# ruiminshen/yolo2-pytorch

Measured on AMD Instinct MI355X. Metric: images/sec (416x416) train+detect, Darknet-19 YOLOv2: value = TRAIN step, batch 64 per GPU (configs[2]) at every N; detect (configs[1]) = roofline.detect_images_per_sec, higher is better.
Workload: dtype f32; 1 GPU; Darknet-19 YOLOv2 20-class train 416x416 batch-64/GPU: fwd + region loss + bwd + SGD (BASELINE configs[2]); classes=20, global_batch=64, parallelism=single GPU, weights=random-init seed 0 (bench_data.randomize)

## Files before the change

### include/yolo2_hip.h

```cpp
#ifndef YOLO2_HIP_H
#define YOLO2_HIP_H

#include <stdint.h>

#ifdef __cplusplus
extern "C" {
#endif

#define Y2_OK 0
#define Y2_EINVAL (-1)
#define Y2_EALIGN (-2)
#define Y2_ENOSUP (-3)

#define Y2_STATS_REPL 32

typedef void* y2_stream_t;

int y2_abi_version(void);
const char* y2_build_info(void);


int y2_pack_weight(const float* w, float* dst, int Cout, int Cin, int ksize, int mode, y2_stream_t stream);

#define Y2_PREP_FPROP 0
#define Y2_PREP_DGRAD 1
#define Y2_PREP_WINO_FPROP 2
#define Y2_PREP_WINO_DGRAD 3
#define Y2_PREP_WINO6_DGRAD 4
#define Y2_PREP_MAX_ITEMS 96
typedef struct {
    const float* src;
    float* dst;
    int32_t Cout, Cin, ksize, mode;
} y2_prep_item;
int y2_prep_weights(const y2_prep_item* items, int32_t count, y2_stream_t stream);

#define Y2_MULTI_ZERO 0
#define Y2_MULTI_F64_TO_F32 1
#define Y2_MULTI_COPY 2
#define Y2_MULTI_MAX_ITEMS 96
typedef struct {
    const void* src;
    float* dst;
    int64_t n;
    int32_t op, reserved;
} y2_multi_item;
int y2_multi(const y2_multi_item* items, int32_t count, y2_stream_t stream);

int y2_small_dot(const float* v, const float* w, int32_t n, float* out, y2_stream_t stream);
int y2_small_scale(const float* g, const float* w, int32_t n, float* out, y2_stream_t stream);

int y2_unpack_weight_grad(const float* src, float* dst, int Cout, int Cin, int ksize, y2_stream_t stream);

int y2_bn_fold(const float* gamma, const float* beta, const float* mean, const float* var, float eps,
               float* scale, float* shift, int C, y2_stream_t stream);

typedef struct y2_conv_params {
    const float* x;
    const float* w;
    const float* scale;
    const float* shift;
    float* y;
    float* y_pool;
    double* stats;
    int32_t B, H, W;
    int32_t Cin, ldx;
    int32_t Cout;
    int32_t ksize;
    int32_t ldy, coff;
    int32_t ldp, poff;
    int32_t out_mode;
    float slope;
    int32_t tile;
    float* workspace;
    int64_t workspace_bytes;
    const float* residual;
    int32_t ldr;
    int32_t stride;
    int32_t pad_plus1;
    int32_t transposed;
    int32_t out_h, out_w;
    int32_t algo;
    int64_t w_plane;
} y2_conv_params;

#define Y2_ALGO_DIRECT 0
#define Y2_ALGO_WINOGRAD 1
#define Y2_ALGO_WINOGRAD_FUSED 2
#define Y2_ALGO_WINOGRAD_IMPLICIT 3
#define Y2_ALGO_WINOGRAD_SPLIT 4

#define Y2_ALGO_WINOGRAD_F43 6
#define Y2_ALGO_WINOGRAD_F43_PRE 7
#define Y2_ALGO_WINOGRAD_SPLIT_F16 5

int y2_split_f16x2(const float* src, void* dst, long long n, float scale, y2_stream_t stream);
int y2_split_f16_overflow(int reset);
int y2_gemm_split_f16(const void* A, const void* B, float* C, long long M, int32_t N, int32_t K, int32_t ldc, int32_t groups, float out_scale, y2_stream_t stream);

int y2_split_bf16x3(const float* src, void* dst, long long n, y2_stream_t stream);

int y2_gemm_split(const void* A, const void* B, float* C, long long M, int32_t N, int32_t K, int32_t ldc, int32_t groups, y2_stream_t stream);

int y2_wino_weight(const float* w_packed, float* u, int32_t Cout, int32_t Cin, y2_stream_t stream);
int y2_wino6_weight(const float* w_packed, float* u6, int32_t Cout, int32_t Cin, y2_stream_t stream);

long long y2_wino_wgrad_workspace_bytes(int32_t B, int32_t H, int32_t W, int32_t Cin, int32_t Cout);
long long y2_wino_wgrad_workspace_bytes_ex(int32_t B, int32_t H, int32_t W, int32_t Cin, int32_t Cout, int32_t native_layout);
int y2_wino_wgrad(const float* x, const float* dz, float* dw_packed, int32_t B, int32_t H, int32_t W, int32_t Cin, int32_t ldx,
                  int32_t Cout, int32_t ldz, const float* v_transformed, float* workspace, long long workspace_bytes, y2_stream_t stream);
int y2_wino_wgrad_ex(const float* x, const float* dz, float* dw, int32_t B, int32_t H, int32_t W, int32_t Cin, int32_t ldx,
                     int32_t Cout, int32_t ldz, const float* v_transformed, float* workspace, long long workspace_bytes, int32_t native_layout,
                     y2_stream_t stream);

int y2_conv_fwd(const y2_conv_params* p, y2_stream_t stream);

long long y2_conv_fwd_workspace_bytes(const y2_conv_params* p);

int y2_conv_fwd_batch(const y2_conv_params* params, int count, y2_stream_t stream);

int y2_conv0_fwd(const float* x_nchw, const float* w, const float* scale, const float* shift,
                 float* y, float* y_pool, double* stats,
                 int B, int H, int W, int Cin, int Cout, int ldy, int ldp, float slope, y2_stream_t stream);

int y2_maxpool2_fwd(const float* x, float* y, int B, int H, int W, int C, int ldx, int ldy, y2_stream_t stream);

int y2_maxpool_fwd(const float* x, float* y, int B, int H, int W, int C, int ldx, int ldy, int ksize, int stride, int pad, int pad_end, y2_stream_t stream);

int y2_nchw_to_nhwc(const float* x, float* y, int B, int C, int H, int W, int ld, y2_stream_t stream);

int y2_decode(const float* feature, const float* anchors, int B, int rows, int cols, int A, int C,
              float* iou, float* center_offset, float* size_norm, float* yx_min, float* yx_max, float* prob,
              float* prob_cls, int32_t* cls, y2_stream_t stream);

int y2_filter_visible(const float* iou, const float* prob, int B, int n, int C, int fix, float thr,
                      int32_t* count, int32_t* index, float* prob_cls, int32_t* cls, y2_stream_t stream);

int y2_expand_classes(const float* iou, const float* prob, const float* yx_min, const float* yx_max, const int32_t* cand, const int32_t* keep,
                      const int32_t* keep_count, int32_t B, int32_t n, int32_t C, int32_t limit, float threshold_cls, float* k_iou, float* k_min, float* k_max,
                      float* e_min, float* e_max, float* e_score, long long* e_cls, int32_t* e_count, y2_stream_t stream);

int y2_iou_rowmax(const float* yx_min1, const float* yx_max1, const float* yx_min2, const float* yx_max2, int32_t N1, int32_t N2, float min_union,
                  float* best, long long* which, y2_stream_t stream);

#define Y2_EVAL_MATCH_MAX_G 1024
int y2_eval_match(const float* det_min, const float* det_max, const long long* det_cls, const int32_t* det_count,
                  const float* gt_min, const float* gt_max, const long long* gt_cls, const uint8_t* gt_difficult,
                  int32_t B, int32_t M, int32_t G, int32_t C, float threshold, float min_union, uint8_t* tp, int32_t* cls_num, y2_stream_t stream);

#define Y2_COLLATE_MAX_W 4096
int y2_collate_images(const uint8_t* src, const int64_t* offset, const int32_t* geom, const float* lut,
                      int32_t B, int32_t H, int32_t W, int32_t flags, float* out, y2_stream_t stream);

#define Y2_WARP_MAX_DIM 16384
int y2_warp_affine_images(const uint8_t* src, const int64_t* src_offset, const int32_t* src_geom, const double* inv,
                          uint8_t* dst, const int64_t* dst_offset, const int32_t* dst_geom,
                          int32_t B, int32_t max_h, int32_t max_w, int32_t fill, y2_stream_t stream);

#define Y2_JITTER_MAX_BLUR 7
int y2_collate_jitter_images(const uint8_t* src, const int64_t* offset, const int32_t* geom, const int32_t* jitter, const uint8_t* hsv_tab,
                             const float* lut, int32_t B, int32_t H, int32_t W, int32_t flags, float* out, y2_stream_t stream);

#define Y2_JPEG_MAX_DIM 16384
#define Y2_JPEG_DESC_BYTES 4096
int y2_jpeg_decode_images(const uint8_t* src, int64_t src_bytes, const int64_t* src_offset, const uint8_t* desc,
                          uint8_t* dst, int64_t dst_bytes, const int64_t* dst_offset, const int32_t* dst_geom,
                          uint8_t* ws, int64_t ws_bytes, int32_t* status, int32_t B, y2_stream_t stream);

#define Y2_KMEANS_MAX_K 16
int y2_anchor_kmeans(const double* size, int32_t N, int32_t K, const int32_t* init, int32_t R, int32_t max_iter, double conv_test,
                     double* means, int32_t* iters, int32_t* status, double* cost, int32_t* counts, y2_stream_t stream);
int y2_anchor_assign(const double* size, int32_t N, const double* means, int32_t K, int32_t* index, double* iou, y2_stream_t stream);

int y2_iou_matrix(const float* yx_min1, const float* yx_max1, const float* yx_min2, const float* yx_max2,
                  int Bt, int N1, int N2, float min_union, int mode, float* out, y2_stream_t stream);
int y2_iou_pair(const float* yx_min1, const float* yx_max1, const float* yx_min2, const float* yx_max2,
                int n, float min_union, float* out, y2_stream_t stream);

int y2_nms(const float* score, const float* yx_min, const float* yx_max, const int32_t* cand, const int32_t* n, int B, int stride,
           float overlap, int limit, int32_t* order_ws, int32_t* keep, int32_t* keep_count, y2_stream_t stream);

int y2_nms_host(const float* score, const float* yx_min, const float* yx_max, const int32_t* cand, const int32_t* n, int B, int stride,
                float overlap, int limit, int32_t* keep, int32_t* keep_count);
int y2_iou_matrix_host(const float* yx_min1, const float* yx_max1, const float* yx_min2, const float* yx_max2,
                       int Bt, int N1, int N2, float min_union, int mode, float* out);
int y2_iou_pair_host(const float* yx_min1, const float* yx_max1, const float* yx_min2, const float* yx_max2,
                     int n, float min_union, float* out);
int y2_eval_match_host(const float* det_min, const float* det_max, const long long* det_cls, const int32_t* det_count,
                       const float* gt_min, const float* gt_max, const long long* gt_cls, const uint8_t* gt_difficult,
                       int32_t B, int32_t M, int32_t G, int32_t C, float threshold, float min_union, uint8_t* tp, int32_t* cls_num);
int y2_collate_images_host(const uint8_t* src, const int64_t* offset, const int32_t* geom, const float* lut,
                           int32_t B, int32_t H, int32_t W, int32_t flags, float* out);
int y2_warp_affine_images_host(const uint8_t* src, const int64_t* src_offset, const int32_t* src_geom, const double* inv,
                               uint8_t* dst, const int64_t* dst_offset, const int32_t* dst_geom,
                               int32_t B, int32_t max_h, int32_t max_w, int32_t fill);
int y2_collate_jitter_images_host(const uint8_t* src, const int64_t* offset, const int32_t* geom, const int32_t* jitter, const uint8_t* hsv_tab,
                                  const float* lut, int32_t B, int32_t H, int32_t W, int32_t flags, float* out);
int y2_jpeg_probe_host(const uint8_t* data, int64_t nbytes, uint8_t* desc);
long long y2_jpeg_workspace_bytes(const uint8_t* desc, int32_t B);
int y2_jpeg_decode_images_host(const uint8_t* src, int64_t src_bytes, const int64_t* src_offset, const uint8_t* desc,
                               uint8_t* dst, int64_t dst_bytes, const int64_t* dst_offset, const int32_t* dst_geom,
                               uint8_t* ws, int64_t ws_bytes, int32_t* status, int32_t B);
int y2_anchor_kmeans_host(const double* size, int32_t N, int32_t K, const int32_t* init, int32_t R, int32_t max_iter, double conv_test,
                          double* means, int32_t* iters, int32_t* status, double* cost, int32_t* counts);
int y2_anchor_assign_host(const double* size, int32_t N, const double* means, int32_t K, int32_t* index, double* iou);

int y2_set_deterministic(int on, float* workspace, long long workspace_bytes);
int y2_get_deterministic(void);
int y2_colstats_det(const float* z, long long M, int32_t C, int32_t ld, double* stats, float* workspace, long long workspace_bytes, y2_stream_t stream);

int y2_prof_enable(int on);
int y2_prof_count(void);
int y2_prof_get(int i, char* name, int name_cap, float* ms, double* flops);
int y2_prof_set_tag(int tag);
int y2_prof_get_tag(int i);


int y2_conv_wgrad(const float* x, const float* dz, float* dw, int B, int H, int W, int Cin, int ldx, int Cout, int ldz,
                  int ksize, y2_stream_t stream);

int y2_conv_wgrad_ex(const float* x, const float* dz, float* dw, int B, int Hi, int Wi, int Cin, int ldx, int Cout, int ldz,
                     int ksize, int stride, int pad, y2_stream_t stream);

int y2_conv0_wgrad(const float* x_nchw, const float* dz, float* dw, int B, int H, int W, int Cin, int Cout, int ldz, y2_stream_t stream);

int y2_conv0_wgrad_fused(const float* x_nchw, const float* z, const float* scale, const float* shift, const float* mean, const float* invstd,
                         const float* gamma, float slope, const float* dy_pool, int32_t ldp, const double* sums, float* dw,
                         int32_t B, int32_t H, int32_t W, int32_t Cin, int32_t Cout, int32_t ldz, int32_t has_bn, y2_stream_t stream);

int y2_bn_finalize(const double* stats, double count, const float* gamma, const float* beta,
                   float* running_mean, float* running_var, float momentum, float eps,
                   float* scale, float* shift, float* mean, float* invstd, int C, long long* num_batches_tracked, y2_stream_t stream);

int y2_bn_act_fwd(const float* z, const float* scale, const float* shift, float slope, float* y, float* y_pool,
                  int B, int H, int W, int C, int ldz, int ldy, int coff, int ldp, int poff, int out_mode, y2_stream_t stream);

int y2_bn_act_bwd(const float* z, const float* scale, const float* shift, const float* mean, const float* invstd, const float* gamma,
                  float slope, const float* dy_full, int ldf, int foff, int fmode, const float* dy_pool, int ldp, int poff,
                  double* sums, float* dz, int ldd, int B, int H, int W, int C, int ldz, int has_bn, y2_stream_t stream);

int y2_bn_act_fwd_ex(const float* z, const float* scale, const float* shift, float slope, const float* residual, int ldr, float* y, float* y_pool,
                     int B, int H, int W, int C, int ldz, int ldy, int coff, int ldp, int poff, int out_mode, y2_stream_t stream);
int y2_bn_act_bwd_ex(const float* z, const float* scale, const float* shift, const float* mean, const float* invstd, const float* gamma,
                     float slope, const float* dy_full, int ldf, int foff, int fmode, const float* dy_pool, int ldp, int poff,
                     const float* dy_full2, int ld2, const float* residual, int ldr, float* dres, int lddr,
                     double* sums, float* dz, int ldd, int B, int H, int W, int C, int ldz, int has_bn, y2_stream_t stream);

long long y2_wino6_tiles(int32_t B, int32_t H, int32_t W);
int y2_bn_act_bwd_wino6(const float* z, const float* scale, const float* shift, const float* mean, const float* invstd, const float* gamma,
                        float slope, const float* dy_full, int ldf, int foff, double* sums, float* v6, float* m6, float* dz, int ldd,
                        int B, int H, int W, int C, int ldz, int has_bn, y2_stream_t stream);

int y2_maxpool_bwd(const float* x, const float* dy, const float* dy2, float* dx, int B, int H, int W, int C, int ldx, int ldy, int lddx,
                   int ksize, int stride, int pad, int pad_end, y2_stream_t stream);

int y2_colsum(const float* x, long long M, int C, int ld, double* out, y2_stream_t stream);
int y2_f64_to_f32(const double* src, float* dst, int n, double mul, y2_stream_t stream);

int y2_decode_bwd(const float* iou, const float* center_offset, const float* d_iou, const float* d_center_offset, const float* d_size_norm,
                  const float* d_logits, float* d_feature, int boxes, int C, y2_stream_t stream);

int y2_region_loss_fwd(const float* iou, const float* center_offset, const float* size_norm, const float* logits,
                       const float* yx_min, const float* yx_max,
                       const float* gt_yx_min, const float* gt_yx_max, const int64_t* gt_cls, const float* gt_onehot,
                       const float* anchors, int B, int rows, int cols, int A, int C, int N, float threshold,
                       float* best_iou, int32_t* best_idx, uint8_t* positive, double* sums, float* loss_out, y2_stream_t stream);

int y2_region_loss_finalize(const double* sums, double cnt, int cross_entropy, float* loss_out, y2_stream_t stream);

int y2_region_loss_bwd(const float* iou, const float* center_offset, const float* size_norm, const float* logits,
                       const float* gt_yx_min, const float* gt_yx_max, const int64_t* gt_cls, const float* gt_onehot,
                       const float* anchors, int B, int rows, int cols, int A, int C, int N, float threshold,
                       const float* best_iou, const int32_t* best_idx, const uint8_t* positive, const double* sums, const float* weights,
                       float* d_iou, float* d_center_offset, float* d_size_norm, float* d_logits, y2_stream_t stream);

#define Y2_OPT_MAX_TENSORS 48
typedef struct {
    float* param;
    float* grad;
    float* state1;
    float* state2;
    int64_t numel;
} y2_opt_tensor;

int y2_opt_sgd(const y2_opt_tensor* tensors, int32_t count, float lr, float momentum, float dampening, float weight_decay,
               int32_t nesterov, int32_t first_step, y2_stream_t stream);
int y2_opt_adam(const y2_opt_tensor* tensors, int32_t count, float lr, float beta1, float beta2, float eps, float weight_decay,
                int32_t step, y2_stream_t stream);
int y2_opt_grad_sumsq(const y2_opt_tensor* tensors, int32_t count, double* sumsq, y2_stream_t stream);
int y2_opt_clip_grads(const y2_opt_tensor* tensors, int32_t count, const double* sumsq, float max_norm, y2_stream_t stream);

int y2_dwconv_fwd(const float* x, const float* w, const float* scale, const float* shift, float slope, float* y, double* stats,
                  int B, int H, int W, int C, int ldx, int ldy, int stride, y2_stream_t stream);
int y2_dwconv_dgrad(const float* dz, const float* w, float* dx, int B, int H, int W, int C, int ldz, int lddx, int stride, y2_stream_t stream);
int y2_dwconv_wgrad(const float* x, const float* dz, float* dw, float* workspace, long long workspace_bytes,
                    int B, int H, int W, int C, int ldx, int ldz, int stride, y2_stream_t stream);
long long y2_dwconv_wgrad_workspace_bytes(int B, int H, int W, int C, int stride);

int y2_preact_conv1x1_fwd(const float* x, const float* w, const float* pre_scale, const float* pre_shift, float pre_slope,
                          const float* scale, const float* shift, float slope, float* y, double* stats,
                          int B, int H, int W, int K, int ldx, int N, int ldy, int coff, int pool, y2_stream_t stream);
int y2_preact_fwd(const float* x, const float* pre_scale, const float* pre_shift, float pre_slope, float* out,
                  int B, int H, int W, int C, int ldx, int ldo, int pool, y2_stream_t stream);
int y2_preact_bwd(const float* x, const float* pre_scale, const float* pre_shift, float pre_slope, const float* mean, const float* invstd,
                  const float* gamma, const float* dA, int ldda, double* sums, float* dx, int lddx, int accumulate,
                  int B, int H, int W, int C, int ldx, int pool, int has_bn, y2_stream_t stream);

#ifdef __cplusplus
}
#endif
#endif
```

### yolo2-pytorch_amd/_hip.py

```python
import ctypes
import os
import subprocess

import torch

_HERE = os.path.dirname(os.path.abspath(__file__))
LIB_PATH = os.environ.get('Y2_LIB') or os.path.join(_HERE, 'csrc', 'libyolo2_hip.so')
_lib = None

c_int, c_float, c_void_p = ctypes.c_int, ctypes.c_float, ctypes.c_void_p


class ConvParams(ctypes.Structure):
    _fields_ = [('x', c_void_p), ('w', c_void_p), ('scale', c_void_p), ('shift', c_void_p),
                ('y', c_void_p), ('y_pool', c_void_p), ('stats', c_void_p),
                ('B', ctypes.c_int32), ('H', ctypes.c_int32), ('W', ctypes.c_int32),
                ('Cin', ctypes.c_int32), ('ldx', ctypes.c_int32), ('Cout', ctypes.c_int32), ('ksize', ctypes.c_int32),
                ('ldy', ctypes.c_int32), ('coff', ctypes.c_int32), ('ldp', ctypes.c_int32), ('poff', ctypes.c_int32),
                ('out_mode', ctypes.c_int32), ('slope', c_float), ('tile', ctypes.c_int32),
                ('workspace', c_void_p), ('workspace_bytes', ctypes.c_int64),
                ('residual', c_void_p), ('ldr', ctypes.c_int32), ('stride', ctypes.c_int32), ('pad_plus1', ctypes.c_int32),
                ('transposed', ctypes.c_int32), ('out_h', ctypes.c_int32), ('out_w', ctypes.c_int32), ('algo', ctypes.c_int32),
                ('w_plane', ctypes.c_int64)]


class OptTensor(ctypes.Structure):
    _fields_ = [('param', c_void_p), ('grad', c_void_p), ('state1', c_void_p), ('state2', c_void_p), ('numel', ctypes.c_int64)]


OPT_MAX_TENSORS = 48


class PrepItem(ctypes.Structure):
    _fields_ = [('src', c_void_p), ('dst', c_void_p), ('Cout', ctypes.c_int32), ('Cin', ctypes.c_int32), ('ksize', ctypes.c_int32), ('mode', ctypes.c_int32)]


PREP_FPROP, PREP_DGRAD, PREP_WINO_FPROP, PREP_WINO_DGRAD, PREP_WINO6_DGRAD = 0, 1, 2, 3, 4


class MultiItem(ctypes.Structure):
    _fields_ = [('src', c_void_p), ('dst', c_void_p), ('n', ctypes.c_int64), ('op', ctypes.c_int32), ('reserved', ctypes.c_int32)]


MULTI_ZERO, MULTI_F64_TO_F32, MULTI_COPY = 0, 1, 2

EVAL_MATCH_MAX_G = 1024
COLLATE_MAX_W = 4096
WARP_MAX_DIM = 16384
JITTER_MAX_BLUR = 7
JPEG_MAX_DIM = 16384
JPEG_DESC_BYTES = 4096
KMEANS_MAX_K = 16

SIGNATURES = {
    'y2_abi_version': [],
    'y2_pack_weight': [c_void_p, c_void_p, c_int, c_int, c_int, c_int, c_void_p],
    'y2_prep_weights': [ctypes.POINTER(PrepItem), c_int, c_void_p],
    'y2_expand_classes': [c_void_p] * 7 + [c_int, c_int, c_int, c_int, c_float] + [c_void_p] * 8 + [c_void_p],
    'y2_iou_rowmax': [c_void_p, c_void_p, c_void_p, c_void_p, c_int, c_int, c_float, c_void_p, c_void_p, c_void_p],
    'y2_split_bf16x3': [c_void_p, c_void_p, ctypes.c_longlong, c_void_p],
    'y2_split_f16x2': [c_void_p, c_void_p, ctypes.c_longlong, c_float, c_void_p],
    'y2_split_f16_overflow': [c_int],
    'y2_gemm_split_f16': [c_void_p, c_void_p, c_void_p, ctypes.c_longlong, c_int, c_int, c_int, c_int, c_float, c_void_p],
    'y2_gemm_split': [c_void_p, c_void_p, c_void_p, ctypes.c_longlong, c_int, c_int, c_int, c_int, c_void_p],
    'y2_multi': [ctypes.POINTER(MultiItem), c_int, c_void_p],
    'y2_small_dot': [c_void_p, c_void_p, c_int, c_void_p, c_void_p],
    'y2_small_scale': [c_void_p, c_void_p, c_int, c_void_p, c_void_p],
    'y2_unpack_weight_grad': [c_void_p, c_void_p, c_int, c_int, c_int, c_void_p],
    'y2_bn_fold': [c_void_p, c_void_p, c_void_p, c_void_p, c_float, c_void_p, c_void_p, c_int, c_void_p],
    'y2_conv_fwd': [ctypes.POINTER(ConvParams), c_void_p],
    'y2_conv_fwd_workspace_bytes': [ctypes.POINTER(ConvParams)],
    'y2_wino_weight': [c_void_p, c_void_p, c_int, c_int, c_void_p],
    'y2_wino6_weight': [c_void_p, c_void_p, c_int, c_int, c_void_p],
    'y2_opt_sgd': [ctypes.POINTER(OptTensor), c_int, c_float, c_float, c_float, c_float, c_int, c_int, c_void_p],
    'y2_opt_adam': [ctypes.POINTER(OptTensor), c_int, c_float, c_float, c_float, c_float, c_float, c_int, c_void_p],
    'y2_opt_grad_sumsq': [ctypes.POINTER(OptTensor), c_int, c_void_p, c_void_p],
    'y2_opt_clip_grads': [ctypes.POINTER(OptTensor), c_int, c_void_p, c_float, c_void_p],
    'y2_wino_wgrad_workspace_bytes': [c_int, c_int, c_int, c_int, c_int],
    'y2_wino_wgrad_workspace_bytes_ex': [c_int, c_int, c_int, c_int, c_int, c_int],
    'y2_wino_wgrad': [c_void_p, c_void_p, c_void_p, c_int, c_int, c_int, c_int, c_int, c_int, c_int, c_void_p, c_void_p, ctypes.c_longlong, c_void_p],
    'y2_wino_wgrad_ex': [c_void_p, c_void_p, c_void_p, c_int, c_int, c_int, c_int, c_int, c_int, c_int, c_void_p, c_void_p, ctypes.c_longlong, c_int, c_void_p],
    'y2_conv_fwd_batch': [ctypes.POINTER(ConvParams), c_int, c_void_p],
    'y2_conv0_fwd': [c_void_p, c_void_p, c_void_p, c_void_p, c_void_p, c_void_p, c_void_p,
                     c_int, c_int, c_int, c_int, c_int, c_int, c_int, c_float, c_void_p],
    'y2_maxpool2_fwd': [c_void_p, c_void_p, c_int, c_int, c_int, c_int, c_int, c_int, c_void_p],
    'y2_maxpool_fwd': [c_void_p, c_void_p, c_int, c_int, c_int, c_int, c_int, c_int, c_int, c_int, c_int, c_int, c_void_p],
    'y2_nchw_to_nhwc': [c_void_p, c_void_p, c_int, c_int, c_int, c_int, c_int, c_void_p],
    'y2_decode': [c_void_p, c_void_p, c_int, c_int, c_int, c_int, c_int,
                  c_void_p, c_void_p, c_void_p, c_void_p, c_void_p, c_void_p, c_void_p, c_void_p, c_void_p],
    'y2_filter_visible': [c_void_p, c_void_p, c_int, c_int, c_int, c_int, c_float, c_void_p, c_void_p, c_void_p, c_void_p, c_void_p],
    'y2_iou_matrix': [c_void_p, c_void_p, c_void_p, c_void_p, c_int, c_int, c_int, c_float, c_int, c_void_p, c_void_p],
    'y2_iou_pair': [c_void_p, c_void_p, c_void_p, c_void_p, c_int, c_float, c_void_p, c_void_p],
    'y2_conv_wgrad': [c_void_p, c_void_p, c_void_p, c_int, c_int, c_int, c_int, c_int, c_int, c_int, c_int, c_void_p],
    'y2_conv_wgrad_ex': [c_void_p, c_void_p, c_void_p, c_int, c_int, c_int, c_int, c_int, c_int, c_int, c_int, c_int, c_int, c_void_p],
    'y2_conv0_wgrad_fused': [c_void_p] * 7 + [c_float, c_void_p, c_int, c_void_p, c_void_p] + [c_int] * 7 + [c_void_p],
    'y2_conv0_wgrad': [c_void_p, c_void_p, c_void_p, c_int, c_int, c_int, c_int, c_int, c_int, c_void_p],
    'y2_bn_finalize': [c_void_p, ctypes.c_double, c_void_p, c_void_p, c_void_p, c_void_p, c_float, c_float, c_void_p, c_void_p, c_void_p, c_void_p, c_int, c_void_p, c_void_p],
    'y2_bn_act_fwd': [c_void_p, c_void_p, c_void_p, c_float, c_void_p, c_void_p, c_int, c_int, c_int, c_int, c_int, c_int, c_int, c_int, c_int, c_int, c_void_p],
    'y2_bn_act_bwd': [c_void_p, c_void_p, c_void_p, c_void_p, c_void_p, c_void_p, c_float, c_void_p, c_int, c_int, c_int, c_void_p, c_int, c_int,
                      c_void_p, c_void_p, c_int, c_int, c_int, c_int, c_int, c_int, c_int, c_void_p],
    'y2_bn_act_fwd_ex': [c_void_p, c_void_p, c_void_p, c_float, c_void_p, c_int, c_void_p, c_void_p, c_int, c_int, c_int, c_int, c_int, c_int, c_int, c_int, c_int, c_int, c_void_p],
    'y2_bn_act_bwd_ex': [c_void_p, c_void_p, c_void_p, c_void_p, c_void_p, c_void_p, c_float, c_void_p, c_int, c_int, c_int, c_void_p, c_int, c_int,
                         c_void_p, c_int, c_void_p, c_int, c_void_p, c_int,
                         c_void_p, c_void_p, c_int, c_int, c_int, c_int, c_int, c_int, c_int, c_void_p],
    'y2_wino6_tiles': [c_int, c_int, c_int],
    'y2_bn_act_bwd_wino6': [c_void_p, c_void_p, c_void_p, c_void_p, c_void_p, c_void_p, c_float, c_void_p, c_int, c_int, c_void_p, c_void_p, c_void_p, c_void_p, c_int,
                            c_int, c_int, c_int, c_int, c_int, c_int, c_void_p],
    'y2_maxpool_bwd': [c_void_p, c_void_p, c_void_p, c_void_p, c_int, c_int, c_int, c_int, c_int, c_int, c_int, c_int, c_int, c_int, c_int, c_void_p],
    'y2_colsum': [c_void_p, ctypes.c_longlong, c_int, c_int, c_void_p, c_void_p],
    'y2_dwconv_fwd': [c_void_p, c_void_p, c_void_p, c_void_p, c_float, c_void_p, c_void_p, c_int, c_int, c_int, c_int, c_int, c_int, c_int, c_void_p],
    'y2_dwconv_dgrad': [c_void_p, c_void_p, c_void_p, c_int, c_int, c_int, c_int, c_int, c_int, c_int, c_void_p],
    'y2_dwconv_wgrad': [c_void_p, c_void_p, c_void_p, c_void_p, ctypes.c_longlong, c_int, c_int, c_int, c_int, c_int, c_int, c_int, c_void_p],
    'y2_dwconv_wgrad_workspace_bytes': [c_int, c_int, c_int, c_int, c_int],
    'y2_preact_conv1x1_fwd': [c_void_p, c_void_p, c_void_p, c_void_p, c_float, c_void_p, c_void_p, c_float, c_void_p, c_void_p] + [c_int] * 9 + [c_void_p],
    'y2_preact_fwd': [c_void_p, c_void_p, c_void_p, c_float, c_void_p] + [c_int] * 7 + [c_void_p],
    'y2_preact_bwd': [c_void_p, c_void_p, c_void_p, c_float, c_void_p, c_void_p, c_void_p, c_void_p, c_int, c_void_p, c_void_p, c_int, c_int] + [c_int] * 7 + [c_void_p],
    'y2_f64_to_f32': [c_void_p, c_void_p, c_int, ctypes.c_double, c_void_p],
    'y2_decode_bwd': [c_void_p, c_void_p, c_void_p, c_void_p, c_void_p, c_void_p, c_void_p, c_int, c_int, c_void_p],
    'y2_region_loss_fwd': [c_void_p] * 11 + [c_int] * 6 + [c_float] + [c_void_p] * 5 + [c_void_p],
    'y2_region_loss_finalize': [c_void_p, ctypes.c_double, c_int, c_void_p, c_void_p],
    'y2_region_loss_bwd': [c_void_p] * 9 + [c_int] * 6 + [c_float] + [c_void_p] * 5 + [c_void_p] * 4 + [c_void_p],
    'y2_nms_host': [c_void_p, c_void_p, c_void_p, c_void_p, c_void_p, c_int, c_int, c_float, c_int, c_void_p, c_void_p],
    'y2_iou_matrix_host': [c_void_p, c_void_p, c_void_p, c_void_p, c_int, c_int, c_int, c_float, c_int, c_void_p],
    'y2_iou_pair_host': [c_void_p, c_void_p, c_void_p, c_void_p, c_int, c_float, c_void_p],
    'y2_eval_match': [c_void_p] * 8 + [c_int, c_int, c_int, c_int, c_float, c_float, c_void_p, c_void_p, c_void_p],
    'y2_eval_match_host': [c_void_p] * 8 + [c_int, c_int, c_int, c_int, c_float, c_float, c_void_p, c_void_p],
    'y2_collate_images': [c_void_p] * 4 + [c_int, c_int, c_int, c_int, c_void_p, c_void_p],
    'y2_collate_images_host': [c_void_p] * 4 + [c_int, c_int, c_int, c_int, c_void_p],
    'y2_warp_affine_images': [c_void_p] * 7 + [c_int, c_int, c_int, c_int, c_void_p],
    'y2_warp_affine_images_host': [c_void_p] * 7 + [c_int, c_int, c_int, c_int],
    'y2_collate_jitter_images': [c_void_p] * 6 + [c_int, c_int, c_int, c_int, c_void_p, c_void_p],
    'y2_collate_jitter_images_host': [c_void_p] * 6 + [c_int, c_int, c_int, c_int, c_void_p],
    'y2_jpeg_probe_host': [c_void_p, ctypes.c_int64, c_void_p],
    'y2_jpeg_workspace_bytes': [c_void_p, c_int],
    'y2_jpeg_decode_images': [c_void_p, ctypes.c_int64, c_void_p, c_void_p, c_void_p, ctypes.c_int64, c_void_p, c_void_p, c_void_p, ctypes.c_int64, c_void_p, c_int, c_void_p],
    'y2_jpeg_decode_images_host': [c_void_p, ctypes.c_int64, c_void_p, c_void_p, c_void_p, ctypes.c_int64, c_void_p, c_void_p, c_void_p, ctypes.c_int64, c_void_p, c_int],
    'y2_anchor_kmeans': [c_void_p, c_int, c_int, c_void_p, c_int, c_int, ctypes.c_double] + [c_void_p] * 5 + [c_void_p],
    'y2_anchor_kmeans_host': [c_void_p, c_int, c_int, c_void_p, c_int, c_int, ctypes.c_double] + [c_void_p] * 5,
    'y2_anchor_assign': [c_void_p, c_int, c_void_p, c_int, c_void_p, c_void_p, c_void_p],
    'y2_anchor_assign_host': [c_void_p, c_int, c_void_p, c_int, c_void_p, c_void_p],
    'y2_set_deterministic': [c_int, c_void_p, ctypes.c_longlong],
    'y2_get_deterministic': [],
    'y2_colstats_det': [c_void_p, ctypes.c_longlong, c_int, c_int, c_void_p, c_void_p, ctypes.c_longlong, c_void_p],
    'y2_prof_enable': [c_int],
    'y2_prof_count': [],
    'y2_prof_set_tag': [c_int],
    'y2_prof_get_tag': [c_int],
    'y2_prof_get': [c_int, ctypes.c_char_p, c_int, ctypes.POINTER(c_float), ctypes.POINTER(ctypes.c_double)],
    'y2_nms': [c_void_p, c_void_p, c_void_p, c_void_p, c_void_p, c_int, c_int, c_float, c_int, c_void_p, c_void_p, c_void_p, c_void_p],
}

STATS_REPL = 32

ERRORS = {-1: 'Y2_EINVAL (bad size / null pointer)', -2: 'Y2_EALIGN (unaligned pointer or stride)', -3: 'Y2_ENOSUP (unsupported combination)'}


class HipLibraryMissing(RuntimeError):
    pass


def build(verbose=False):
    out = subprocess.run(['bash', os.path.join(_HERE, 'csrc', 'build.sh')], capture_output=True, text=True)
    if verbose or out.returncode != 0:
        print(out.stdout + out.stderr)
    if out.returncode != 0:
        raise RuntimeError('building libyolo2_hip.so failed')
    return LIB_PATH


def lib():
    global _lib
    if _lib is None:
        if not os.path.exists(LIB_PATH):
            raise HipLibraryMissing('%s not found: run `python __graft_entry__.py build` (or yolo2-pytorch_amd/csrc/build.sh); '
                                    'the YOLOv2 hot path has no CPU/eager fallback' % LIB_PATH)
        l = ctypes.CDLL(LIB_PATH)
        for name, argtypes in SIGNATURES.items():
            fn = getattr(l, name)
            fn.argtypes = argtypes
            fn.restype = c_int
        l.y2_conv_fwd_workspace_bytes.restype = ctypes.c_longlong
        l.y2_wino_wgrad_workspace_bytes.restype = ctypes.c_longlong
        l.y2_wino6_tiles.restype = ctypes.c_longlong
        l.y2_dwconv_wgrad_workspace_bytes.restype = ctypes.c_longlong
        l.y2_wino_wgrad_workspace_bytes_ex.restype = ctypes.c_longlong
        l.y2_jpeg_workspace_bytes.restype = ctypes.c_longlong
        l.y2_build_info.argtypes = []
        l.y2_build_info.restype = ctypes.c_char_p
        _lib = l
    return _lib


LAUNCHES = [0]


def check(rc, what):
    LAUNCHES[0] += 1
    if rc != 0:
        if rc <= -1000:
            raise RuntimeError('%s: HIP error %d' % (what, -rc - 1000))
        raise RuntimeError('%s: %s' % (what, ERRORS.get(rc, rc)))


_LAUNCH = None


def stream():
    return c_void_p((_LAUNCH if _LAUNCH is not None else torch.cuda.current_stream()).cuda_stream)


class launch_on(object):

    def __init__(self, s):
        self.s, self.prev = s, None

    def __enter__(self):
        global _LAUNCH
        self.prev, _LAUNCH = _LAUNCH, self.s
        return self.s

    def __exit__(self, *exc):
        global _LAUNCH
        _LAUNCH = self.prev
        return False


def _timing_stream():
    import contextlib
    return torch.cuda.stream(_LAUNCH) if _LAUNCH is not None else contextlib.nullcontext()


def ptr(t):
    return None if t is None else c_void_p(t.data_ptr())


def multi(items, st=None):
    if not items:
        return
    table = (MultiItem * len(items))()
    for e, (op, dst, src) in zip(table, items):
        e.op, e.dst = op, dst.data_ptr()
        if op == MULTI_ZERO:
            nbytes = dst.numel() * dst.element_size()
            assert nbytes % 4 == 0 and dst.is_contiguous()
            e.n, e.src = nbytes // 4, None
        else:
            assert dst.dtype == torch.float32 and dst.is_contiguous() and src.is_contiguous() and src.numel() >= dst.numel()
            e.n, e.src = dst.numel(), src.data_ptr()
    check(lib().y2_multi(table, len(items), stream() if st is None else st), 'y2_multi')


def require_gpu(*tensors):
    for t in tensors:
        if t is not None and not t.is_cuda:
            raise RuntimeError('yolo2-hip: this operator runs only on an MI355X GPU tensor (got device %s); there is no CPU fallback' % t.device)


def wrote(tensors):
    try:
        torch.autograd.graph.increment_version(tensors)
    except TypeError:
        for t in tensors:
            torch.autograd.graph.increment_version(t)


_TUNE_EPOCH = [0]


def tune_epoch():
    return _TUNE_EPOCH[0]


DETERMINISTIC = os.environ.get('Y2_DETERMINISTIC', '0') == '1'
_DET_WS = {}
_DET_BYTES = int(os.environ.get('Y2_DET_WS_MB', '256')) << 20


def set_deterministic(on, dev=None):
    global DETERMINISTIC
    DETERMINISTIC = bool(on)
    L = lib()
    if not on:
        check(L.y2_set_deterministic(0, None, 0), 'y2_set_deterministic')
        return
    dev = torch.device('cuda', torch.cuda.current_device()) if dev is None else torch.device(dev)
    ws = _DET_WS.get(str(dev))
    if ws is None:
        ws = torch.empty(_DET_BYTES // 4, dtype=torch.float32, device=dev)
        _DET_WS[str(dev)] = ws
    check(L.y2_set_deterministic(1, ws.data_ptr(), ws.numel() * 4), 'y2_set_deterministic')


def ensure_deterministic(dev):
    if DETERMINISTIC and (str(torch.device(dev)) not in _DET_WS or not lib().y2_get_deterministic()):
        set_deterministic(True, dev)
    return DETERMINISTIC


def colstats_det(z, M, C, ld, stats):
    G = min(1024, (M + 255) // 256)
    key = 'colstats:' + str(z.device)
    ws = _DET_WS.get(key)
    if ws is None or ws.numel() * 4 < G * 2 * C * 8:
        ws = torch.empty(max(G * 2 * C * 2, 1 << 18), dtype=torch.float32, device=z.device)
        _DET_WS[key] = ws
    check(lib().y2_colstats_det(ptr(z), M, C, ld, ptr(stats), ptr(ws), ws.numel() * 4, stream()), 'y2_colstats_det')


_WS = {}
SCOPE = None


def _cache(d):
    if SCOPE is None:
        return d
    return SCOPE.setdefault(('_hip', id(d)), {})


def workspace(dev, nbytes):
    key = str(dev)
    ws = _cache(_WS)
    t = ws.get(key)
    if t is None or t.numel() * 4 < nbytes:
        _retire(t)
        t = torch.empty(max(int(nbytes) // 4 + 4, 1024), dtype=torch.float32, device=dev)
        ws[key] = t
    return t


def _retire(t):
    if t is not None and SCOPE is not None:
        SCOPE.setdefault(('_hip', 'retired'), []).append(t)


def conv_workspace(params, dev):
    need = lib().y2_conv_fwd_workspace_bytes(ctypes.byref(params))
    if need > 0:
        ws = workspace(dev, need)
        params.workspace, params.workspace_bytes = ws.data_ptr(), ws.numel() * 4
    else:
        params.workspace, params.workspace_bytes = None, 0
    return need


class PlanCache(object):

    def __init__(self, entries=None, gbytes=None):
        import collections
        self.entries = int(os.environ.get('Y2_PLAN_CACHE', '12')) if entries is None else entries
        self.bytes = int(float(os.environ.get('Y2_PLAN_CACHE_GB', '64')) * (1 << 30)) if gbytes is None else int(gbytes * (1 << 30))
        self.d = collections.OrderedDict()
        self.hits = self.misses = 0

    def get(self, key):
        plan = self.d.get(key)
        if plan is None:
            self.misses += 1
            return None
        self.hits += 1
        self.d.move_to_end(key)
        return plan

    def put(self, key, plan, nbytes):
        self.d[key] = plan
        plan['nbytes'] = nbytes
        while len(self.d) > 1 and (len(self.d) > self.entries or sum(p['nbytes'] for p in self.d.values()) > self.bytes):
            self.d.popitem(last=False)

    def latest(self):
        return next(reversed(self.d.values())) if self.d else None

    def clear(self):
        self.d.clear()


_TUNE = {}
TUNE_MISSES = []
AUTOTUNE = os.environ.get('Y2_AUTOTUNE', '1') != '0'
TUNE_CACHE = os.environ.get('Y2_TUNE_CACHE')
if TUNE_CACHE and os.path.exists(TUNE_CACHE):
    try:
        import json as _json
        _TUNE.update({tuple(_json.loads(k)): v for k, v in _json.load(open(TUNE_CACHE)).items()})
    except Exception:
        pass


TUNE_DEFAULTS = os.environ.get('Y2_TUNE_DEFAULTS', '1') != '0'
DEFAULTS_PATH = os.path.join(_HERE, 'tune', 'default_gfx950.json')
_DEFAULTS_SEEN = {}


def kernel_hash():
    import glob
    import hashlib
    files = sorted(glob.glob(os.path.join(_HERE, 'csrc', '*.hip'))) + [os.path.join(_HERE, 'csrc', 'common.h'), os.path.join(_HERE, 'csrc', 'resample.h'), os.path.join(_HERE, 'csrc', 'jpeg.h'), os.path.join(_HERE, 'csrc', 'kmeans.h'), os.path.join(os.path.dirname(_HERE), 'include', 'yolo2_hip.h')]
    if len(files) < 3 or not all(os.path.exists(f) for f in files):
        return None
    h = hashlib.sha256()
    for f in files:
        h.update(os.path.basename(f).encode())
        for line in open(f, 'r', errors='replace'):
            if line.startswith('// y2-build-flags:'):
                h.update(line.strip().encode())
                h.update(b'\n')
            cut = line.find('//')
            while cut >= 0 and line.count('"', 0, cut) % 2:
# ... 383 lines not shown
```

### yolo2-pytorch_amd/csrc/conv0_fwd.hip

```cpp
#include <stdlib.h>
#include "common.h"

namespace {

constexpr int TH = 16, TW = 32;
constexpr int PW = 48;
constexpr int PLANE = (TH + 2) * PW;

struct Conv0Args {
    const float* x; const float* w; const float* scale; const float* shift;
    float* y; float* y_pool; double* stats;
    int B, H, W, Cout, ldy, ldp;
    float slope;
    int tiles_y, tiles_x, ntiles;
};

typedef float f32x2 __attribute__((ext_vector_type(2)));

template <int CIN>
struct StepTap {
    static constexpr int G0 = 3 * CIN, G1 = G0 + CIN, G2 = G1 + CIN / 2;
    static constexpr int group(int s) { return s < G0 ? 0 : s < G1 ? 1 : s < G2 ? 2 : 3; }
    static constexpr int tap0(int s) {
        return s < G0 ? (s / 3) * 9 + (s % 3) * 3 : s < G1 ? (s - G0) * 9 + 2 : s < G2 ? (2 * (s - G1)) * 9 + 8 : (CIN - 1) * 9 + 8;
    }
    static constexpr int tap1(int s) {
        return s < G0 ? tap0(s) + 1 : s < G1 ? tap0(s) + 3 : s < G2 ? tap0(s) + 9 : -1;
    }
    static constexpr int lds(int tap) { return (tap / 9) * PLANE + ((tap % 9) / 3) * PW + (tap % 3); }
    static constexpr int dist(int g) { return g == 0 ? 1 : g == 1 ? PW : g == 2 ? PLANE : 0; }
};

template <int CIN, int NBLK, int OUT = -1, bool FULL = false, bool RAW = false>
__global__ __launch_bounds__(256) void conv0_kernel(const Conv0Args a) {
    const bool has_y = OUT < 0 ? a.y != nullptr : (OUT & 1) != 0;
    const bool has_pool = OUT < 0 ? a.y_pool != nullptr : (OUT & 2) != 0;
    const bool has_stats = OUT < 0 ? a.stats != nullptr : (OUT & 4) != 0;
    constexpr bool POOL_FIRST = FULL && OUT == 2 && !RAW;
    constexpr int K = CIN * 9;
    constexpr int KS = (K + 1) / 2;
    constexpr int PR = TH + 2;
    constexpr int RPW = (PR + 3) / 4, RIT = CIN * RPW;
    __shared__ __attribute__((aligned(16))) float patch[3][CIN * PLANE];

    const int t = threadIdx.x;
    const int lane = t & 63, wave = __builtin_amdgcn_readfirstlane(t >> 6);
    const int l31 = lane & 31, half = lane >> 5;
    const int ldy = FULL ? 32 * NBLK : a.ldy, ldp = FULL ? 32 * NBLK : a.ldp;

    float sc[NBLK], sh[NBLK];
#pragma unroll
    for (int j = 0; j < NBLK; ++j) {
        const int n = j * 32 + l31;
        sc[j] = (!RAW && a.scale != nullptr && n < a.Cout) ? a.scale[n] : 1.f;
        sh[j] = (!RAW && a.shift != nullptr && n < a.Cout) ? a.shift[n] : 0.f;
    }
    float wreg[NBLK][KS];
#pragma unroll
    for (int j = 0; j < NBLK; ++j) {
        const int n = j * 32 + l31;
#pragma unroll
        for (int s = 0; s < KS; ++s) {
            const int k = half ? StepTap<CIN>::tap1(s) : StepTap<CIN>::tap0(s);
            const float w = (n < a.Cout && k >= 0) ? a.w[(size_t)n * K + k] : 0.f;
            wreg[j][s] = (POOL_FIRST && sc[j] < 0.f) ? -w : w;
        }
        if (POOL_FIRST) sc[j] = fabsf(sc[j]);
    }

    float pv[RIT];
    const int HW = a.H * a.W;
    auto origin = [&](int tile, int& b, int& y0, int& x0) {
        const unsigned u = (unsigned)tile, row = u / (unsigned)a.tiles_x, tx = u - row * (unsigned)a.tiles_x;
        const unsigned ub = row / (unsigned)a.tiles_y, ty = row - ub * (unsigned)a.tiles_y;
        b = (int)ub; y0 = (int)ty * TH; x0 = (int)tx * TW;
    };
    auto issue = [&](int b, int y0, int x0) {
        const float* xb = a.x + (size_t)b * CIN * HW;
        const int gx = min(max(x0 + lane - 1, 0), a.W - 1);
#pragma unroll
        for (int it = 0; it < RIT; ++it) {
            const int c = it / RPW, py = min(wave + 4 * (it % RPW), PR - 1);
            const int gy = min(max(y0 + py - 1, 0), a.H - 1);
            const float* rowp = xb + (c * HW + gy * a.W);
            pv[it] = rowp[gx];
        }
    };
    auto commit = [&](int y0, int x0, float* dst) {
        const bool okx = (unsigned)(x0 + lane - 1) < (unsigned)a.W;
        float* d = dst + wave * PW + lane;
        if (lane < TW + 2) {
#pragma unroll
            for (int it = 0; it < RIT; ++it) {
                const int c = it / RPW, k4 = 4 * (it % RPW), py = wave + k4;
                const bool oky = (unsigned)(y0 + py - 1) < (unsigned)a.H;
                const float v = (okx && oky) ? pv[it] : 0.f;
                if (k4 + 3 < PR || py < PR) d[c * PLANE + k4 * PW] = v;
            }
        }
    };

    double d1[NBLK], d2[NBLK];
#pragma unroll
    for (int j = 0; j < NBLK; ++j) { d1[j] = 0.0; d2[j] = 0.0; }
    const int stride = gridDim.x;
    int tile = blockIdx.x;
    __builtin_amdgcn_s_waitcnt(0x0f70);
    int b, y0, x0, b1 = 0, y1 = 0, x1 = 0;
    origin(tile, b, y0, x0);
    issue(b, y0, x0);
    commit(y0, x0, patch[0]);
    if (tile + stride < a.ntiles) { origin(tile + stride, b1, y1, x1); issue(b1, y1, x1); commit(y1, x1, patch[1]); }
    __syncthreads();

    const int wi = l31 >> 2, e = l31 & 3;
    const int lpy = e >> 1, lpx = 2 * wi + (e & 1);
    int buf = 0;
    for (; tile < a.ntiles; tile += stride, buf = buf == 2 ? 0 : buf + 1) {
    const float* cur = patch[buf];
    const bool more = tile + 2 * stride < a.ntiles;
    int b2 = 0, y2 = 0, x2 = 0;
    f32x2 s1[NBLK], s2[NBLK];
#pragma unroll
    for (int j = 0; j < NBLK; ++j) { s1[j] = 0.f; s2[j] = 0.f; }
    const int bt = b, yt = y0, xt = x0;

#pragma unroll 1
    for (int blk = 0; blk < 4; blk += 2) {
        const int rp = (wave * 4 + blk) >> 1;
        const int pbase = (2 * rp + lpy) * PW + lpx;
        f32x16 acc[2][NBLK];
#pragma unroll
        for (int u = 0; u < 2; ++u)
#pragma unroll
            for (int j = 0; j < NBLK; ++j)
#pragma unroll
                for (int r = 0; r < 16; ++r) acc[u][j][r] = 0.f;
        float av[2][KS];
        const float* gb[4];
#pragma unroll
        for (int g = 0; g < 4; ++g) gb[g] = cur + pbase + (half ? StepTap<CIN>::dist(g) : 0);
#pragma unroll
        for (int s = 0; s < KS; ++s) {
            const int g = StepTap<CIN>::group(s);
#pragma unroll
            for (int u = 0; u < 2; ++u) {
                av[u][s] = gb[g][StepTap<CIN>::lds(StepTap<CIN>::tap0(s)) + 16 * u];
                if (g == 3) av[u][s] = half ? 0.f : av[u][s];
            }
        }
        __builtin_amdgcn_sched_barrier(0);
#if defined(Y2_C0_DBG) && (Y2_C0_DBG & 1)
#pragma unroll
        for (int u = 0; u < 2; ++u)
#pragma unroll
            for (int j = 0; j < NBLK; ++j)
#pragma unroll
                for (int r = 0; r < 16; ++r) acc[u][j][r] = av[u][r % KS] * wreg[j][r % KS];
#else
#pragma unroll
        for (int s = 0; s < KS; ++s)
#pragma unroll
            for (int u = 0; u < 2; ++u)
#pragma unroll
                for (int j = 0; j < NBLK; ++j)
                    acc[u][j] = __builtin_amdgcn_mfma_f32_32x32x2f32(av[u][s], wreg[j][s], acc[u][j], 0, 0, 0);
#endif
#if !(defined(Y2_C0_DBG) && (Y2_C0_DBG & 4))
        if (more) {
            if (blk == 0) { origin(tile + 2 * stride, b2, y2, x2); issue(b2, y2, x2); }
            else commit(y2, x2, patch[buf == 0 ? 2 : buf - 1]);
        }
#endif
#if defined(Y2_C0_DBG) && (Y2_C0_DBG & 2)
        if (acc[0][0][0] + acc[1][0][5] == 12345.678f) a.y_pool[lane] = 1.f;
        if (false)
#endif
#pragma unroll
        for (int u = 0; u < 2; ++u) {
        const int Y0 = yt + 2 * rp, X0 = xt + 16 * u;
        float* yb0 = has_y ? a.y + ((size_t)(bt * a.H + Y0) * a.W + X0) * ldy : nullptr;
        float* yb1 = has_y ? yb0 + (size_t)a.W * ldy : nullptr;
        float* pb = has_pool ? a.y_pool + ((size_t)(bt * (a.H >> 1) + (Y0 >> 1)) * (a.W >> 1) + (X0 >> 1)) * ldp : nullptr;
        const unsigned ylane = (unsigned)(2 * half * ldy + l31), plane = (unsigned)(half * ldp + l31);
#pragma unroll
        for (int j = 0; j < NBLK; ++j) {
            const int n = j * 32 + l31;
            const bool nok = FULL || n < a.Cout;
#pragma unroll
            for (int g = 0; g < 4; ++g) {
                const int w = 2 * g + half;
                const int Y = Y0, X = X0 + 2 * w;
                if (has_stats) {
                    if (FULL) {
                        const f32x2 za = {acc[u][j][4 * g], acc[u][j][4 * g + 1]}, zb = {acc[u][j][4 * g + 2], acc[u][j][4 * g + 3]};
                        s1[j] += za; s2[j] = __builtin_elementwise_fma(za, za, s2[j]);
                        s1[j] += zb; s2[j] = __builtin_elementwise_fma(zb, zb, s2[j]);
                    } else {
#pragma unroll
                        for (int q = 0; q < 4; ++q) {
                            const float z = acc[u][j][4 * g + q];
                            if ((Y + (q >> 1)) < a.H && (X + (q & 1)) < a.W) { s1[j][q & 1] += z; s2[j][q & 1] += z * z; }
                        }
                    }
                }
                if (!nok) continue;
                if (POOL_FIRST) {
                    const float m = fmaxf(fmaxf(acc[u][j][4 * g], acc[u][j][4 * g + 1]), fmaxf(acc[u][j][4 * g + 2], acc[u][j][4 * g + 3]));
                    const float uu = m * sc[j] + sh[j];
                    (pb + (2 * g * ldp + j * 32))[plane] = fmaxf(uu, uu * a.slope);
                    continue;
                }
                float v[4];
#pragma unroll
                for (int q = 0; q < 4; ++q) {
                    const float z = acc[u][j][4 * g + q];
                    if (RAW) { v[q] = z; continue; }
                    const float uu = z * sc[j] + sh[j];
                    v[q] = uu > 0.f ? uu : uu * a.slope;
                }
                if (has_y) {
#pragma unroll
                    for (int q = 0; q < 4; ++q) {
                        const int yy = Y + (q >> 1), xx = X + (q & 1);
                        if (FULL || (yy < a.H && xx < a.W)) (((q >> 1) ? yb1 : yb0) + ((4 * g + (q & 1)) * ldy + j * 32))[ylane] = v[q];
                    }
                }
                if (has_pool && (FULL || (Y < a.H && X < a.W))) {
                    const float pm = fmaxf(fmaxf(v[0], v[1]), fmaxf(v[2], v[3]));
                    (pb + (2 * g * ldp + j * 32))[plane] = pm;
                }
            }
        }
        }
    }
    if (has_stats) {
#pragma unroll
        for (int j = 0; j < NBLK; ++j) { d1[j] += (double)s1[j][0] + (double)s1[j][1]; d2[j] += (double)s2[j][0] + (double)s2[j][1]; }
    }
    b = b1; y0 = y1; x0 = x1; b1 = b2; y1 = y2; x1 = x2;
    __syncthreads();
    }
    if (has_stats) {
#pragma unroll
        for (int j = 0; j < NBLK; ++j) {
            const int n = j * 32 + l31;
            const double t1 = d1[j] + __shfl_xor(d1[j], 32);
            const double t2 = d2[j] + __shfl_xor(d2[j], 32);
            if (half == 0 && n < a.Cout) {
                double* st = a.stats + (size_t)(blockIdx.x % Y2_STATS_REPL) * 2 * a.Cout;
                atomicAdd(st + n, t1);
                atomicAdd(st + a.Cout + n, t2);
            }
        }
    }
}

template <int CIN>
int launch0(const Conv0Args& a, hipStream_t s) {
    const long long tiles = (long long)a.B * a.tiles_y * a.tiles_x;
    if (tiles <= 0 || tiles > 0x7fffffffLL) return Y2_EINVAL;
    static const int per_cu = getenv("Y2_CONV0_WGS") != nullptr ? atoi(getenv("Y2_CONV0_WGS")) : 8;
    const long long grid = per_cu > 0 && tiles > (long long)Y2_NUM_CU * per_cu ? (long long)Y2_NUM_CU * per_cu : tiles;
    const double flops = 2.0 * (double)a.B * a.H * a.W * 9 * CIN * a.Cout;
    if (CIN == 3 && (a.H % TH) == 0 && (a.W % TW) == 0 && (a.Cout == 32 || a.Cout == 64) && (a.y == nullptr || a.ldy == a.Cout) && (a.y_pool == nullptr || a.ldp == a.Cout)) {
        const int out = (a.y != nullptr ? 1 : 0) | (a.y_pool != nullptr ? 2 : 0) | (a.stats != nullptr ? 4 : 0);
        const bool raw = a.scale == nullptr && a.shift == nullptr && a.slope == 1.f;
        const bool mono = a.slope >= 0.f && a.slope <= 1.f;
#define Y2_C0(NB_, OUT_, RAW_) Y2_LAUNCH("conv0_kernel", flops, (conv0_kernel<3, NB_, OUT_, true, RAW_>), dim3((unsigned)grid), dim3(256), 0, s, a)
        bool done = true;
        if (a.Cout == 32) {
            if (out == 2 && mono) Y2_C0(1, 2, false); else if (out == 5 && raw) Y2_C0(1, 5, true); else if (out == 5) Y2_C0(1, 5, false);
            else if (out == 1) Y2_C0(1, 1, false); else if (out == 3) Y2_C0(1, 3, false); else done = false;
        } else {
            if (out == 2 && mono) Y2_C0(2, 2, false); else if (out == 5 && raw) Y2_C0(2, 5, true); else if (out == 1) Y2_C0(2, 1, false); else done = false;
        }
#undef Y2_C0
        if (done) { Y2_LAUNCH_CHECK(); return Y2_OK; }
    }
    if (a.Cout <= 32) Y2_LAUNCH("conv0_kernel", flops, (conv0_kernel<CIN, 1>), dim3((unsigned)grid), dim3(256), 0, s, a);
    else Y2_LAUNCH("conv0_kernel", flops, (conv0_kernel<CIN, 2>), dim3((unsigned)grid), dim3(256), 0, s, a);
    Y2_LAUNCH_CHECK();
    return Y2_OK;
}

}

extern "C" int y2_conv0_fwd(const float* x_nchw, const float* w, const float* scale, const float* shift,
                            float* y, float* y_pool, double* stats,
                            int B, int H, int W, int Cin, int Cout, int ldy, int ldp, float slope, y2_stream_t stream) {
    if (x_nchw == nullptr || w == nullptr || (y == nullptr && y_pool == nullptr && stats == nullptr)) return Y2_EINVAL;
    if (B <= 0 || H <= 0 || W <= 0 || Cin < 1 || Cin > 4 || Cout < 1 || Cout > 64) return Y2_ENOSUP;
    if (y != nullptr && ldy < Cout) return Y2_EINVAL;
    if (y_pool != nullptr && (ldp < Cout || (H & 1) || (W & 1))) return Y2_EINVAL;
    if (stats != nullptr && y2_det.on) return Y2_ENOSUP;
    Conv0Args a;
    a.x = x_nchw; a.w = w; a.scale = scale; a.shift = shift; a.y = y; a.y_pool = y_pool; a.stats = stats;
    a.B = B; a.H = H; a.W = W; a.Cout = Cout; a.ldy = ldy; a.ldp = ldp; a.slope = slope;
    a.tiles_y = y2_cdiv(H, TH); a.tiles_x = y2_cdiv(W, TW);
    a.ntiles = B * a.tiles_y * a.tiles_x;
    hipStream_t s = y2_s(stream);
    switch (Cin) {
        case 1: return launch0<1>(a, s);
        case 2: return launch0<2>(a, s);
        case 3: return launch0<3>(a, s);
        default: return launch0<4>(a, s);
    }
}
```

### yolo2-pytorch_amd/csrc/train.hip

```cpp
#include "common.h"

namespace {

inline int stream_grid(long long total, int block, int cap_mult = 8) {
    long long g = (total + block - 1) / block;
    const long long cap = (long long)Y2_NUM_CU * cap_mult;
    return (int)(g < 1 ? 1 : (g > cap ? cap : g));
}

__global__ void bn_finalize_kernel(const double* __restrict__ stats, double n, const float* gamma, const float* beta,
                                   float* running_mean, float* running_var, float momentum, float eps,
                                   float* scale, float* shift, float* mean_out, float* invstd_out, int C, long long* num_batches_tracked) {
    const int c = blockIdx.x * blockDim.x + threadIdx.x;
    if (c >= C) return;
    if (c == 0 && num_batches_tracked != nullptr) *num_batches_tracked += 1;
    double s1 = 0.0, s2 = 0.0;
    for (int r = 0; r < Y2_STATS_REPL; ++r) { s1 += stats[(size_t)r * 2 * C + c]; s2 += stats[(size_t)r * 2 * C + C + c]; }
    const double mean = s1 / n;
    double var = s2 / n - mean * mean;
    if (var < 0.0) var = 0.0;
    const float invstd = (float)(1.0 / sqrt(var + (double)eps));
    const float s = gamma[c] * invstd;
    scale[c] = s;
    shift[c] = beta[c] - (float)mean * s;
    mean_out[c] = (float)mean;
    invstd_out[c] = invstd;
    if (running_mean != nullptr) {
        const double unbiased = n > 1.0 ? var * n / (n - 1.0) : var;
        running_mean[c] = (1.f - momentum) * running_mean[c] + momentum * (float)mean;
        running_var[c] = (1.f - momentum) * running_var[c] + momentum * (float)unbiased;
    }
}

struct ActArgs {
    const float* z; const float* scale; const float* shift;
    float* y; float* y_pool;
    int B, H, W, C, ldz, ldy, coff, ldp, poff, out_mode;
    float slope;
    const float* res; int ldr;
    y2_fastdiv d_wo, d_ho;
};

__device__ __forceinline__ float act1(float z, float sc, float sh, float slope) {
    const float u = z * sc + sh;
    return u > 0.f ? u : u * slope;
}

__device__ __forceinline__ void act_decode(uint32_t p, const y2_fastdiv& d_wo, const y2_fastdiv& d_ho, int Wo, int Ho, int& b, int& yo, int& xo) {
    const uint32_t r = y2_div(p, d_wo);
    xo = (int)(p - r * (uint32_t)Wo);
    const uint32_t bb = y2_div(r, d_ho);
    yo = (int)(r - bb * (uint32_t)Ho);
    b = (int)bb;
}

template <bool POOL, int CV>
__global__ void bn_act_fwd_kernel(const ActArgs a, long long total) {
    const int Cg = a.C / CV;
    const int Wo = POOL ? a.W / 2 : a.W, Ho = POOL ? a.H / 2 : a.H;
    const long long tid = (long long)blockIdx.x * blockDim.x + threadIdx.x;
    const long long nthreads = (long long)gridDim.x * blockDim.x;
    const int c = (int)(tid % Cg) * CV;
    const uint32_t npix = (uint32_t)(total / Cg), pstep = (uint32_t)(nthreads / Cg);
    float sc[CV], sh[CV];
#pragma unroll
    for (int e = 0; e < CV; ++e) { sc[e] = a.scale ? a.scale[c + e] : 1.f; sh[e] = a.shift ? a.shift[c + e] : 0.f; }
    const bool need_yx = POOL || a.out_mode == 1;
    for (uint32_t p = (uint32_t)(tid / Cg); p < npix; p += pstep) {
        int b = 0, yo = 0, xo = 0;
        if (need_yx) act_decode(p, a.d_wo, a.d_ho, Wo, Ho, b, yo, xo);
        float pm[CV];
#pragma unroll
        for (int q = 0; q < (POOL ? 4 : 1); ++q) {
            const int yy = POOL ? 2 * yo + (q >> 1) : yo, xx = POOL ? 2 * xo + (q & 1) : xo;
            const long long pix = need_yx ? ((long long)b * a.H + yy) * a.W + xx : (long long)p;
            float v[CV];
            if (CV == 4) {
                const f32x4 zz = *reinterpret_cast<const f32x4*>(a.z + pix * a.ldz + c);
                f32x4 rr = {0.f, 0.f, 0.f, 0.f};
                if (a.res != nullptr) rr = *reinterpret_cast<const f32x4*>(a.res + pix * a.ldr + c);
#pragma unroll
                for (int e = 0; e < 4; ++e) { const float u = zz[e] * sc[e] + sh[e] + rr[e]; v[e] = u > 0.f ? u : u * a.slope; }
            } else {
                const float u = a.z[pix * a.ldz + c] * sc[0] + sh[0] + (a.res != nullptr ? a.res[pix * a.ldr + c] : 0.f);
                v[0] = u > 0.f ? u : u * a.slope;
            }
            if (a.y != nullptr) {
                long long o;
                if (a.out_mode == 1) {
                    o = (((long long)b * (a.H >> 1) + (yy >> 1)) * (a.W >> 1) + (xx >> 1)) * a.ldy + a.coff + ((yy & 1) * 2 + (xx & 1)) * a.C + c;
                } else {
                    o = pix * a.ldy + a.coff + c;
                }
                if (CV == 4) { f32x4 w = {v[0], v[1], v[2], v[3]}; *reinterpret_cast<f32x4*>(a.y + o) = w; }
                else a.y[o] = v[0];
            }
#pragma unroll
            for (int e = 0; e < CV; ++e) pm[e] = (q == 0) ? v[e] : fmaxf(pm[e], v[e]);
        }
        if (POOL && a.y_pool != nullptr) {
            const long long o = (long long)p * a.ldp + a.poff + c;
            if (CV == 4) { f32x4 w = {pm[0], pm[1], pm[2], pm[3]}; *reinterpret_cast<f32x4*>(a.y_pool + o) = w; }
            else a.y_pool[o] = pm[0];
        }
    }
}

struct ActBwdArgs {
    const float* z; const float* scale; const float* shift; const float* mean; const float* invstd; const float* gamma;
    const float* dy_full; const float* dy_pool;
    const float* dy_full2; int ld2;
    const float* res; int ldr;
    float* dres; int lddr;
    double* sums;
    float* partial;
    float* block_partial;
    float* dz;
    int B, H, W, C, ldz, ldf, foff, fmode, ldp, poff, ldd;
    float slope;
    double n;
    int has_bn;
    y2_fastdiv d_wo, d_ho;
};

template <bool POOL, int CV, bool APPLY>
__global__ void bn_act_bwd_kernel(const ActBwdArgs a, long long total) {
    extern __shared__ float red[];
    const int Cg = a.C / CV;
    if (!APPLY) {
        for (int i = threadIdx.x; i < 2 * a.C; i += blockDim.x) red[i] = 0.f;
        __syncthreads();
    }
    const int Wo = POOL ? a.W / 2 : a.W, Ho = POOL ? a.H / 2 : a.H;
    const long long tid = (long long)blockIdx.x * blockDim.x + threadIdx.x;
    const long long nthreads = (long long)gridDim.x * blockDim.x;
    const int c = (int)(tid % Cg) * CV;
    float sc[CV], sh[CV], mu[CV], is[CV], gs[CV], ma[CV], mb[CV];
#pragma unroll
    for (int e = 0; e < CV; ++e) {
        sc[e] = a.scale ? a.scale[c + e] : 1.f; sh[e] = a.shift ? a.shift[c + e] : 0.f;
        mu[e] = a.has_bn ? a.mean[c + e] : 0.f; is[e] = a.has_bn ? a.invstd[c + e] : 1.f;
        if (APPLY && a.has_bn == 1) {
            gs[e] = a.gamma[c + e] * is[e];
            ma[e] = (float)(a.sums[c + e] / a.n);
            mb[e] = (float)(a.sums[a.C + c + e] / a.n);
        } else if (APPLY && a.has_bn == 2) {
            gs[e] = a.gamma[c + e] * is[e]; ma[e] = 0.f; mb[e] = 0.f;
        } else { gs[e] = 1.f; ma[e] = 0.f; mb[e] = 0.f; }
    }
    float s1[CV], s2[CV];
#pragma unroll
    for (int e = 0; e < CV; ++e) { s1[e] = 0.f; s2[e] = 0.f; }

    const uint32_t npix = (uint32_t)(total / Cg), pstep = (uint32_t)(nthreads / Cg);
    const bool need_yx = POOL || a.fmode == 1;
    for (uint32_t p = (uint32_t)(tid / Cg); p < npix; p += pstep) {
        int b = 0, yo = 0, xo = 0;
        if (need_yx) act_decode(p, a.d_wo, a.d_ho, Wo, Ho, b, yo, xo);
        float zv[POOL ? 4 : 1][CV], yv[POOL ? 4 : 1][CV];
        long long pixs[POOL ? 4 : 1];
#pragma unroll
        for (int q = 0; q < (POOL ? 4 : 1); ++q) {
            const int yy = POOL ? 2 * yo + (q >> 1) : yo, xx = POOL ? 2 * xo + (q & 1) : xo;
            pixs[q] = need_yx ? ((long long)b * a.H + yy) * a.W + xx : (long long)p;
            if (CV == 4) {
                const f32x4 zz = *reinterpret_cast<const f32x4*>(a.z + pixs[q] * a.ldz + c);
#pragma unroll
                for (int e = 0; e < 4; ++e) zv[q][e] = zz[e];
            } else zv[q][0] = a.z[pixs[q] * a.ldz + c];
#pragma unroll
            for (int e = 0; e < CV; ++e) yv[q][e] = zv[q][e] * sc[e] + sh[e];
            if (a.res != nullptr) {
                if (CV == 4) {
                    const f32x4 rr = *reinterpret_cast<const f32x4*>(a.res + pixs[q] * a.ldr + c);
#pragma unroll
                    for (int e = 0; e < 4; ++e) yv[q][e] += rr[e];
                } else yv[q][0] += a.res[pixs[q] * a.ldr + c];
            }
        }
        float dp[CV];
        int arg[CV];
        if (POOL) {
            const long long o = (long long)p * a.ldp + a.poff + c;
            if (CV == 4) { const f32x4 d = *reinterpret_cast<const f32x4*>(a.dy_pool + o);
#pragma unroll
                for (int e = 0; e < 4; ++e) dp[e] = d[e]; }
            else dp[0] = a.dy_pool[o];
#pragma unroll
            for (int e = 0; e < CV; ++e) {
                float best = 0.f; int bi = 0;
#pragma unroll
                for (int q = 0; q < 4; ++q) {
                    const float u = yv[q][e];
                    const float v = u > 0.f ? u : u * a.slope;
                    if (q == 0 || v > best) { best = v; bi = q; }
                }
                arg[e] = bi;
            }
        }
#pragma unroll
        for (int q = 0; q < (POOL ? 4 : 1); ++q) {
            float g[CV];
#pragma unroll
            for (int e = 0; e < CV; ++e) g[e] = (POOL && arg[e] == q) ? dp[e] : 0.f;
            if (a.dy_full != nullptr) {
                const int yy = POOL ? 2 * yo + (q >> 1) : yo, xx = POOL ? 2 * xo + (q & 1) : xo;
                long long o;
                if (a.fmode == 1) o = (((long long)b * (a.H >> 1) + (yy >> 1)) * (a.W >> 1) + (xx >> 1)) * a.ldf + a.foff + ((yy & 1) * 2 + (xx & 1)) * a.C + c;
                else o = pixs[q] * a.ldf + a.foff + c;
                if (CV == 4) { const f32x4 d = *reinterpret_cast<const f32x4*>(a.dy_full + o);
#pragma unroll
                    for (int e = 0; e < 4; ++e) g[e] += d[e]; }
                else g[0] += a.dy_full[o];
            }
            if (a.dy_full2 != nullptr) {
                const long long o = pixs[q] * a.ld2 + c;
                if (CV == 4) { const f32x4 d = *reinterpret_cast<const f32x4*>(a.dy_full2 + o);
#pragma unroll
                    for (int e = 0; e < 4; ++e) g[e] += d[e]; }
                else g[0] += a.dy_full2[o];
            }
            float outv[CV], gev[CV];
#pragma unroll
            for (int e = 0; e < CV; ++e) {
                const float ge = g[e] * (yv[q][e] > 0.f ? 1.f : a.slope);
                gev[e] = ge;
                const float zh = (zv[q][e] - mu[e]) * is[e];
                if (!APPLY) { s1[e] += ge; s2[e] += ge * zh; }
                else outv[e] = gs[e] * (ge - ma[e] - zh * mb[e]);
            }
            if (APPLY) {
                const long long o = pixs[q] * a.ldd + c;
                if (CV == 4) { f32x4 w = {outv[0], outv[1], outv[2], outv[3]}; *reinterpret_cast<f32x4*>(a.dz + o) = w; }
                else a.dz[o] = outv[0];
                if (a.dres != nullptr) {
                    const long long r = pixs[q] * a.lddr + c;
                    if (CV == 4) { f32x4 w = {gev[0], gev[1], gev[2], gev[3]}; *reinterpret_cast<f32x4*>(a.dres + r) = w; }
                    else a.dres[r] = gev[0];
                }
            }
        }
    }
    if (!APPLY && a.partial != nullptr) {
        float* row = a.partial + (size_t)(tid / Cg) * 2 * a.C;
#pragma unroll
        for (int e = 0; e < CV; ++e) { row[c + e] = s1[e]; row[a.C + c + e] = s2[e]; }
        return;
    }
    if (!APPLY) {
#pragma unroll
        for (int e = 0; e < CV; ++e) { atomicAdd(&red[c + e], s1[e]); atomicAdd(&red[a.C + c + e], s2[e]); }
        __syncthreads();
        if (a.block_partial != nullptr) {
            float* row = a.block_partial + (size_t)blockIdx.x * 2 * a.C;
            for (int i = threadIdx.x; i < 2 * a.C; i += blockDim.x) row[i] = red[i];
            return;
        }
        for (int i = threadIdx.x; i < 2 * a.C; i += blockDim.x) {
            const float v = red[i];
            if (v != 0.f) atomicAdd(a.sums + i, (double)v);
        }
    }
}

__global__ __launch_bounds__(1024) void bn_bwd_block_reduce_kernel(const float* __restrict__ part, int rows, int n, double* __restrict__ sums) {
    __shared__ double acc[16][65];
    const int col = blockIdx.x * 64 + (threadIdx.x & 63), lane = threadIdx.x >> 6;
    const int per = (rows + (int)gridDim.y - 1) / (int)gridDim.y;
    const int r0 = blockIdx.y * per, r1 = min(rows, r0 + per);
    double s = 0.0;
    if (col < n)
        for (int r = r0 + lane; r < r1; r += 16) s += (double)part[(size_t)r * n + col];
    acc[lane][threadIdx.x & 63] = s;
    __syncthreads();
    if (lane == 0 && col < n) {
        double t = 0.0;
#pragma unroll
        for (int l = 0; l < 16; ++l) t += acc[l][threadIdx.x & 63];
        atomicAdd(sums + col, t);
    }
}

struct BnWino6Args {
    const float* z; const float* scale; const float* shift; const float* mean; const float* invstd; const float* gamma;
    const float* dy; const double* sums;
    float* v6; float* m6;
    float* dz;
    int B, H, W, C, ldz, ldf, foff, ldd, has_bn;
    float slope;
    double n;
    int th, tw, T, tall, wide, gx;
    y2_fastdiv d_c, d_tt, d_tw, d_tall, d_wide;
};

__global__ __launch_bounds__(256) void bn_bwd_wino6_kernel(const BnWino6Args a) {
    constexpr float BT[6][6] = {{1.f, 1.5f, -2.f, -1.5f, 1.f, 0.f}, {0.f, -1.f, -2.5f, -0.5f, 1.f, 0.f}, {0.f, 1.f, 0.5f, -2.5f, 1.f, 0.f},
                                {0.f, -0.5f, -1.f, 0.5f, 1.f, 0.f}, {0.f, 2.f, -1.f, -2.f, 1.f, 0.f}, {0.f, 1.f, 1.5f, -2.f, -1.5f, 1.f}};
    constexpr float GM[6][4] = {{1.f, 0.f, 0.f, 0.f}, {-1.f / 3, -1.f / 3, -1.f / 3, -1.f / 3}, {1.f / 3, -1.f / 3, 1.f / 3, -1.f / 3},
                                {1.f / 15, 2.f / 15, 4.f / 15, 8.f / 15}, {-16.f / 15, 8.f / 15, -4.f / 15, 2.f / 15}, {0.f, 0.f, 0.f, 1.f}};
    const uint32_t idx = blockIdx.x * 256u + threadIdx.x;
    const uint32_t t = y2_div(idx, a.d_c);
    if (t >= (uint32_t)a.T) return;
    const int c = (int)(idx - t * (uint32_t)a.C);
    const float sc = a.scale ? a.scale[c] : 1.f, sh = a.shift ? a.shift[c] : 0.f;
    const float mu = a.has_bn ? a.mean[c] : 0.f, is = a.has_bn ? a.invstd[c] : 1.f;
    float gs = 1.f, ma = 0.f, mb = 0.f;
    if (a.has_bn == 1) { gs = a.gamma[c] * is; ma = (float)(a.sums[c] / a.n); mb = (float)(a.sums[a.C + c] / a.n); }
    else if (a.has_bn == 2) { gs = a.gamma[c] * is; }
    int b = 0, ty, tx;
    if (a.tall) {
        ty = (int)y2_div(t, a.d_tw);
        tx = (int)t - ty * a.tw;
    } else {
        b = (int)y2_div(t, a.d_tt);
        const int r = (int)t - b * a.th * a.tw;
        ty = (int)y2_div((uint32_t)r, a.d_tw);
        tx = r - ty * a.tw;
    }
    const int y0 = 4 * ty - 1, x0 = 4 * tx - 1;
    int colx[6], colb[6];
#pragma unroll
    for (int j = 0; j < 6; ++j) {
        int xx = x0 + j, bx = 0;
        bool ok = (unsigned)xx < (unsigned)a.W;
        if (a.wide) {
            ok = (unsigned)xx < (unsigned)(a.gx * a.wide);
            bx = ok ? (int)y2_div((uint32_t)xx, a.d_wide) : 0;
            xx -= bx * a.wide;
            ok = ok && xx < a.W;
        }
        colx[j] = ok ? xx : -1;
        colb[j] = bx;
    }
    float d[6][6];
#pragma unroll
    for (int half = 0; half < 2; ++half) {
        uint32_t pixs[3][6];
        bool oks[3][6];
#pragma unroll
        for (int ii = 0; ii < 3; ++ii) {
            int yy = y0 + 3 * half + ii, by = 0;
            bool rowok = (unsigned)yy < (unsigned)a.H;
            if (a.tall) {
                rowok = yy >= 0;
                by = rowok ? (int)y2_div((uint32_t)yy, a.d_tall) : 0;
                yy -= by * a.tall;
                rowok = rowok && yy < a.H;
            }
#pragma unroll
            for (int j = 0; j < 6; ++j) {
                const int bb = a.tall ? by * a.gx + colb[j] : b;
                const bool ok = rowok && colx[j] >= 0 && bb < a.B;
                oks[ii][j] = ok;
                pixs[ii][j] = ok ? (uint32_t)((bb * a.H + yy) * a.W + colx[j]) : 0u;
            }
        }
        float zs[3][6], gsrc[3][6];
#pragma unroll
        for (int ii = 0; ii < 3; ++ii)
#pragma unroll
            for (int j = 0; j < 6; ++j) {
                zs[ii][j] = a.z[(size_t)pixs[ii][j] * a.ldz + c];
                gsrc[ii][j] = a.dy[(size_t)pixs[ii][j] * a.ldf + a.foff + c];
            }
#pragma unroll
        for (int ii = 0; ii < 3; ++ii)
#pragma unroll
            for (int j = 0; j < 6; ++j) {
                const int i = 3 * half + ii;
                const float zv = zs[ii][j];
                const float g = 0.f + gsrc[ii][j];
                const float yv = zv * sc + sh;
                const float ge = g * (yv > 0.f ? 1.f : a.slope);
                const float zh = (zv - mu) * is;
                const float v = oks[ii][j] ? gs * (ge - ma - zh * mb) : 0.f;
                if (a.dz != nullptr && oks[ii][j] && i >= 1 && i <= 4 && j >= 1 && j <= 4) a.dz[(size_t)pixs[ii][j] * a.ldd + c] = v;
                d[i][j] = v;
            }
    }
    const size_t plane = (size_t)a.T * a.C;
    if (a.v6 != nullptr) {
        float sm[6][6];
#pragma unroll
        for (int u = 0; u < 6; ++u)
#pragma unroll
            for (int j = 0; j < 6; ++j) {
                float v = 0.f;
#pragma unroll
                for (int i = 0; i < 6; ++i)
                    if (BT[u][i] != 0.f) v += BT[u][i] * d[i][j];
                sm[u][j] = v;
            }
        float* dst = a.v6 + (size_t)t * a.C + c;
#pragma unroll
        for (int u = 0; u < 6; ++u)
#pragma unroll
            for (int v6 = 0; v6 < 6; ++v6) {
                float v = 0.f;
#pragma unroll
                for (int j = 0; j < 6; ++j)
                    if (BT[v6][j] != 0.f) v += BT[v6][j] * sm[u][j];
                dst[(size_t)(6 * u + v6) * plane] = v;
            }
    }
    if (a.m6 != nullptr) {
        float sm[6][4];
// ... 130 lines not shown
        const int wx = w % WW, wy = w / WW;
        const int oy = y0 / 2 + wy, ox = x0 / 2 + wx;
        int at = 255;
        if (oy < Ho && ox < Wo) {
            float best = 0.f;
#pragma unroll
            for (int ky = 0; ky < 3; ++ky) {
                const int gy = 2 * oy - 1 + ky;
                if ((unsigned)gy >= (unsigned)H) continue;
#pragma unroll
                for (int kx = 0; kx < 3; ++kx) {
                    const int gx = 2 * ox - 1 + kx;
                    if ((unsigned)gx >= (unsigned)W) continue;
                    const float v = xs[((2 * wy + ky) * RW + 2 * wx + kx) * MP_CH + c];
                    if (at == 255 || v > best) { best = v; at = ky * 3 + kx; }
                }
            }
        }
        arg[i] = (unsigned char)at;
    }
    __syncthreads();
    const float* dyb = dy + (size_t)b * Ho * Wo * ldy + c0;
    const float* dy2b = dy2 != nullptr ? dy2 + (size_t)b * Ho * Wo * ldy + c0 : nullptr;
    for (int i = t; i < MP_TH * MP_TW * (MP_CH / 4); i += 256) {
        const int c4 = i % (MP_CH / 4), p = i / (MP_CH / 4);
        const int lx = p % MP_TW, ly = p / MP_TW;
        const int yy = y0 + ly, xx = x0 + lx;
        if (yy >= H || xx >= W) continue;
        float g[4] = {0.f, 0.f, 0.f, 0.f};
#pragma unroll
        for (int a = 0; a < 2; ++a) {
            const int oy = (yy + 1) / 2 - a;
            if (oy < 0 || oy >= Ho || 2 * oy - 1 > yy || 2 * oy + 1 < yy) continue;
#pragma unroll
            for (int bb = 0; bb < 2; ++bb) {
                const int ox = (xx + 1) / 2 - bb;
                if (ox < 0 || ox >= Wo || 2 * ox - 1 > xx || 2 * ox + 1 < xx) continue;
                const int mine = (yy - (2 * oy - 1)) * 3 + (xx - (2 * ox - 1));
                const unsigned char* aw = arg + ((oy - y0 / 2) * WW + (ox - x0 / 2)) * MP_CH + 4 * c4;
                const bool m0 = aw[0] == mine, m1 = aw[1] == mine, m2 = aw[2] == mine, m3 = aw[3] == mine;
                if (m0 || m1 || m2 || m3) {
                    const size_t o = ((size_t)oy * Wo + ox) * ldy + 4 * c4;
                    float4 d = *reinterpret_cast<const float4*>(dyb + o);
                    if (dy2b != nullptr) { const float4 e = *reinterpret_cast<const float4*>(dy2b + o); d.x += e.x; d.y += e.y; d.z += e.z; d.w += e.w; }
                    if (m0) g[0] += d.x;
                    if (m1) g[1] += d.y;
                    if (m2) g[2] += d.z;
                    if (m3) g[3] += d.w;
                }
            }
        }
        *reinterpret_cast<float4*>(dx + ((size_t)(b * H + yy) * W + xx) * lddx + c0 + 4 * c4) = make_float4(g[0], g[1], g[2], g[3]);
    }
}

__global__ void colsum_kernel(const float* __restrict__ x, long long M, int C, int ld, double* out) {
    extern __shared__ float red[];
    for (int i = threadIdx.x; i < C; i += blockDim.x) red[i] = 0.f;
    __syncthreads();
    const long long total = M * C;
    const long long tid = (long long)blockIdx.x * blockDim.x + threadIdx.x, nth = (long long)gridDim.x * blockDim.x;
    const int c = (int)(tid % C);
    float s = 0.f;
    for (long long i = tid; i < total; i += nth) s += x[(i / C) * ld + c];
    atomicAdd(&red[c], s);
    __syncthreads();
    for (int i = threadIdx.x; i < C; i += blockDim.x) if (red[i] != 0.f) atomicAdd(out + i, (double)red[i]);
}

__global__ void f64_to_f32_kernel(const double* s, float* d, int n, double mul) {
    const int i = blockIdx.x * blockDim.x + threadIdx.x;
    if (i < n) d[i] = (float)(s[i] * mul);
}

__global__ void decode_bwd_kernel(const float* __restrict__ iou, const float* __restrict__ co, const float* __restrict__ d_iou,
                                  const float* __restrict__ d_co, const float* __restrict__ d_sn, const float* __restrict__ d_logits,
                                  float* __restrict__ dfeat, int total, int C) {
    const int E = 5 + C;
    for (long long i = (long long)blockIdx.x * blockDim.x + threadIdx.x; i < (long long)total * E; i += (long long)gridDim.x * blockDim.x) {
        const int box = (int)(i / E), k = (int)(i % E);
        float v;
        if (k == 0) { const float s = iou[box]; v = d_iou ? d_iou[box] * s * (1.f - s) : 0.f; }
        else if (k < 3) { const float s = co[2 * (size_t)box + k - 1]; v = d_co ? d_co[2 * (size_t)box + k - 1] * s * (1.f - s) : 0.f; }
        else if (k < 5) v = d_sn ? d_sn[2 * (size_t)box + k - 3] : 0.f;
        else v = d_logits ? d_logits[(size_t)box * C + k - 5] : 0.f;
        dfeat[i] = v;
    }
}

__device__ __forceinline__ float iou_box(float ymin1, float xmin1, float ymax1, float xmax1,
                                         float ymin2, float xmin2, float ymax2, float xmax2) {
    const float ih = fmaxf(fminf(ymax1, ymax2) - fmaxf(ymin1, ymin2), 0.f);
    const float iw = fmaxf(fminf(xmax1, xmax2) - fmaxf(xmin1, xmin2), 0.f);
    const float inter = ih * iw;
    const float a1 = (ymax1 - ymin1) * (xmax1 - xmin1);
    const float a2 = (ymax2 - ymin2) * (xmax2 - xmin2);
    const float uni = fmaxf((a1 + a2) - inter, 1.1920929e-07f);
    return inter / uni;
}

__global__ __launch_bounds__(256) void loss_match_kernel(const float* __restrict__ yx_min, const float* __restrict__ yx_max,
                                                         const float* __restrict__ gt_min, const float* __restrict__ gt_max,
                                                         int n, int N, float* best_iou, int32_t* best_idx, uint8_t* positive, double* sums) {
    __shared__ float g[4 * 256];
    const int b = blockIdx.y;
    const int i = blockIdx.x * 256 + threadIdx.x;
    if (blockIdx.x == 0 && b == 0 && threadIdx.x < 6) sums[threadIdx.x] = 0.0;
    if (i < n) positive[(size_t)b * n + i] = 0;
    float y0 = 0, x0 = 0, y1 = 0, x1 = 0;
    if (i < n) {
        const size_t o = ((size_t)b * n + i) * 2;
        y0 = yx_min[o]; x0 = yx_min[o + 1]; y1 = yx_max[o]; x1 = yx_max[o + 1];
    }
    float best = 0.f; int arg = 0; bool first = true;
    for (int j0 = 0; j0 < N; j0 += 256) {
        const int cnt = min(256, N - j0);
        __syncthreads();
        if (threadIdx.x < cnt) {
            const size_t o = ((size_t)b * N + j0 + threadIdx.x) * 2;
            g[4 * threadIdx.x] = gt_min[o]; g[4 * threadIdx.x + 1] = gt_min[o + 1];
            g[4 * threadIdx.x + 2] = gt_max[o]; g[4 * threadIdx.x + 3] = gt_max[o + 1];
        }
        __syncthreads();
        for (int j = 0; j < cnt; ++j) {
            const float v = iou_box(y0, x0, y1, x1, g[4 * j], g[4 * j + 1], g[4 * j + 2], g[4 * j + 3]);
            if (first || v > best) { best = v; arg = j0 + j; first = false; }
        }
    }
    if (i < n) { best_iou[(size_t)b * n + i] = best; best_idx[(size_t)b * n + i] = arg; }
}

__global__ void loss_positive_kernel(const float* __restrict__ gt_min, const float* __restrict__ gt_max, const float* __restrict__ anchors,
                                     int B, int N, int rows, int cols, int A, uint8_t* positive) {
    const int i = blockIdx.x * blockDim.x + threadIdx.x;
    if (i >= B * N) return;
    const int b = i / N;
    const float y0 = gt_min[2 * (size_t)i], x0 = gt_min[2 * (size_t)i + 1], y1 = gt_max[2 * (size_t)i], x1 = gt_max[2 * (size_t)i + 1];
    if (!(y0 < y1 && x0 < x1)) return;
    const float cy = (y0 + y1) / 2.f, cx = (x0 + x1) / 2.f;
    const int ci = (int)floorf(cy), cj = (int)floorf(cx);
    if (ci < 0 || ci >= rows || cj < 0 || cj >= cols) return;
    float best = 0.f; int arg = 0;
    for (int k = 0; k < A; ++k) {
        const float ah = anchors[2 * k] / 2.f, aw = anchors[2 * k + 1] / 2.f;
        const float v = iou_box(y0 - cy, x0 - cx, y1 - cy, x1 - cx, -ah, -aw, ah, aw);
        if (k == 0 || v > best) { best = v; arg = k; }
    }
    positive[((size_t)b * rows * cols + (size_t)ci * cols + cj) * A + arg] = 1;
}

struct LossArgs {
    const float* iou; const float* co; const float* sn; const float* logits;
    const float* best_iou; const int32_t* best_idx; const uint8_t* positive;
    const float* gt_min; const float* gt_max; const int64_t* gt_cls; const float* gt_onehot;
    const float* anchors;
    int B, n, N, A, C;
    float threshold;
};

__device__ __forceinline__ void slot_targets(const LossArgs& a, int b, int i, float& t_cy, float& t_cx, float& t_h, float& t_w, int& gi) {
    gi = a.best_idx[(size_t)b * a.n + i];
    const size_t o = ((size_t)b * a.N + gi) * 2;
    const float y0 = a.gt_min[o], x0 = a.gt_min[o + 1], y1 = a.gt_max[o], x1 = a.gt_max[o + 1];
    const float cy = (y0 + y1) / 2.f, cx = (x0 + x1) / 2.f;
    t_cy = cy - floorf(cy); t_cx = cx - floorf(cx);
    const int anc = i % a.A;
    t_h = logf((y1 - y0) / a.anchors[2 * anc]);
    t_w = logf((x1 - x0) / a.anchors[2 * anc + 1]);
}

__global__ __launch_bounds__(256) void loss_fwd_kernel(const LossArgs a, double* sums, float* blocksums) {
    __shared__ float part[6][4];
    const int b = blockIdx.y;
    const int i = blockIdx.x * 256 + threadIdx.x;
    float v[6] = {0, 0, 0, 0, 0, 0};
    if (i < a.n) {
        const size_t s = (size_t)b * a.n + i;
        const float p_iou = a.iou[s];
        const float bi = a.best_iou[s];
        const bool pos = a.positive[s] != 0;
        const bool neg = !pos && bi < a.threshold;
        if (neg) v[1] = p_iou * p_iou;
        if (pos) {
            float t_cy, t_cx, t_h, t_w; int gi;
            slot_targets(a, b, i, t_cy, t_cx, t_h, t_w, gi);
            const float d0 = p_iou - bi; v[0] = d0 * d0;
            const float dcy = a.co[2 * s] - t_cy, dcx = a.co[2 * s + 1] - t_cx; v[2] = dcy * dcy + dcx * dcx;
            const float dh = a.sn[2 * s] - t_h, dw = a.sn[2 * s + 1] - t_w; v[3] = dh * dh + dw * dw;
            v[5] = 1.f;
            if (a.C > 0) {
                const float* lg = a.logits + s * a.C;
                float mx = lg[0];
                for (int c = 1; c < a.C; ++c) mx = fmaxf(mx, lg[c]);
                float sum = 0.f;
                for (int c = 0; c < a.C; ++c) sum += expf(lg[c] - mx);
                if (a.gt_cls != nullptr) {
                    const int k = (int)a.gt_cls[(size_t)b * a.N + gi];
                    v[4] = -(lg[k] - mx - logf(sum));
                } else if (a.gt_onehot != nullptr) {
                    const float* oh = a.gt_onehot + ((size_t)b * a.N + gi) * a.C;
                    float acc = 0.f;
                    for (int c = 0; c < a.C; ++c) { const float d = expf(lg[c] - mx) / sum - oh[c]; acc += d * d; }
                    v[4] = acc;
                }
            }
        }
    }
    const int lane = threadIdx.x & 63, wave = threadIdx.x >> 6;
#pragma unroll
    for (int k = 0; k < 6; ++k) {
        float x = v[k];
#pragma unroll
        for (int off = 32; off > 0; off >>= 1) x += __shfl_xor(x, off);
        if (lane == 0) part[k][wave] = x;
    }
    __syncthreads();
    if (threadIdx.x < 6) {
        const float x = part[threadIdx.x][0] + part[threadIdx.x][1] + part[threadIdx.x][2] + part[threadIdx.x][3];
        if (blocksums != nullptr) blocksums[((size_t)blockIdx.y * gridDim.x + blockIdx.x) * 6 + threadIdx.x] = x;
        else if (x != 0.f) atomicAdd(sums + threadIdx.x, (double)x);
    }
}

__global__ void loss_finalize_kernel(const double* sums, double cnt, int ce, float* out) {
    const int k = threadIdx.x;
    if (k < 4) out[k] = (float)(sums[k] / cnt);
    else if (k == 4) out[4] = ce ? (float)(sums[4] / sums[5] / cnt) : (float)(sums[4] / cnt);
}

__global__ __launch_bounds__(256) void loss_bwd_kernel(const LossArgs a, const double* sums, double cnt, const float* __restrict__ w,
                                                       float* d_iou, float* d_co, float* d_sn, float* d_logits) {
    const int b = blockIdx.y;
    const int i = blockIdx.x * 256 + threadIdx.x;
    if (i >= a.n) return;
    const size_t s = (size_t)b * a.n + i;
    const float inv = (float)(1.0 / cnt);
    const float p_iou = a.iou[s];
    const float bi = a.best_iou[s];
    const bool pos = a.positive[s] != 0;
    const bool neg = !pos && bi < a.threshold;
    float g_iou = 0.f, g_cy = 0.f, g_cx = 0.f, g_h = 0.f, g_w = 0.f;
    if (neg) g_iou = w[1] * 2.f * p_iou * inv;
    int gi = 0;
    if (pos) {
        float t_cy, t_cx, t_h, t_w;
        slot_targets(a, b, i, t_cy, t_cx, t_h, t_w, gi);
        g_iou = w[0] * 2.f * (p_iou - bi) * inv;
        g_cy = w[2] * 2.f * (a.co[2 * s] - t_cy) * inv;
        g_cx = w[2] * 2.f * (a.co[2 * s + 1] - t_cx) * inv;
        g_h = w[3] * 2.f * (a.sn[2 * s] - t_h) * inv;
        g_w = w[3] * 2.f * (a.sn[2 * s + 1] - t_w) * inv;
    }
    d_iou[s] = g_iou;
    d_co[2 * s] = g_cy; d_co[2 * s + 1] = g_cx;
    d_sn[2 * s] = g_h; d_sn[2 * s + 1] = g_w;
    if (a.C > 0 && d_logits != nullptr) {
        float* dl = d_logits + s * a.C;
        if (!pos || (a.gt_cls == nullptr && a.gt_onehot == nullptr)) {
            for (int c = 0; c < a.C; ++c) dl[c] = 0.f;
        } else {
            const float* lg = a.logits + s * a.C;
            float mx = lg[0];
            for (int c = 1; c < a.C; ++c) mx = fmaxf(mx, lg[c]);
            float sum = 0.f;
            for (int c = 0; c < a.C; ++c) sum += expf(lg[c] - mx);
            if (a.gt_cls != nullptr) {
                const int k = (int)a.gt_cls[(size_t)b * a.N + gi];
                const float f = w[4] * inv / (float)sums[5];
                for (int c = 0; c < a.C; ++c) dl[c] = f * (expf(lg[c] - mx) / sum - (c == k ? 1.f : 0.f));
            } else {
                const float* oh = a.gt_onehot + ((size_t)b * a.N + gi) * a.C;
                const float f = w[4] * 2.f * inv;
                float dot = 0.f;
                for (int c = 0; c < a.C; ++c) { const float sm = expf(lg[c] - mx) / sum; dot += f * (sm - oh[c]) * sm; }
                for (int c = 0; c < a.C; ++c) { const float sm = expf(lg[c] - mx) / sum; dl[c] = sm * (f * (sm - oh[c]) - dot); }
            }
        }
    }
}

inline int act_grid(long long total, int Cg) {
    int g = 256, r = Cg;
    while (r) { const int t = g % r; g = r; r = t; }
    const int unit = Cg / g;
    long long want = (total + 256 * 8 - 1) / (256 * 8);
    const long long cap = (long long)Y2_NUM_CU * 8;
    if (want > cap) want = cap;
    if (want < 1) want = 1;
    return (int)(((want + unit - 1) / unit) * unit);
}

}

extern "C" int y2_bn_finalize(const double* stats, double count, const float* gamma, const float* beta,
                              float* running_mean, float* running_var, float momentum, float eps,
                              float* scale, float* shift, float* mean, float* invstd, int C, long long* num_batches_tracked, y2_stream_t stream) {
    if (!stats || !gamma || !beta || !scale || !shift || !mean || !invstd || C <= 0 || count <= 0) return Y2_EINVAL;
    Y2_LAUNCH("bn_finalize_kernel", 0.0, bn_finalize_kernel, dim3(y2_cdiv(C, 256)), dim3(256), 0, y2_s(stream), stats, count, gamma, beta, running_mean, running_var,
                       momentum, eps, scale, shift, mean, invstd, C, num_batches_tracked);
    Y2_LAUNCH_CHECK();
    return Y2_OK;
}

extern "C" int y2_bn_act_fwd_ex(const float* z, const float* scale, const float* shift, float slope, const float* residual, int ldr, float* y, float* y_pool,
                                int B, int H, int W, int C, int ldz, int ldy, int coff, int ldp, int poff, int out_mode, y2_stream_t stream) {
    if (!z || (!y && !y_pool) || B <= 0 || H <= 0 || W <= 0 || C <= 0) return Y2_EINVAL;
    const bool pool = y_pool != nullptr;
    if ((pool || out_mode == 1) && ((H & 1) || (W & 1))) return Y2_EINVAL;
    ActArgs a;
    a.z = z; a.scale = scale; a.shift = shift; a.y = y; a.y_pool = y_pool;
    a.B = B; a.H = H; a.W = W; a.C = C; a.ldz = ldz; a.ldy = ldy; a.coff = coff; a.ldp = ldp; a.poff = poff; a.out_mode = out_mode; a.slope = slope;
    a.res = residual; a.ldr = ldr;
    if (residual != nullptr && ldr < C) return Y2_EINVAL;
    const bool vec = (!residual || (!(ldr & 3) && y2_aligned16(residual))) && !(C & 3) && !(ldz & 3) && (!y || (!(ldy & 3) && !(coff & 3) && y2_aligned16(y))) && (!pool || (!(ldp & 3) && !(poff & 3) && y2_aligned16(y_pool))) && y2_aligned16(z);
    const long long pix = (long long)B * (pool ? H / 2 : H) * (pool ? W / 2 : W);
    if (pix >= 0x7fffffffLL || C > 8192) return Y2_ENOSUP;
    const long long total = pix * (vec ? C / 4 : C);
    const int grid = act_grid(total, vec ? C / 4 : C);
    a.d_wo = y2_make_fastdiv((uint32_t)(pool ? W / 2 : W)); a.d_ho = y2_make_fastdiv((uint32_t)(pool ? H / 2 : H));
    hipStream_t s = y2_s(stream);
    if (pool) { if (vec) Y2_LAUNCH("bn_act_fwd_kernel", 0.0, (bn_act_fwd_kernel<true, 4>), dim3(grid), dim3(256), 0, s, a, total); else Y2_LAUNCH("bn_act_fwd_kernel", 0.0, (bn_act_fwd_kernel<true, 1>), dim3(grid), dim3(256), 0, s, a, total); }
    else { if (vec) Y2_LAUNCH("bn_act_fwd_kernel", 0.0, (bn_act_fwd_kernel<false, 4>), dim3(grid), dim3(256), 0, s, a, total); else Y2_LAUNCH("bn_act_fwd_kernel", 0.0, (bn_act_fwd_kernel<false, 1>), dim3(grid), dim3(256), 0, s, a, total); }
    Y2_LAUNCH_CHECK();
    return Y2_OK;
}

static int bn_act_bwd_impl(const float* z, const float* scale, const float* shift, const float* mean, const float* invstd, const float* gamma,
                           float slope, const float* dy_full, int ldf, int foff, int fmode, const float* dy_pool, int ldp, int poff,
                           const float* dy_full2, int ld2, const float* residual, int ldr, float* dres, int lddr,
                           double* sums, float* dz, int ldd, int B, int H, int W, int C, int ldz, int has_bn, y2_stream_t stream, float* park, long long park_floats) {
    if (!z || (!dy_full && !dy_pool) || !sums || B <= 0 || H <= 0 || W <= 0 || C <= 0) return Y2_EINVAL;
    if (dz == nullptr && dres != nullptr) return Y2_EINVAL;
    if (has_bn < 0 || has_bn > 2 || (has_bn && (!mean || !invstd || !gamma))) return Y2_EINVAL;
    const bool pool = dy_pool != nullptr;
    if ((pool || fmode == 1) && ((H & 1) || (W & 1))) return Y2_EINVAL;
    if (C > 8192) return Y2_ENOSUP;
    ActBwdArgs a;
    a.z = z; a.scale = scale; a.shift = shift; a.mean = mean; a.invstd = invstd; a.gamma = gamma;
    a.dy_full = dy_full; a.dy_pool = dy_pool; a.sums = sums; a.dz = dz;
    a.B = B; a.H = H; a.W = W; a.C = C; a.ldz = ldz; a.ldf = ldf; a.foff = foff; a.fmode = fmode; a.ldp = ldp; a.poff = poff; a.ldd = ldd;
    a.slope = slope; a.n = (double)B * H * W; a.has_bn = has_bn;
    a.dy_full2 = dy_full2; a.ld2 = ld2; a.res = residual; a.ldr = ldr; a.dres = dres; a.lddr = lddr;
    const bool vec = (!dy_full2 || (!(ld2 & 3) && y2_aligned16(dy_full2))) && (!residual || (!(ldr & 3) && y2_aligned16(residual))) && (!dres || (!(lddr & 3) && y2_aligned16(dres))) && !(C & 3) && !(ldz & 3) && (!dz || (!(ldd & 3) && y2_aligned16(dz))) && y2_aligned16(z) &&
                     (!dy_full || (!(ldf & 3) && !(foff & 3) && y2_aligned16(dy_full))) && (!pool || (!(ldp & 3) && !(poff & 3) && y2_aligned16(dy_pool)));
    const int Cg = vec ? C / 4 : C;
    const long long pix = (long long)B * (pool ? H / 2 : H) * (pool ? W / 2 : W);
    if (pix >= 0x7fffffffLL) return Y2_ENOSUP;
    const long long total = pix * Cg;
    const int grid = act_grid(total, Cg);
    a.d_wo = y2_make_fastdiv((uint32_t)(pool ? W / 2 : W)); a.d_ho = y2_make_fastdiv((uint32_t)(pool ? H / 2 : H));
    const size_t lds = (size_t)2 * C * sizeof(float);
    hipStream_t s = y2_s(stream);
    a.partial = nullptr;
    const long long npix = (long long)B * H * W;
    auto overlaps = [&](const float* p, long long floats) {
        if (p == nullptr) return false;
        const char* lo = (const char*)dz; const char* hi = lo + (size_t)npix * ldd * sizeof(float);
        const char* q = (const char*)p;
        return q < hi && lo < q + (size_t)floats * sizeof(float);
    };
    const long long opix = pix;
    const bool aliased = dz != nullptr && (overlaps(z, npix * ldz) || overlaps(dy_full, (fmode == 1 ? npix / 4 : npix) * (long long)ldf) || overlaps(dy_pool, opix * ldp) ||
                                           overlaps(dy_full2, npix * ld2) || overlaps(residual, npix * ldr) || overlaps(dres, npix * lddr));
    a.block_partial = (dz != nullptr && !aliased && !y2_det.on && ldd == C && grid > 16 && (long long)grid * 2 * C <= npix * ldd) ? dz : nullptr;
    if (dz == nullptr && park != nullptr && !y2_det.on && grid > 16 && (long long)grid * 2 * C <= park_floats && y2_aligned16(park)) a.block_partial = park;
    const long long prow = (long long)grid * 256 / Cg;
    if (y2_det.on) {
        if ((size_t)prow * 2 * C * sizeof(float) > y2_det.bytes || prow > 0x7fffffffLL) return Y2_EINVAL;
        a.partial = y2_det.ws;
    }
#define Y2_BWD(POOL, CV)                                                                                             \
    do {                                                                                                             \
        Y2_LAUNCH("bn_act_bwd_kernel", 0.0, (bn_act_bwd_kernel<POOL, CV, false>), dim3(grid), dim3(256), lds, s, a, total);            \
        if (a.partial != nullptr) {                                                                                  \
            const int rc_ = y2_det_reduce_f32(a.partial, (int)prow, (long long)2 * C, (long long)2 * C, sums, nullptr, s);            \
            if (rc_ != Y2_OK) return rc_;                                                                            \
        }                                                                                                            \
        if (a.block_partial != nullptr)                                                                              \
            Y2_LAUNCH("bn_bwd_block_reduce_kernel", 0.0, bn_bwd_block_reduce_kernel, dim3((unsigned)y2_cdiv(2 * C, 64), (unsigned)(grid >= 512 ? 16 : (grid >= 64 ? 4 : 1))), dim3(1024), 0, s, a.block_partial, grid, 2 * C, sums);            \
        if (dz != nullptr) Y2_LAUNCH("bn_act_bwd_kernel", 0.0, (bn_act_bwd_kernel<POOL, CV, true>), dim3(grid), dim3(256), 0, s, a, total);               \
    } while (0)
    if (pool) { if (vec) Y2_BWD(true, 4); else Y2_BWD(true, 1); }
    else { if (vec) Y2_BWD(false, 4); else Y2_BWD(false, 1); }
#undef Y2_BWD
    Y2_LAUNCH_CHECK();
    return Y2_OK;
}

extern "C" int y2_bn_act_bwd_ex(const float* z, const float* scale, const float* shift, const float* mean, const float* invstd, const float* gamma,
                                float slope, const float* dy_full, int ldf, int foff, int fmode, const float* dy_pool, int ldp, int poff,
                                const float* dy_full2, int ld2, const float* residual, int ldr, float* dres, int lddr,
                                double* sums, float* dz, int ldd, int B, int H, int W, int C, int ldz, int has_bn, y2_stream_t stream) {
    return bn_act_bwd_impl(z, scale, shift, mean, invstd, gamma, slope, dy_full, ldf, foff, fmode, dy_pool, ldp, poff, dy_full2, ld2, residual, ldr, dres, lddr,
                           sums, dz, ldd, B, H, W, C, ldz, has_bn, stream, nullptr, 0);
}

extern "C" long long y2_wino6_tiles(int32_t B, int32_t H, int32_t W) {
    if (B <= 0 || H <= 0 || W <= 0) return Y2_EINVAL;
    return wino6_grid(B, H, W).T;
}

extern "C" int y2_bn_act_bwd_wino6(const float* z, const float* scale, const float* shift, const float* mean, const float* invstd, const float* gamma,
                                   float slope, const float* dy_full, int ldf, int foff, double* sums, float* v6, float* m6, float* dz, int ldd,
                                   int B, int H, int W, int C, int ldz, int has_bn, y2_stream_t stream) {
    if (!z || !dy_full || !sums || (v6 == nullptr && m6 == nullptr) || B <= 0 || H <= 0 || W <= 0 || C <= 0 || ldz < C || ldf < foff + C) return Y2_EINVAL;
    if (dz != nullptr && ldd < C) return Y2_EINVAL;
    if (y2_det.on) return Y2_ENOSUP;
    const Wino6Grid g6 = wino6_grid(B, H, W);
    if (g6.T * C >= 0xffffffffLL || g6.T > 0x7fffffff || (long long)B * H * W >= 0x7fffffffLL) return Y2_ENOSUP;
    float* park = v6 != nullptr ? v6 : m6;
    if (const int rc = bn_act_bwd_impl(z, scale, shift, mean, invstd, gamma, slope, dy_full, ldf, foff, 0, nullptr, 0, 0, nullptr, 0, nullptr, 0, nullptr, 0,
                                       sums, nullptr, 0, B, H, W, C, ldz, has_bn, stream, park, 36LL * g6.T * C)) return rc;
    BnWino6Args a;
    a.z = z; a.scale = scale; a.shift = shift; a.mean = mean; a.invstd = invstd; a.gamma = gamma; a.dy = dy_full; a.sums = sums;
    a.v6 = v6; a.m6 = m6; a.dz = dz; a.ldd = ldd;
    a.B = B; a.H = H; a.W = W; a.C = C; a.ldz = ldz; a.ldf = ldf; a.foff = foff; a.has_bn = has_bn; a.slope = slope; a.n = (double)B * H * W;
    a.th = g6.th; a.tw = g6.tw; a.T = (int)g6.T; a.tall = g6.tall; a.wide = g6.wide; a.gx = g6.gx;
    a.d_c = y2_make_fastdiv((uint32_t)C); a.d_tt = y2_make_fastdiv((uint32_t)(g6.th * g6.tw)); a.d_tw = y2_make_fastdiv((uint32_t)g6.tw);
    a.d_tall = y2_make_fastdiv((uint32_t)(g6.tall > 0 ? g6.tall : 1)); a.d_wide = y2_make_fastdiv((uint32_t)(g6.wide > 0 ? g6.wide : 1));
    Y2_LAUNCH("bn_bwd_wino6_kernel", 0.0, bn_bwd_wino6_kernel, dim3((unsigned)y2_cdiv(g6.T * C, 256)), dim3(256), 0, y2_s(stream), a);
    Y2_LAUNCH_CHECK();
    return Y2_OK;
}

extern "C" int y2_bn_act_fwd(const float* z, const float* scale, const float* shift, float slope, float* y, float* y_pool,
                             int B, int H, int W, int C, int ldz, int ldy, int coff, int ldp, int poff, int out_mode, y2_stream_t stream) {
    return y2_bn_act_fwd_ex(z, scale, shift, slope, nullptr, 0, y, y_pool, B, H, W, C, ldz, ldy, coff, ldp, poff, out_mode, stream);
}

extern "C" int y2_bn_act_bwd(const float* z, const float* scale, const float* shift, const float* mean, const float* invstd, const float* gamma,
                             float slope, const float* dy_full, int ldf, int foff, int fmode, const float* dy_pool, int ldp, int poff,
                             double* sums, float* dz, int ldd, int B, int H, int W, int C, int ldz, int has_bn, y2_stream_t stream) {
    return y2_bn_act_bwd_ex(z, scale, shift, mean, invstd, gamma, slope, dy_full, ldf, foff, fmode, dy_pool, ldp, poff, nullptr, 0, nullptr, 0, nullptr, 0,
                            sums, dz, ldd, B, H, W, C, ldz, has_bn, stream);
}

extern "C" int y2_colsum(const float* x, long long M, int C, int ld, double* out, y2_stream_t stream) {
    if (!x || !out || M <= 0 || C <= 0 || ld < C || C > 16384) return Y2_EINVAL;
    int g = 256, r = C;
    while (r) { const int t = g % r; g = r; r = t; }
    const int unit = C / g;
    long long want = (M * C + 256 * 16 - 1) / (256 * 16);
    const long long cap = (long long)Y2_NUM_CU * 4;
    if (want > cap) want = cap;
    if (want < 1) want = 1;
    const int grid = (int)(((want + unit - 1) / unit) * unit);
    Y2_LAUNCH("colsum_kernel", 0.0, colsum_kernel, dim3(grid), dim3(256), (size_t)C * sizeof(float), y2_s(stream), x, M, C, ld, out);
    Y2_LAUNCH_CHECK();
    return Y2_OK;
}

extern "C" int y2_f64_to_f32(const double* src, float* dst, int n, double mul, y2_stream_t stream) {
    if (!src || !dst || n <= 0) return Y2_EINVAL;
    Y2_LAUNCH("f64_to_f32_kernel", 0.0, f64_to_f32_kernel, dim3(y2_cdiv(n, 256)), dim3(256), 0, y2_s(stream), src, dst, n, mul);
    Y2_LAUNCH_CHECK();
    return Y2_OK;
}

extern "C" int y2_decode_bwd(const float* iou, const float* center_offset, const float* d_iou, const float* d_center_offset, const float* d_size_norm,
                             const float* d_logits, float* d_feature, int boxes, int C, y2_stream_t stream) {
    if (!iou || !center_offset || !d_feature || boxes <= 0 || C < 0) return Y2_EINVAL;
    const long long total = (long long)boxes * (5 + C);
    Y2_LAUNCH("decode_bwd_kernel", 0.0, decode_bwd_kernel, dim3(stream_grid(total, 256)), dim3(256), 0, y2_s(stream), iou, center_offset, d_iou, d_center_offset, d_size_norm, d_logits,
                       d_feature, boxes, C);
    Y2_LAUNCH_CHECK();
    return Y2_OK;
}

extern "C" int y2_region_loss_fwd(const float* iou, const float* center_offset, const float* size_norm, const float* logits,
                                  const float* yx_min, const float* yx_max,
                                  const float* gt_yx_min, const float* gt_yx_max, const int64_t* gt_cls, const float* gt_onehot,
                                  const float* anchors, int B, int rows, int cols, int A, int C, int N, float threshold,
                                  float* best_iou, int32_t* best_idx, uint8_t* positive, double* sums, float* loss_out, y2_stream_t stream) {
    if (!iou || !center_offset || !size_norm || !yx_min || !yx_max || !gt_yx_min || !gt_yx_max || !anchors) return Y2_EINVAL;
    if (!best_iou || !best_idx || !positive || !sums || !loss_out) return Y2_EINVAL;
    if (B <= 0 || rows <= 0 || cols <= 0 || A <= 0 || C < 0 || N <= 0) return Y2_EINVAL;
    if (C > 0 && !logits) return Y2_EINVAL;
    const int n = rows * cols * A;
    hipStream_t s = y2_s(stream);
    Y2_LAUNCH("loss_match_kernel", 0.0, loss_match_kernel, dim3(y2_cdiv(n, 256), B), dim3(256), 0, s, yx_min, yx_max, gt_yx_min, gt_yx_max, n, N, best_iou, best_idx, positive, sums);
    Y2_LAUNCH("loss_positive_kernel", 0.0, loss_positive_kernel, dim3(y2_cdiv((long long)B * N, 256)), dim3(256), 0, s, gt_yx_min, gt_yx_max, anchors, B, N, rows, cols, A, positive);
    LossArgs a;
    a.iou = iou; a.co = center_offset; a.sn = size_norm; a.logits = logits; a.best_iou = best_iou; a.best_idx = best_idx; a.positive = positive;
    a.gt_min = gt_yx_min; a.gt_max = gt_yx_max; a.gt_cls = gt_cls; a.gt_onehot = gt_onehot; a.anchors = anchors;
    a.B = B; a.n = n; a.N = N; a.A = A; a.C = C; a.threshold = threshold;
    float* blocksums = nullptr;
    const long long nblk = (long long)y2_cdiv(n, 256) * B;
    if (y2_det.on) {
        if ((size_t)nblk * 6 * sizeof(float) > y2_det.bytes) return Y2_EINVAL;
        blocksums = y2_det.ws;
    }
    Y2_LAUNCH("loss_fwd_kernel", 0.0, loss_fwd_kernel, dim3(y2_cdiv(n, 256), B), dim3(256), 0, s, a, sums, blocksums);
    if (blocksums != nullptr) {
        const int rc = y2_det_reduce_f32(blocksums, (int)nblk, 6, 6, sums, nullptr, s);
        if (rc != Y2_OK) return rc;
    }
    Y2_LAUNCH("loss_finalize_kernel", 0.0, loss_finalize_kernel, dim3(1), dim3(64), 0, s, sums, (double)B * n, gt_cls != nullptr ? 1 : 0, loss_out);
    Y2_LAUNCH_CHECK();
    return Y2_OK;
}

extern "C" int y2_region_loss_bwd(const float* iou, const float* center_offset, const float* size_norm, const float* logits,
                                  const float* gt_yx_min, const float* gt_yx_max, const int64_t* gt_cls, const float* gt_onehot,
                                  const float* anchors, int B, int rows, int cols, int A, int C, int N, float threshold,
                                  const float* best_iou, const int32_t* best_idx, const uint8_t* positive, const double* sums, const float* weights,
                                  float* d_iou, float* d_center_offset, float* d_size_norm, float* d_logits, y2_stream_t stream) {
    if (!iou || !center_offset || !size_norm || !gt_yx_min || !gt_yx_max || !anchors || !best_iou || !best_idx || !positive || !sums || !weights) return Y2_EINVAL;
    if (!d_iou || !d_center_offset || !d_size_norm) return Y2_EINVAL;
    const int n = rows * cols * A;
    LossArgs a;
    a.iou = iou; a.co = center_offset; a.sn = size_norm; a.logits = logits; a.best_iou = best_iou; a.best_idx = best_idx; a.positive = positive;
    a.gt_min = gt_yx_min; a.gt_max = gt_yx_max; a.gt_cls = gt_cls; a.gt_onehot = gt_onehot; a.anchors = anchors;
    a.B = B; a.n = n; a.N = N; a.A = A; a.C = C; a.threshold = threshold;
    Y2_LAUNCH("loss_bwd_kernel", 0.0, loss_bwd_kernel, dim3(y2_cdiv(n, 256), B), dim3(256), 0, y2_s(stream), a, sums, (double)B * n, weights, d_iou, d_center_offset, d_size_norm, d_logits);
    Y2_LAUNCH_CHECK();
    return Y2_OK;
}

extern "C" int y2_region_loss_finalize(const double* sums, double cnt, int cross_entropy, float* loss_out, y2_stream_t stream) {
    if (!sums || !loss_out || cnt <= 0) return Y2_EINVAL;
    Y2_LAUNCH("loss_finalize_kernel", 0.0, loss_finalize_kernel, dim3(1), dim3(64), 0, y2_s(stream), sums, cnt, cross_entropy, loss_out);
    Y2_LAUNCH_CHECK();
    return Y2_OK;
}

extern "C" int y2_maxpool_bwd(const float* x, const float* dy, const float* dy2, float* dx, int B, int H, int W, int C, int ldx, int ldy, int lddx,
                              int ksize, int stride, int pad, int pad_end, y2_stream_t stream) {
    if (!x || !dy || !dx || B <= 0 || H <= 0 || W <= 0 || C <= 0 || ksize <= 0 || stride <= 0 || pad < 0 || pad_end < 0) return Y2_EINVAL;
    const int Ho = (H + pad + pad_end - ksize) / stride + 1, Wo = (W + pad + pad_end - ksize) / stride + 1;
    if (Ho <= 0 || Wo <= 0) return Y2_EINVAL;
    const long long total = (long long)B * H * W * C;
    const bool aligned = !(C & 3) && !(ldx & 3) && !(ldy & 3) && !(lddx & 3) && y2_aligned16(x) && y2_aligned16(dy) && y2_aligned16(dx) && (!dy2 || y2_aligned16(dy2));
    static const bool tiled_env = getenv("Y2_POOL_BWD_TILED") == nullptr || atoi(getenv("Y2_POOL_BWD_TILED")) != 0;
    if (tiled_env && aligned && ksize == 3 && stride == 2 && pad == 1 && !(C % MP_CH) && (long long)B * (C / MP_CH) < 65535 && (long long)H * W * ldx < 0x7fffffffLL) {
        const dim3 grid((unsigned)y2_cdiv(W, MP_TW), (unsigned)y2_cdiv(H, MP_TH), (unsigned)(B * (C / MP_CH)));
        Y2_LAUNCH("maxpool_bwd_kernel", 0.0, maxpool3s2_bwd_kernel, grid, dim3(256), 0, y2_s(stream), x, dy, dy2, dx, H, W, Ho, Wo, C / MP_CH, ldx, ldy, lddx);
        Y2_LAUNCH_CHECK();
        return Y2_OK;
    }
    if (!(C & 3) && !(ldx & 3) && !(ldy & 3) && !(lddx & 3) && y2_aligned16(x) && y2_aligned16(dy) && y2_aligned16(dx) && (!dy2 || y2_aligned16(dy2)) && (long long)B * H < 65535
        && (long long)H * W * ldx < 0x7fffffffLL) {
        const int per_row = W * (C / 4);
        Y2_LAUNCH("maxpool_bwd_kernel", 0.0, maxpool_bwd4_kernel, dim3((per_row + 255) / 256, B * H), dim3(256), 0, y2_s(stream), x, dy, dy2, dx, H, W, Ho, Wo, C / 4, ldx, ldy, lddx, ksize, stride, pad);
        Y2_LAUNCH_CHECK();
        return Y2_OK;
    }
    Y2_LAUNCH("maxpool_bwd_kernel", 0.0, maxpool_bwd_kernel, dim3(stream_grid(total, 256)), dim3(256), 0, y2_s(stream), x, dy, dy2, dx, H, W, Ho, Wo, C, ldx, ldy, lddx, ksize, stride, pad, total);
    Y2_LAUNCH_CHECK();
    return Y2_OK;
}
```

### yolo2-pytorch_amd/model/train_graph.py

```python
import collections
import ctypes
import os

import numpy as np
import torch
import torch.distributed as dist

import _hip
from model import train_oplist
from model._train_parts import BN_MOMENTUM, LEAKY, GradSink, StatsArena, _new, bn_params, cached_buf, prep_weights

BWD_STREAMS = int(os.environ.get('Y2_BWD_STREAMS', '2'))
_SIDE = {}


def _side_stream(dev):
    s = _SIDE.get(str(dev))
    if s is None:
        s = torch.cuda.Stream(device=dev)
        _SIDE[str(dev)] = s
    return s


GRAPH_FORK = {'1': True, '0': False}.get(os.environ.get('Y2_GRAPH_FORK', 'auto'), 'auto')
GRAD_F43 = os.environ.get('Y2_GRAD_F43', '1') != '0'
FUSE_WINO6 = os.environ.get('Y2_FUSE_WINO6', '1') != '0'
FUSE_CONV0 = os.environ.get('Y2_FUSE_CONV0', '1') != '0'
DEBUG_TAP = None

SYNC_POSITIVES = True

DP_TAG = '_y2_dp_reduce'


def _sum_over_ranks(t, reducer):
    return bool(reducer(t)) if reducer is not None else False


_WINO_CHUNK_BYTES = int(os.environ.get('Y2_WINO_CHUNK_MB', '4096')) << 20


OperandPruned = _hip.OperandMissing


def _problem(B, H, W, cin, ldx, cout, k, ldy, coff=0, ldp=0, out_mode=0, slope=1.0):
    p = _hip.ConvParams()
    p.x = p.y = 256
    p.B, p.H, p.W, p.Cin, p.ldx, p.Cout, p.ksize = B, H, W, cin, ldx, cout, k
    p.ldy, p.coff, p.ldp, p.poff, p.out_mode = ldy, coff, ldp, 0, out_mode
    p.slope, p.tile = slope, 0
    return p


def _f43_offered(eligible, cin, H, W):
    return bool(GRAD_F43 and eligible and cin >= 128 and H * W <= 52 * 52)


def _conv(L, st, x, wp, y, B, H, W, cin, ldx, cout, k, ldy, scale=None, shift=None, slope=1.0, stats=None, y_pool=None, ldp=0, coff=0, out_mode=0, keep_v=False, u=False,
          us=None, us_plane=0, grad=False, note=None, u_eligible=None, u6=None, choice=None, pre=None, problem=None):
    p = problem if problem is not None else _problem(B, H, W, cin, ldx, cout, k, ldy, coff, ldp, out_mode, slope)
    p.x, p.w = (x.data_ptr() if x is not None else 256), (wp.data_ptr() if wp is not None else None)
    for field, t in (('scale', scale), ('shift', shift), ('y', y), ('y_pool', y_pool), ('stats', stats)):
        setattr(p, field, t.data_ptr() if t is not None else None)
    if u is False:
        u = _hip.wino_weight(wp, cout, cin) if (out_mode == 0 and _hip.wino_eligible(cout, cin, k)) else None
    elif out_mode != 0:
        u = None
    def f43_operand():
        if u6 is not None:
            return u6
        if wp is None:
            raise OperandPruned('the 4x4-tile data-gradient operand is derived from a packed weight this step did not prepare')
        return _hip.wino6_weight(wp, cout, cin)
    eligible = (u is not None) if u_eligible is None else (bool(u_eligible) and out_mode == 0)
    dev = (x if x is not None else pre).device
    _hip.autotune_conv(p, dev, wino_w=u, implicit_ok=not keep_v, wino_split=us if u is not None else None, split_plane=us_plane,
                       f43=f43_operand if (grad and _f43_offered(eligible, cin, H, W)) else None, wino_eligible=eligible, choice=choice)
    if pre is not None:
        assert p.algo == 6, p.algo
        p.algo, p.x, p.ldx = 7, pre.data_ptr(), cin
    if wp is None and (p.algo == 0 or (p.algo in (6, 7) and u6 is None)):
        raise OperandPruned('algorithm %d reads the packed weight, which this step did not prepare' % p.algo)
    if note is not None:
        note('w' if p.algo == 0 else '6' if p.algo in (6, 7) else 'u')
    kept = None
    if keep_v and p.algo in (1, 2):
        T = B * ((H + 1) // 2) * ((W + 1) // 2)
        if 16 * T * (cin + cout) * 4 <= _WINO_CHUNK_BYTES and 16 * T * cin * 4 < 0x7fffffff:
            need = L.y2_conv_fwd_workspace_bytes(ctypes.byref(p))
            kept = torch.empty(need // 4 + 4, dtype=torch.float32, device=x.device)
            p.workspace, p.workspace_bytes = kept.data_ptr(), kept.numel() * 4
    if kept is None:
        _hip.conv_workspace(p, dev)
    _hip.check(L.y2_conv_fwd(ctypes.byref(p), st), 'y2_conv_fwd')
    return kept


class _Block(object):
    __slots__ = ('mod', 'name', 'x', 'ldx', 'H', 'W', 'cin', 'cout', 'k', 'z', 'scale', 'shift', 'mean', 'invstd', 'pool',
                 'out_full', 'out_pool', 'out_ld', 'out_off', 'out_mode', 'has_bn', 'slope', 'first', 'wino_v', 'eff')


PRUNE_OPERANDS = os.environ.get('Y2_PRUNE_OPERANDS', '1') != '0'


def _train_operands(dnn, dev, scope=None, only=None, alloc_only=False):
    from model import yolo2 as _yolo2
    if _hip.split_mode() or scope is None:
        only = None
    key = (dev, dnn._weight_versions(), _hip.split_mode(), _hip.WINOGRAD)
    if scope is not None:
        bufs = (dev, scope)
    else:
        cache = getattr(dnn, '_train_cache', None)
        if cache is not None and cache[0] == key:
            return cache[1]
        bufs = getattr(dnn, '_train_bufs', None)
        if bufs is None or bufs[0] != dev:
            bufs = (dev, {})
            dnn._train_bufs = bufs

    def buf(tag, n):
        return cached_buf(bufs[1], tag, n, dev)
    first = dnn._first_block()
    items, ops = [], {}
    wino = []
    for name, blk in dnn.named_modules():
        if not isinstance(blk, _yolo2.Conv2d) or blk is first:
            continue
        w = blk.conv.weight.detach()
        cout, cin, k, _ = w.shape
        if cout % 4 or cin % 4 or not w.is_contiguous() or w.dtype != torch.float32:
            continue
        n = w.numel()
        want = lambda tag: only is None or (blk, tag) in only
        d = dict(name=name, wp=buf((name, 'wp'), n) if want('wp') else None, wd=buf((name, 'wd'), n) if want('wd') else None, uf=None, ud=None, ufs=None, uds=None, plane=0,
                 uf_ok=bool(_hip.wino_eligible(cout, cin, k)), ud_ok=bool(_hip.wino_eligible(cin, cout, k)))
        if d['wp'] is not None:
            items.append((w, d['wp'], cout, cin, k, _hip.PREP_FPROP))
        if d['wd'] is not None:
            items.append((w, d['wd'], cout, cin, k, _hip.PREP_DGRAD))
        if _hip.wino_eligible(cout, cin, k) and want('uf'):
            wino.append((d, 'uf', w, cout, cin, k, _hip.PREP_WINO_FPROP))
        if _hip.wino_eligible(cin, cout, k) and want('ud'):
            wino.append((d, 'ud', w, cout, cin, k, _hip.PREP_WINO_DGRAD))
        d['u6d'] = None
        if only is not None and (blk, 'u6d') in only and d['ud_ok']:
            d['u6d'] = buf((name, 'u6d'), 36 * cout * cin)
            items.append((w, d['u6d'], cout, cin, k, _hip.PREP_WINO6_DGRAD))
        ops[blk] = d
    usize = sum(16 * cout * cin for _, _, _, cout, cin, _, _ in wino)
    if usize:
        if only is None:
            arena = buf('u_arena', usize)
        off = 0
        for d, tag, w, cout, cin, k, mode in wino:
            d[tag] = arena[off:off + 16 * cout * cin] if only is None else buf((d['name'], tag), 16 * cout * cin)
            items.append((w, d[tag], cout, cin, k, mode))
            off += 16 * cout * cin
    if alloc_only:
        return ops
    prep_weights(items)
    if usize and _hip.split_mode():
        f16 = _hip.split_mode() == 'f16'
        np_, dt = (2, torch.float16) if f16 else (3, torch.bfloat16)
        planes = bufs[1].get('u_split')
        if planes is None or planes.numel() != np_ * usize or planes.dtype != dt:
            planes = bufs[1]['u_split'] = torch.empty(np_ * usize, dtype=dt, device=dev)
        if f16:
            _hip.check(_hip.lib().y2_split_f16x2(_hip.ptr(arena), _hip.ptr(planes), usize, _hip.F16_U_SCALE, _hip.stream()), 'y2_split_f16x2')
        else:
            _hip.check(_hip.lib().y2_split_bf16x3(_hip.ptr(arena), _hip.ptr(planes), usize, _hip.stream()), 'y2_split_bf16x3')
        off = 0
        for d, tag, w, cout, cin, k, mode in wino:
            if (cout if tag == 'ud' else cin) % 32 == 0:
                d[tag + 's'] = planes[off:off + 16 * cout * cin]
            d['plane'] = usize
            off += 16 * cout * cin
    if scope is None:
        dnn._train_cache = (key, ops)
    return ops


def darknet_forward(dnn, x):
    params = [p for p in dnn.parameters()]
    out = DarknetTrainFn.apply(dnn, x, *params)
    return out.permute(0, 3, 1, 2)


def darknet_forward_eval_grad(dnn, x):
    params = [p for p in dnn.parameters()]
    out = DarknetEvalGradFn.apply(dnn, x, *params)
    return out.permute(0, 3, 1, 2)


class _Eff(object):
    __slots__ = ('w', 'gamma', 'beta', 'rm', 'rv', 'bias', 'cout', 'cin', 'cout_r', 'cin_r', 'in_idx', 'padded')


def _pad_layout(dnn):
    b1, b2, b3 = dnn._blocks()
    up = lambda c: (c + 3) // 4 * 4
    mods = [m for _, m, _ in b1 + b2 + b3] + [dnn.passthrough]
    head = b3[-1][1]
    if all(m.conv.weight.shape[0] % 4 == 0 or m is head for m in mods) and all(m.conv.weight.shape[1] % 4 == 0 for m in mods[1:]):
        return None
    lay = {}
    prev = None
    for i, (_, m, _) in enumerate(b1):
        cout, cin = m.conv.weight.shape[:2]
        lay[m] = (up(cout), cin if i == 0 else prev, None)
        prev = up(cout)
    route = prev
    m = dnn.passthrough
    c_pt = m.conv.weight.shape[0]
    lay[m] = (up(c_pt), route, None)
    for _, m, _ in b2:
        lay[m] = (up(m.conv.weight.shape[0]), prev, None)
        prev = up(m.conv.weight.shape[0])
    c_l2 = b2[-1][1].conv.weight.shape[0]
    idx = [q * up(c_pt) + c for q in range(4) for c in range(c_pt)] + [4 * up(c_pt) + c for c in range(c_l2)]
    m = b3[0][1]
    lay[m] = (up(m.conv.weight.shape[0]), 4 * up(c_pt) + up(c_l2), idx)
    lay[head] = (head.conv.weight.shape[0], up(m.conv.weight.shape[0]), None)
    return lay


def _effective(dnn, dev, frozen):
    lay = _pad_layout(dnn)
    out = {}
    for m in dnn.modules():
        if not hasattr(m, 'conv') or not hasattr(m, 'has_act'):
            continue
        e = _Eff()
        w = m.conv.weight.detach()
        cout, cin = w.shape[:2]
        e.cout_r, e.cin_r = cout, cin
        e.cout, e.cin, e.in_idx = (cout, cin, None) if lay is None else lay[m]
        e.padded = (e.cout, e.cin) != (cout, cin)
        bn = m.bn
        if not e.padded:
            e.w = _hip.f32c(w)
            e.gamma, e.beta = (bn.weight.detach(), bn.bias.detach()) if bn is not None else (None, None)
            e.rm, e.rv = (bn.running_mean, bn.running_var) if bn is not None else (None, None)
            e.bias = _hip.f32c(m.conv.bias.detach()) if m.conv.bias is not None else None
        else:
            k = w.shape[2]
            e.w = torch.zeros(e.cout, e.cin, k, k, dtype=torch.float32, device=dev)
            if e.in_idx is None:
                e.w[:cout, :cin] = w
            else:
                e.w[:cout].index_copy_(1, torch.tensor(e.in_idx, dtype=torch.long, device=dev), _hip.f32c(w))
            pad = lambda t, fill: torch.cat([_hip.f32c(t.detach()), torch.full((e.cout - cout,), fill, dtype=torch.float32, device=dev)])
            e.gamma, e.beta = (pad(bn.weight, 1.0), pad(bn.bias, 0.0)) if bn is not None else (None, None)
            e.rm, e.rv = (pad(bn.running_mean, 0.0), pad(bn.running_var, 1.0)) if bn is not None else (None, None)
            e.bias = pad(m.conv.bias, 0.0) if m.conv.bias is not None else None
        out[m] = e
    return out


def _darknet_fwd(ctx, dnn, x, params, frozen, scope=None):
    _hip.require_gpu(x)
    L = _hip.lib()
    st = _hip.stream()
    x = _hip.f32c(x.detach())
    B, cin0, H, W = x.shape
    if H % 32 or W % 32:
        raise ValueError('input size must be a multiple of 32 (got %dx%d)' % (H, W))
    dev = x.device
    b1, b2, b3 = dnn._blocks()
    eff = _effective(dnn, dev, frozen)
    used = ctx.used = set()
    prepared = _train_operands(dnn, dev, (getattr(ctx, 'ops_scope', None) or scope) if scope is not None else None, only=getattr(ctx, 'only', None)) if not any(e.padded for e in eff.values()) else {}
    arena = StatsArena(dev, sum(e.cout for e in eff.values()), frozen)
    blocks = []
    written = []

    def keep_v(h, w, cin, ldx, cout, k):
        if k != 3:
            return False
        with_v, without_v = (_hip.wgrad_choice(B, h, w, cin, ldx, cout, cout, k, hv, dev) for hv in (True, False))
        return not (with_v in (0, 2) or (with_v is None and without_v in (0, 2)))

    def run_block(name, mod, xin, ldx, h, w, pool, out_full=None, out_ld=0, out_off=0, out_mode=0, want_full=True, first=False):
        blk = _Block()
        e = eff[mod]
        L.y2_prof_set_tag(1 + len(blocks))
        cout, cin, k = e.cout, e.cin, mod.kernel_size
        blk.mod, blk.name, blk.x, blk.ldx, blk.H, blk.W, blk.cin, blk.cout, blk.k = mod, name, xin, ldx, h, w, cin, cout, k
        blk.pool, blk.has_bn, blk.slope, blk.first = pool, mod.bn is not None, (LEAKY if mod.has_act else 1.0), first
        blk.wino_v = None
        blk.eff = e
        z = _new(dev, B, h, w, cout)
        stats = arena.take(cout) if (blk.has_bn and not frozen) else None
        estats = arena.epilogue(stats)
        if first:
            _hip.check(L.y2_conv0_fwd(_hip.ptr(xin), _hip.ptr(e.w), None, None, _hip.ptr(z), None, _hip.ptr(estats),
                                      B, h, w, cin, cout, cout, 0, 1.0, st), 'y2_conv0_fwd')
        elif mod in prepared:
            blk.wino_v = _conv(L, st, xin, prepared[mod]['wp'], z, B, h, w, cin, ldx, cout, k, cout, stats=estats, keep_v=keep_v(h, w, cin, ldx, cout, k), u=prepared[mod]['uf'],
                               us=prepared[mod]['ufs'], us_plane=prepared[mod]['plane'], note=lambda kind, m=mod: used.add((m, 'uf' if kind == 'u' else 'wp')), u_eligible=prepared[mod]['uf_ok'])
        else:
            wp = _new(dev, e.w.numel())
            _hip.check(L.y2_pack_weight(_hip.ptr(e.w), _hip.ptr(wp), cout, cin, k, 0, st), 'y2_pack_weight')
            blk.wino_v = _conv(L, st, xin, wp, z, B, h, w, cin, ldx, cout, k, cout, stats=estats, keep_v=keep_v(h, w, cin, ldx, cout, k))
        arena.settle(stats, z, B * h * w, cout, cout)
        blk.z = z
        if blk.has_bn:
            bn = mod.bn
            blk.scale, blk.shift, blk.mean, blk.invstd = bn_params(L, st, dev, bn, stats, B * h * w, cout, frozen, BN_MOMENTUM, tensors=(e.gamma, e.beta, e.rm, e.rv))
            if not frozen and e.padded and bn.running_mean is not None:
                bn.running_mean.copy_(e.rm[:e.cout_r])
                bn.running_var.copy_(e.rv[:e.cout_r])
                written.extend(t for t in (bn.num_batches_tracked,) if t is not None)
            elif not frozen:
                written.extend(t for t in (bn.running_mean, bn.running_var, bn.num_batches_tracked) if t is not None)
        else:
            blk.scale, blk.mean, blk.invstd = None, None, None
            blk.shift = e.bias
        y_full = y_pool = None
        if out_full is not None:
            y_full = out_full
        elif want_full:
            y_full, out_ld, out_off = _new(dev, B, h, w, cout), cout, 0
        if pool:
            y_pool = _new(dev, B, h // 2, w // 2, cout)
        _hip.check(L.y2_bn_act_fwd(_hip.ptr(z), _hip.ptr(blk.scale), _hip.ptr(blk.shift), blk.slope, _hip.ptr(y_full), _hip.ptr(y_pool),
                                   B, h, w, cout, cout, out_ld, out_off, cout, 0, out_mode, st), 'y2_bn_act_fwd')
        blk.out_full, blk.out_pool, blk.out_ld, blk.out_off, blk.out_mode = y_full, y_pool, out_ld, out_off, out_mode
        blocks.append(blk)
        return blk, y_full, y_pool

    cur, ld, h, w = x, cin0, H, W
    full_last = None
    for i, (name, mod, pool) in enumerate(b1):
        last = i == len(b1) - 1
        pool = pool or last
        blk, yf, yp = run_block(name, mod, cur, ld, h, w, pool, want_full=(not pool) or last, first=(i == 0))
        if last:
            full_last, fh, fw = yf, h, w
        if pool:
            cur, h, w = yp, h // 2, w // 2
        else:
            cur = yf
        ld = blk.cout
    c_pt = eff[dnn.passthrough].cout
    c_l2 = eff[b2[-1][1]].cout
    cat = _new(dev, B, h, w, 4 * c_pt + c_l2)
    run_block('passthrough', dnn.passthrough, full_last, full_last.shape[-1], fh, fw, False, out_full=cat, out_ld=cat.shape[-1], out_off=0, out_mode=1)
    for i, (name, mod, pool) in enumerate(b2):
        if i == len(b2) - 1:
            blk, yf, yp = run_block(name, mod, cur, ld, h, w, False, out_full=cat, out_ld=cat.shape[-1], out_off=4 * c_pt)
        else:
            blk, yf, yp = run_block(name, mod, cur, ld, h, w, False)
            cur, ld = yf, blk.cout
    cur, ld = cat, cat.shape[-1]
    for i, (name, mod, pool) in enumerate(b3):
        blk, yf, yp = run_block(name, mod, cur, ld, h, w, False)
        cur, ld = yf, blk.cout
    if written:
        _hip.wrote(written)
    ctx.dnn = dnn
    ctx.blocks = blocks
    ctx.prepared = prepared
    ctx.prepared_key = dnn._train_cache[0] if (prepared and scope is None) else None
    ctx.scope = scope
    ctx.geom = (B, cin0, H, W, c_pt, c_l2)
    ctx.x = x
    ctx.frozen = frozen
    ctx.param_ids = [id(p) for p in params]
    L.y2_prof_set_tag(0)
    return cur


_Geo = collections.namedtuple('_Geo', 'H W cin cout k ldx first has_v padded ud_ok full pooled')
_Plan = collections.namedtuple('_Plan', 'wgrad zero final fuse0 fused6 problem')


def _routes(names, pools, n1, c_pt):
    idx = {name: i for i, name in enumerate(names)}
    out, full, pooled = [[] for _ in names], [None] * (len(names) - 1) + [0], [False] * len(names)
    for i, name in enumerate(names[1:], 1):
        if name == 'layers3.0':
            out[i] = [(idx['passthrough'], False, 0, 1), (i - 1, False, 4 * c_pt, 0)]
        elif name == 'passthrough':
            out[i] = [(n1 - 1, False, 0, 0)]
        elif i == n1 + 1:
            out[i] = [(n1 - 1, True, 0, 0)]
        else:
            out[i] = [(i - 1, pools[i - 1], 0, 0)]
    for j, is_pool, _, mode in sum(out, []):
        if is_pool:
            pooled[j] = True
        else:
            full[j] = mode
    return out, full, pooled


def _decide_bwd(geo, B, dev, need_dx=False):
    plans = []
    for g in geo:
        cop = (g.cout + 3) // 4 * 4
        if g.first:
            small = g.cin <= 3 and g.cout <= 64
            fuse0 = bool(FUSE_CONV0 and small and g.full is None and g.pooled and not (g.H & 1) and not (g.W & 15) and B * g.H * g.W * g.cout * 4 < 0xffff0000 and not need_dx)
            plans.append(_Plan(0, small, small, fuse0, None, None))
            continue
        wgrad = _hip.wgrad_choice(B, g.H, g.W, g.cin, g.ldx, cop, cop, g.k, g.has_v, dev)
        fused6 = problem = None
        if (FUSE_WINO6 and wgrad == 2 and g.k == 3 and g.ud_ok is not None and not g.pooled and g.full == 0 and cop == g.cout and not g.padded
                and DEBUG_TAP is None and not _hip.DETERMINISTIC and not _hip.split_mode()):
            problem = _problem(B, g.H, g.W, cop, cop, g.cin, g.k, g.cin)
            hit = _hip.autotune_conv(problem, dev, f43=True if _f43_offered(g.ud_ok, cop, g.H, g.W) else None, wino_eligible=g.ud_ok, peek=True)
            fused6 = tuple(hit) if (hit is not None and hit[0] == 6) else None
        plans.append(_Plan(wgrad, wgrad == 0, g.k == 1 and cop == g.cout and not g.padded, False, fused6, problem if fused6 else None))
    return plans


def _darknet_bwd(ctx, dout):
    L = _hip.lib()
    st = _hip.stream()
    dnn, blocks = ctx.dnn, ctx.blocks
    scope = getattr(ctx, 'scope', None)
    if ctx.prepared and scope is None and (getattr(dnn, '_train_cache', (None, None))[0] != ctx.prepared_key or ctx.prepared_key[:2] != (dout.device, dnn._weight_versions())):
        raise RuntimeError('model.yolo2: a convolution weight was modified (optimizer step, load_state_dict, in-place edit) between this forward and '
                           'its backward; the per-model GEMM operand buffers this graph was recorded against hold other weights now')
    B, cin0, H, W, c_pt, c_l2 = ctx.geom
    dev = dout.device
    dout = _hip.f32c(dout)
    sink = GradSink(dnn, dev)
    ready, dest, grads = sink.ready, sink.dest, sink.grads

    n = len(blocks)
    src_full, src_pool = [None] * (n - 1) + [(dout, blocks[n - 1].cout, 0, 0)], [None] * n
    routes, full, pooled = _routes([b.name for b in blocks], [b.pool for b in blocks], len(dnn._blocks()[0]), c_pt)
    need_dx = bool(getattr(ctx, 'need_dx', False))
    plans = _decide_bwd([_Geo(b.H, b.W, b.cin, b.cout, b.k, b.ldx, b.first, b.wino_v is not None, b.eff.padded,
                              ctx.prepared[b.mod]['ud_ok'] if (not b.first and b.mod in ctx.prepared) else None, full[i], pooled[i]) for i, b in enumerate(blocks)], B, str(dev), need_dx)
    order = list(range(n - 1, -1, -1))
    main = torch.cuda.current_stream(dev)
    side = _side_stream(dev) if (BWD_STREAMS > 1 and not _hip.DETERMINISTIC and (not torch.cuda.is_current_stream_capturing() or getattr(ctx, 'fork_ok', False))) else None
    late = []

    def join():
        for item in late:
            if item[2] is not None:
                main.wait_event(item[2])
                item[2] = None
    ctx.join = join
    affine_grads = []

    sums_arena = torch.empty(2 * sum(b.cout for b in blocks), dtype=torch.float64, device=dev)
    zero = [sums_arena]
    bufs = (dev, scope) if scope is not None else dnn.__dict__.setdefault('_train_bufs', (dev, {}))
    if bufs[0] != dev:
        bufs = dnn._train_bufs = (dev, {})
    wg, dzs = {}, {}
    for i in order:
        blk, plan = blocks[i], plans[i]
        cop = (blk.cout + 3) // 4 * 4
        weight = blk.mod.conv.weight
        if cop != blk.cout:
            dzs[i] = _new(dev, B, blk.H, blk.W, cop)
            zero.append(dzs[i])
        if blk.first:
            if plan.final:
                wg[i] = dest(weight) if not blk.eff.padded else _new(dev, blk.cout, blk.cin, 3, 3)
        elif blk.k == 1:
            wg[i] = dest(weight).view(-1) if plan.final else _new(dev, cop * blk.cin)
        else:
            wg[i] = cached_buf(bufs[1], (blk.name, 'dwp'), cop * blk.cin * blk.k * blk.k, dev)
        if plan.zero:
            zero.append(wg[i])
    _hip.multi([(_hip.MULTI_ZERO, t, None) for t in zero], st)
    sums_used = 0

    def flush_weight_grads(keep=0):
        while len(late) > keep:
            prm, g, evt, held = late.pop(0)
            if evt is not None:
                main.wait_event(evt)
            del held
            ready(prm, g)
    for i in order:
        blk, plan = blocks[i], plans[i]
        e = blk.eff
        L.y2_prof_set_tag(101 + i)
        h, w, cout, cin, k = blk.H, blk.W, blk.cout, blk.cin, blk.k
        sums = sums_arena[sums_used:sums_used + 2 * cout]
        sums_used += 2 * cout
        cop = (cout + 3) // 4 * 4
        sf, sp = src_full[i], src_pool[i]
        fuse0, fused6 = plan.fuse0, None
        if plan.fused6:
            T6 = int(L.y2_wino6_tiles(B, h, w))
            fused6 = (_new(dev, 36 * T6 * cout), _new(dev, 36 * T6 * cout))
        dz = None if (fuse0 or fused6) else (dzs[i] if i in dzs else _new(dev, B, h, w, cop))
        if DEBUG_TAP is not None:
            DEBUG_TAP(blk.name + ':in', blk.z, blk.shift, sf, sp)
        if fused6:
            _hip.check(L.y2_bn_act_bwd_wino6(_hip.ptr(blk.z), _hip.ptr(blk.scale), _hip.ptr(blk.shift), _hip.ptr(blk.mean), _hip.ptr(blk.invstd),
                                             _hip.ptr(e.gamma) if blk.has_bn else None, blk.slope, _hip.ptr(sf[0]), sf[1], sf[2], _hip.ptr(sums),
                                             _hip.ptr(fused6[0]), _hip.ptr(fused6[1]), None, 0, B, h, w, cout, cout,
                                             (2 if ctx.frozen else 1) if blk.has_bn else 0, st), 'y2_bn_act_bwd_wino6')
        else:
            _hip.check(L.y2_bn_act_bwd(_hip.ptr(blk.z), _hip.ptr(blk.scale), _hip.ptr(blk.shift), _hip.ptr(blk.mean), _hip.ptr(blk.invstd),
                                       _hip.ptr(e.gamma) if blk.has_bn else None, blk.slope,
                                       _hip.ptr(sf[0]) if sf else None, sf[1] if sf else 0, sf[2] if sf else 0, sf[3] if sf else 0,
                                       _hip.ptr(sp), cout, 0, _hip.ptr(sums), _hip.ptr(dz), cop, B, h, w, cout, cout,
                                       (2 if ctx.frozen else 1) if blk.has_bn else 0, st), 'y2_bn_act_bwd')
        if blk.has_bn:
            affine_grads.append((blk.mod.bn.bias, sums_used - 2 * cout, e.cout_r))
            affine_grads.append((blk.mod.bn.weight, sums_used - cout, e.cout_r))
        elif blk.mod.conv.bias is not None:
            affine_grads.append((blk.mod.conv.bias, sums_used - 2 * cout, e.cout_r))
        weight = blk.mod.conv.weight

        def real(dw):
            if not e.padded and cop == cout:
                return dw
            dw = dw[:e.cout_r]
            if e.cin != e.cin_r:
                dw = dw.index_select(1, torch.tensor(e.in_idx, dtype=torch.long, device=dev)) if e.in_idx is not None else dw[:, :e.cin_r].contiguous()
            return dw

        def weight_grad(st_w):
            if blk.first and fuse0:
                _hip.check(L.y2_conv0_wgrad_fused(_hip.ptr(ctx.x), _hip.ptr(blk.z), _hip.ptr(blk.scale), _hip.ptr(blk.shift), _hip.ptr(blk.mean), _hip.ptr(blk.invstd),
                                                  _hip.ptr(e.gamma) if blk.has_bn else None, blk.slope, _hip.ptr(sp), cout, _hip.ptr(sums), _hip.ptr(wg[i]),
                                                  B, h, w, cin, cout, cout, (2 if ctx.frozen else 1) if blk.has_bn else 0, st_w), 'y2_conv0_wgrad_fused')
                return real(wg[i])
            if blk.first and plan.final:
                _hip.check(L.y2_conv0_wgrad(_hip.ptr(ctx.x), _hip.ptr(dz), _hip.ptr(wg[i]), B, h, w, cin, cout, cop, st_w), 'y2_conv0_wgrad')
                return real(wg[i])
            if blk.first:
                x4 = torch.zeros(B, h, w, 4, dtype=torch.float32, device=dev)
                x4[..., :cin] = ctx.x.permute(0, 2, 3, 1)
                dwp = torch.zeros(cop * k * k * 4, dtype=torch.float32, device=dev)
                _hip.check(L.y2_conv_wgrad(_hip.ptr(x4), _hip.ptr(dz), _hip.ptr(dwp), B, h, w, 4, 4, cop, cop, k, st_w), 'y2_conv_wgrad')
                dw4 = _new(dev, cop, 4, k, k)
                _hip.check(L.y2_unpack_weight_grad(_hip.ptr(dwp), _hip.ptr(dw4), cop, 4, k, st_w), 'y2_unpack_weight_grad')
                return dw4[:e.cout_r, :cin].contiguous()
            tgt = wg[i]
            if plan.wgrad is None:
                _hip.multi([(_hip.MULTI_ZERO, tgt, None)], st_w)
            dw = None
            if k == 3:
                dw = dest(weight) if (cop == cout and not e.padded) else _new(dev, cop, cin, k, k)
            got = _hip.conv_wgrad(blk.x, fused6[1] if fused6 else dz, B, h, w, cin, blk.ldx, cop, cop, k, v=blk.wino_v, out=tgt, zeroed=plan.zero or plan.wgrad is None,
                                  native=dw, dz_pre=bool(fused6), choice=plan.wgrad)
            if plan.final:
                return tgt.view(cout, cin, 1, 1)
            if k == 1:
                return real(tgt.view(cop, cin, 1, 1))
            if got is not dw:
                _hip.check(L.y2_unpack_weight_grad(_hip.ptr(tgt), _hip.ptr(dw), cop, cin, k, st_w), 'y2_unpack_weight_grad')
            return real(dw)

        if side is not None and not e.padded and (not blk.first or plan.final):
            ev = torch.cuda.Event()
            ev.record(main)
            with _hip.launch_on(side):
                side.wait_event(ev)
                gw = weight_grad(_hip.stream())
                done = torch.cuda.Event()
                done.record(side)
            held = (dz, blk.x, blk.wino_v, ctx.x) + ((blk.z, sp) if fuse0 else ()) + ((fused6[1],) if fused6 else ())
            flush_weight_grads(keep=1)
            late.append([weight, gw, done, held])
        else:
            ready(weight, weight_grad(st))
        blk.wino_v = None
        if blk.first and need_dx:
            cin4 = (cin + 3) // 4 * 4
            wpad = torch.zeros(cop, cin4, k, k, dtype=torch.float32, device=dev)
            wpad[:cout, :cin] = e.w
            wd = _new(dev, wpad.numel())
            _hip.check(L.y2_pack_weight(_hip.ptr(wpad), _hip.ptr(wd), cop, cin4, k, 1, st), 'y2_pack_weight')
            dx4 = _new(dev, B, h, w, cin4)
            _conv(L, st, dz, wd, dx4, B, h, w, cop, cop, cin4, k, cin4)
            ctx_dx = dx4[..., :cin].permute(0, 3, 1, 2).contiguous()
            grads['__x__'] = ctx_dx
        if not blk.first:
            dx = _new(dev, B, h, w, cin)
            ready_ops = ctx.prepared.get(blk.mod)
            if ready_ops is not None:
                dg_split = ready_ops['uds'] if _hip.split_mode() == 'bf16' else None
                _conv(L, st, dz, ready_ops['wd'], dx, B, h, w, cop, cop, cin, k, cin, u=ready_ops['ud'], us=dg_split, us_plane=ready_ops['plane'], grad=True,
                      note=lambda kind, m=blk.mod: ctx.used.add((m, 'wd' if kind == 'w' else 'u6d' if kind == '6' else 'ud')), u_eligible=ready_ops['ud_ok'], u6=ready_ops.get('u6d'),
                      choice=plan.fused6, pre=fused6[0] if fused6 else None, problem=plan.problem)
            else:
                wsrc = e.w
                if cop != cout:
                    wpad = bufs[1].get((blk.name, 'wpad'))
                    if wpad is None or wpad.shape != (cop, cin, k, k):
                        wpad = bufs[1][(blk.name, 'wpad')] = torch.zeros(cop, cin, k, k, dtype=torch.float32, device=dev)
                    _hip.multi([(_hip.MULTI_COPY, wpad[:cout], wsrc)], st)
                    wsrc = wpad
                wd = _new(dev, wsrc.numel())
                _hip.check(L.y2_pack_weight(_hip.ptr(wsrc), _hip.ptr(wd), cop, cin, k, 1, st), 'y2_pack_weight')
                _conv(L, st, dz, wd, dx, B, h, w, cop, cop, cin, k, cin)
            if DEBUG_TAP is not None and dz is not None:
                DEBUG_TAP(blk.name, dz, dx, None, None)
            for j, to_pool, off, mode in routes[i]:
                if to_pool:
                    src_pool[j] = dx
                else:
                    src_full[j] = (dx, cin, off, mode)
        blk.z = None
    sink.hand_affine(sums_arena, affine_grads, st)
    flush_weight_grads()
    L.y2_prof_set_tag(0)
    out = [None, grads.get('__x__')]
    for pid in ctx.param_ids:
        out.append(grads.get(pid))
    ctx.blocks = None
    ctx.prepared = None
    ctx.join = None
    return tuple(out)


class DarknetTrainFn(torch.autograd.Function):
    @staticmethod
    def forward(ctx, dnn, x, *params):
        ctx.need_dx = x.requires_grad
        return _darknet_fwd(ctx, dnn, x, params, frozen=False)

    @staticmethod
    def backward(ctx, dout):
        return _darknet_bwd(ctx, dout)


class _Tape(object):
    need_dx = False
    saved_tensors = ()

    def save_for_backward(self, *tensors):
        self.saved_tensors = tensors

    def mark_non_differentiable(self, *tensors):
        pass

    def set_materialize_grads(self, value):
        pass


class DarknetEvalGradFn(torch.autograd.Function):
    @staticmethod
    def forward(ctx, dnn, x, *params):
        ctx.need_dx = x.requires_grad
        ctx.dnn, ctx.x, ctx.params = dnn, x.detach(), params
        ctx.key = dnn._versions()
        return dnn.forward_nhwc(x.detach())

    @staticmethod
    def backward(ctx, dout):
        if ctx.dnn._versions() != ctx.key:
            raise RuntimeError('model.yolo2: parameters or buffers were modified between an eval-mode forward and its backward')
        tape = _Tape()
        tape.need_dx = ctx.need_dx
        _darknet_fwd(tape, ctx.dnn, ctx.x, ctx.params, frozen=True)
        return _darknet_bwd(tape, dout)


class DecodeFn(torch.autograd.Function):

    @staticmethod
    def forward(ctx, feature_nhwc, anchors_dev, A):
        L = _hip.lib()
        f = _hip.f32c(feature_nhwc.detach())
        B, rows, cols, ch = f.shape
        E = ch // A
        C = E - 5
        cells = rows * cols
        dev = f.device
        iou = _new(dev, B, cells, A)
        co, sn, mn, mx = (_new(dev, B, cells, A, 2) for _ in range(4))
        _hip.check(L.y2_decode(_hip.ptr(f), _hip.ptr(anchors_dev), B, rows, cols, A, C, _hip.ptr(iou), _hip.ptr(co), _hip.ptr(sn), _hip.ptr(mn), _hip.ptr(mx),
                               None, None, None, _hip.stream()), 'y2_decode')
        logits = f.view(B, cells, A, E)[..., 5:].contiguous() if C > 0 else torch.empty(0, device=dev)
        ctx.save_for_backward(iou, co)
        ctx.shape = (B, rows, cols, A, C)
        ctx.mark_non_differentiable(mn, mx)
        ctx.set_materialize_grads(False)
        return iou, co, sn, mn, mx, logits

    @staticmethod
    def backward(ctx, d_iou, d_co, d_sn, d_mn, d_mx, d_logits):
        L = _hip.lib()
        iou, co = ctx.saved_tensors
        B, rows, cols, A, C = ctx.shape
        dev = iou.device
        df = _new(dev, B, rows, cols, A * (5 + C))
        c = lambda t: _hip.f32c(t) if t is not None else None
        if d_iou is None:
            d_iou = torch.zeros_like(iou)
        if d_co is None:
            d_co = torch.zeros_like(co)
        if d_sn is None:
            d_sn = torch.zeros_like(co)
        d_iou, d_co, d_sn = c(d_iou), c(d_co), c(d_sn)
        d_logits = c(d_logits) if (C > 0 and d_logits is not None) else None
        _hip.check(L.y2_decode_bwd(_hip.ptr(iou), _hip.ptr(co), _hip.ptr(d_iou), _hip.ptr(d_co), _hip.ptr(d_sn), _hip.ptr(d_logits),
                                   _hip.ptr(df), B * rows * cols * A, C, _hip.stream()), 'y2_decode_bwd')
        return df, None, None


def inference_forward(inference, feature):
    import model
    A = inference.anchors.size(0)
    _feature = feature.permute(0, 2, 3, 1).contiguous()
    anchors = model._device_anchors(inference.anchors, _feature.device)
    iou, co, sn, mn, mx, logits = DecodeFn.apply(_feature, anchors, A)
    return feature, iou, co, sn, mn, mx, (logits if logits.numel() else None)


class RegionLossFn(torch.autograd.Function):
    @staticmethod
    def forward(ctx, iou, co, sn, logits, yx_min, yx_max, gt_min, gt_max, gt_cls, anchors_dev, rows, cols, threshold, reducer=None):
        L = _hip.lib()
        dev = iou.device
        B, cells, A = iou.shape
        n = cells * A
        iou, co, sn, yx_min, yx_max = (_hip.f32c(t.detach()) for t in (iou, co, sn, yx_min, yx_max))
        C = 0 if logits is None else logits.shape[-1]
        lg = _hip.f32c(logits.detach()) if C else None
        gt_min, gt_max = _hip.f32c(gt_min), _hip.f32c(gt_max)
        N = gt_min.shape[1]
        cls_i = cls_oh = None
        if C:
            if gt_cls.dim() > 2:
                cls_oh = _hip.f32c(gt_cls)
            else:
                cls_i = gt_cls.to(torch.int64).contiguous()
        best_iou = _new(dev, B, cells, A)
        best_idx = torch.empty(B, cells, A, dtype=torch.int32, device=dev)
        positive = torch.empty(B, cells, A, dtype=torch.uint8, device=dev)
        sums = torch.empty(6, dtype=torch.float64, device=dev)
        out = _new(dev, 5)
        _hip.check(L.y2_region_loss_fwd(_hip.ptr(iou), _hip.ptr(co), _hip.ptr(sn), _hip.ptr(lg), _hip.ptr(yx_min), _hip.ptr(yx_max),
                                        _hip.ptr(gt_min), _hip.ptr(gt_max), _hip.ptr(cls_i), _hip.ptr(cls_oh), _hip.ptr(anchors_dev),
                                        B, rows, cols, A, C, N, float(threshold), _hip.ptr(best_iou), _hip.ptr(best_idx), _hip.ptr(positive),
                                        _hip.ptr(sums), _hip.ptr(out), _hip.stream()), 'y2_region_loss_fwd')
        if SYNC_POSITIVES and cls_i is not None:
            npos = sums[5:6]
            if _sum_over_ranks(npos, reducer):
                _hip.check(L.y2_region_loss_finalize(_hip.ptr(sums), float(B * n), 1, _hip.ptr(out), _hip.stream()), 'y2_region_loss_finalize')
        ctx.saved = (iou, co, sn, lg, gt_min, gt_max, cls_i, cls_oh, anchors_dev, best_iou, best_idx, positive, sums)
        ctx.geom = (B, rows, cols, A, C, N, float(threshold))
        ctx.mark_non_differentiable(best_iou, best_idx, positive)
        ctx.set_materialize_grads(False)
        return out, best_iou, best_idx, positive

    @staticmethod
    def backward(ctx, d_out, *_):
        L = _hip.lib()
        iou, co, sn, lg, gt_min, gt_max, cls_i, cls_oh, anchors_dev, best_iou, best_idx, positive, sums = ctx.saved
        B, rows, cols, A, C, N, thr = ctx.geom
        dev = iou.device
        if d_out is None:
            return (None,) * 14
        w = _hip.f32c(d_out)
        d_iou = torch.empty_like(iou)
        d_co, d_sn = torch.empty_like(co), torch.empty_like(sn)
        d_lg = torch.empty_like(lg) if C else None
        _hip.check(L.y2_region_loss_bwd(_hip.ptr(iou), _hip.ptr(co), _hip.ptr(sn), _hip.ptr(lg), _hip.ptr(gt_min), _hip.ptr(gt_max),
                                        _hip.ptr(cls_i), _hip.ptr(cls_oh), _hip.ptr(anchors_dev), B, rows, cols, A, C, N, thr,
                                        _hip.ptr(best_iou), _hip.ptr(best_idx), _hip.ptr(positive), _hip.ptr(sums), _hip.ptr(w),
                                        _hip.ptr(d_iou), _hip.ptr(d_co), _hip.ptr(d_sn), _hip.ptr(d_lg), _hip.stream()), 'y2_region_loss_bwd')
        return (d_iou, d_co, d_sn, d_lg) + (None,) * 10


class LossDict(dict):
    vector = None


class _LazyDebug(object):

    def __init__(self, makers):
        self._makers, self._values = makers, {}

    def __getitem__(self, key):
        if key not in self._values:
            self._values[key] = self._makers[key]()
        return self._values[key]

    def __contains__(self, key):
        return key in self._makers

    def __iter__(self):
        return iter(self._makers)

    def __len__(self):
        return len(self._makers)

    def keys(self):
        return self._makers.keys()

    def items(self):
        return [(k, self[k]) for k in self._makers]

    def get(self, key, default=None):
        return self[key] if key in self._makers else default


def loss(anchors, data, pred, threshold):
    import model
    iou = pred['iou']
    _hip.require_gpu(iou)
    rows, cols = pred['feature'].size()[-2:]
    anchors_dev = model._device_anchors(anchors, iou.device)
    logits = pred.get('logits')
    dev = iou.device
    gt_min, gt_max, gt_cls = (data[k].to(dev) for k in ('yx_min', 'yx_max', 'cls'))
    out, best_iou, best_idx, positive = RegionLossFn.apply(iou, pred['center_offset'], pred['size_norm'], logits, pred['yx_min'], pred['yx_max'],
                                                           gt_min, gt_max, gt_cls, anchors_dev, rows, cols, threshold,
                                                           getattr(pred['feature'], DP_TAG, None))
    result = LossDict(foreground=out[0:1], background=out[1:2], center=out[2:3], size=out[3:4])
    if logits is not None:
        result['cls'] = out[4:5]
    result.vector = out

    def matched():
        B = iou.shape[0]
        flat = best_idx.view(B, -1).long()
        _data = {}
        for key, t in (('yx_min', gt_min), ('yx_max', gt_max), ('cls', gt_cls)):
            if t.dim() == 2:
                _data[key] = torch.gather(t, 1, flat).view(*best_idx.shape)
            else:
                _data[key] = torch.gather(t, 1, flat.unsqueeze(-1).expand(-1, -1, t.shape[-1])).view(*best_idx.shape, -1)
        return _data
    debug = _LazyDebug(dict(iou=lambda: best_iou, data=matched, positive=lambda: positive.bool(),
                            negative=lambda: ~positive.bool() & (best_iou < threshold)))
    return result, debug


_HPARAM_DEV = {}


class _WeightedTotalFn(torch.autograd.Function):
    @staticmethod
    def forward(ctx, vector, weights):
        total = torch.empty(1, dtype=torch.float32, device=vector.device)
        _hip.check(_hip.lib().y2_small_dot(_hip.ptr(vector), _hip.ptr(weights), vector.numel(), _hip.ptr(total), _hip.stream()), 'y2_small_dot')
        ctx.weights = weights
        return total

    @staticmethod
    def backward(ctx, g):
        out = torch.empty_like(ctx.weights)
        _hip.check(_hip.lib().y2_small_scale(_hip.ptr(_hip.f32c(g)), _hip.ptr(ctx.weights), out.numel(), _hip.ptr(out), _hip.stream()), 'y2_small_scale')
        return out, None


def weighted_total(loss_, hparam):
    vec = getattr(loss_, 'vector', None)
    keys = list(loss_)
    if vec is None or not vec.is_cuda or keys != ['foreground', 'background', 'center', 'size', 'cls'][:len(keys)]:
        return sum(loss_[key] * hparam[key] for key in loss_)
    w = tuple(float(hparam[k]) for k in keys) + (0.0,) * (vec.numel() - len(keys))
    key = (w, str(vec.device))
    wd = _HPARAM_DEV.get(key)
    if wd is None:
        if len(_HPARAM_DEV) > 64:
            _HPARAM_DEV.clear()
        wd = _HPARAM_DEV[key] = torch.tensor(w, dtype=torch.float32, device=vec.device)
    return _WeightedTotalFn.apply(vec, wd)


class _Segments(object):

    def __init__(self, pool, mode):
        self.pool, self.mode = pool, mode
        self.ops, self.graph, self.mark = [], None, 0
        self.held = []

    def begin(self):
        self.graph = torch.cuda.CUDAGraph()
        self.graph.capture_begin(pool=self.pool, capture_error_mode='thread_local')
        self.mark = _hip.LAUNCHES[0]

    def cut(self, op, maybe_foreign=False):
        if _hip.LAUNCHES[0] == self.mark and maybe_foreign:
            t = torch.empty(4, dtype=torch.float32, device=torch.device('cuda', torch.cuda.current_device()))
            self.held.append(t)
            _hip.multi([(_hip.MULTI_ZERO, t, None)])
        if _hip.LAUNCHES[0] != self.mark:
            self.graph.capture_end()
            self.ops.append(('graph', self.graph))
            self.ops.append(op)
            self.begin()
        else:
            self.ops.append(op)

    def end(self):
        self.graph.capture_end()
        if _hip.LAUNCHES[0] != self.mark:
            self.ops.append(('graph', self.graph))
        self.graph = None

    def abort(self, fork=None):
        if self.graph is not None:
            try:
                if fork is not None:
                    with torch.cuda.stream(fork):
                        forked = torch.cuda.is_current_stream_capturing()
                    if forked:
                        torch.cuda.current_stream().wait_stream(fork)
                self.graph.capture_end()
            except Exception:
                pass
# ... 309 lines not shown
```

Before: 2252 images/sec.

## Record pre-activation of max-pool winners to fuse pooled BN+act forward and backward

For BN+leaky+maxpool blocks whose full output is not consumed, the forward pass now saves the raw conv value that wins each 2x2 pool window into a quarter-size z_sel buffer. The backward pass reads this buffer instead of recomputing the pool argmax over the full tensor. For the first conv, the conv0 kernel picks the winner before BN by using the sign of gamma, since the BN affine plus leaky ReLU is monotone in z with direction set by gamma's sign. The following BN+act then runs only on the pooled quarter-size tensor. This adds an extra buffer per pooled block and new kernel variants, and the gamma-sign selection relies on that monotonicity, which breaks if invstd/scale or slope behave unexpectedly.

Measured after the change: 2293 images/sec, median of 6. +1.8%, better.

```diff
diff --git a/include/yolo2_hip.h b/include/yolo2_hip.h
--- a/include/yolo2_hip.h
+++ b/include/yolo2_hip.h
@@ -122,6 +122,8 @@
 int y2_conv0_fwd(const float* x_nchw, const float* w, const float* scale, const float* shift,
                  float* y, float* y_pool, double* stats,
                  int B, int H, int W, int Cin, int Cout, int ldy, int ldp, float slope, y2_stream_t stream);
+int y2_conv0_fwd_sel(const float* x_nchw, const float* w, const float* gamma, float* z, float* z_sel, double* stats,
+                     int B, int H, int W, int Cin, int Cout, int ldz, int ldzs, y2_stream_t stream);
 
 int y2_maxpool2_fwd(const float* x, float* y, int B, int H, int W, int C, int ldx, int ldy, y2_stream_t stream);
 
@@ -246,6 +248,12 @@
                      const float* dy_full2, int ld2, const float* residual, int ldr, float* dres, int lddr,
                      double* sums, float* dz, int ldd, int B, int H, int W, int C, int ldz, int has_bn, y2_stream_t stream);
 
+int y2_bn_act_fwd_sel(const float* z, const float* scale, const float* shift, float slope, float* y_pool, float* z_sel,
+                      int B, int H, int W, int C, int ldz, int ldp, int poff, int ldzs, y2_stream_t stream);
+int y2_bn_act_bwd_sel(const float* z, const float* z_sel, int ldzs, const float* scale, const float* shift, const float* mean, const float* invstd,
+                      const float* gamma, float slope, const float* dy_pool, int ldp, int poff, double* sums, float* dz, int ldd,
+                      int B, int H, int W, int C, int ldz, y2_stream_t stream);
+
 long long y2_wino6_tiles(int32_t B, int32_t H, int32_t W);
 int y2_bn_act_bwd_wino6(const float* z, const float* scale, const float* shift, const float* mean, const float* invstd, const float* gamma,
                         float slope, const float* dy_full, int ldf, int foff, double* sums, float* v6, float* m6, float* dz, int ldd,
diff --git a/yolo2-pytorch_amd/_hip.py b/yolo2-pytorch_amd/_hip.py
--- a/yolo2-pytorch_amd/_hip.py
+++ b/yolo2-pytorch_amd/_hip.py
@@ -83,6 +83,7 @@
     'y2_conv_fwd_batch': [ctypes.POINTER(ConvParams), c_int, c_void_p],
     'y2_conv0_fwd': [c_void_p, c_void_p, c_void_p, c_void_p, c_void_p, c_void_p, c_void_p,
                      c_int, c_int, c_int, c_int, c_int, c_int, c_int, c_float, c_void_p],
+    'y2_conv0_fwd_sel': [c_void_p, c_void_p, c_void_p, c_void_p, c_void_p, c_void_p, c_int, c_int, c_int, c_int, c_int, c_int, c_int, c_void_p],
     'y2_maxpool2_fwd': [c_void_p, c_void_p, c_int, c_int, c_int, c_int, c_int, c_int, c_void_p],
     'y2_maxpool_fwd': [c_void_p, c_void_p, c_int, c_int, c_int, c_int, c_int, c_int, c_int, c_int, c_int, c_int, c_void_p],
     'y2_nchw_to_nhwc': [c_void_p, c_void_p, c_int, c_int, c_int, c_int, c_int, c_void_p],
@@ -103,6 +104,9 @@
     'y2_bn_act_bwd_ex': [c_void_p, c_void_p, c_void_p, c_void_p, c_void_p, c_void_p, c_float, c_void_p, c_int, c_int, c_int, c_void_p, c_int, c_int,
                          c_void_p, c_int, c_void_p, c_int, c_void_p, c_int,
                          c_void_p, c_void_p, c_int, c_int, c_int, c_int, c_int, c_int, c_int, c_void_p],
+    'y2_bn_act_fwd_sel': [c_void_p, c_void_p, c_void_p, c_float, c_void_p, c_void_p, c_int, c_int, c_int, c_int, c_int, c_int, c_int, c_int, c_void_p],
+    'y2_bn_act_bwd_sel': [c_void_p, c_void_p, c_int, c_void_p, c_void_p, c_void_p, c_void_p, c_void_p, c_float, c_void_p, c_int, c_int, c_void_p, c_void_p, c_int,
+                          c_int, c_int, c_int, c_int, c_int, c_void_p],
     'y2_wino6_tiles': [c_int, c_int, c_int],
     'y2_bn_act_bwd_wino6': [c_void_p, c_void_p, c_void_p, c_void_p, c_void_p, c_void_p, c_float, c_void_p, c_int, c_int, c_void_p, c_void_p, c_void_p, c_void_p, c_int,
                             c_int, c_int, c_int, c_int, c_int, c_int, c_void_p],
diff --git a/yolo2-pytorch_amd/csrc/conv0_fwd.hip b/yolo2-pytorch_amd/csrc/conv0_fwd.hip
--- a/yolo2-pytorch_amd/csrc/conv0_fwd.hip
+++ b/yolo2-pytorch_amd/csrc/conv0_fwd.hip
@@ -13,6 +13,7 @@
     int B, H, W, Cout, ldy, ldp;
     float slope;
     int tiles_y, tiles_x, ntiles;
+    const float* pool_sign;
 };
 
 typedef float f32x2 __attribute__((ext_vector_type(2)));
@@ -37,6 +38,7 @@
     const bool has_pool = OUT < 0 ? a.y_pool != nullptr : (OUT & 2) != 0;
     const bool has_stats = OUT < 0 ? a.stats != nullptr : (OUT & 4) != 0;
     constexpr bool POOL_FIRST = FULL && OUT == 2 && !RAW;
+    const bool sel = (OUT == 7 && RAW) ? true : (OUT < 0 ? a.pool_sign != nullptr : false);
     constexpr int K = CIN * 9;
     constexpr int KS = (K + 1) / 2;
     constexpr int PR = TH + 2;
@@ -54,6 +56,13 @@
         const int n = j * 32 + l31;
         sc[j] = (!RAW && a.scale != nullptr && n < a.Cout) ? a.scale[n] : 1.f;
         sh[j] = (!RAW && a.shift != nullptr && n < a.Cout) ? a.shift[n] : 0.f;
+    }
+    float sg[NBLK];
+#pragma unroll
+    for (int j = 0; j < NBLK; ++j) {
+        const int n = j * 32 + l31;
+        const float gm = (sel && n < a.Cout) ? a.pool_sign[n] : 0.f;
+        sg[j] = gm > 0.f ? 1.f : (gm < 0.f ? -1.f : 0.f);
     }
     float wreg[NBLK][KS];
 #pragma unroll
@@ -227,7 +236,18 @@
                     }
                 }
                 if (has_pool && (FULL || (Y < a.H && X < a.W))) {
-                    const float pm = fmaxf(fmaxf(v[0], v[1]), fmaxf(v[2], v[3]));
+                    float pm;
+                    if (sel) {
+                        float best = sg[j] * v[0];
+                        pm = v[0];
+#pragma unroll
+                        for (int q = 1; q < 4; ++q) {
+                            const float key = sg[j] * v[q];
+                            if (key > best) { best = key; pm = v[q]; }
+                        }
+                    } else {
+                        pm = fmaxf(fmaxf(v[0], v[1]), fmaxf(v[2], v[3]));
+                    }
                     (pb + (2 * g * ldp + j * 32))[plane] = pm;
                 }
             }
@@ -267,6 +287,11 @@
         const int out = (a.y != nullptr ? 1 : 0) | (a.y_pool != nullptr ? 2 : 0) | (a.stats != nullptr ? 4 : 0);
         const bool raw = a.scale == nullptr && a.shift == nullptr && a.slope == 1.f;
         const bool mono = a.slope >= 0.f && a.slope <= 1.f;
+        if (a.pool_sign != nullptr && a.Cout == 32 && out == 7 && raw) {
+            Y2_LAUNCH("conv0_kernel", flops, (conv0_kernel<3, 1, 7, true, true>), dim3((unsigned)grid), dim3(256), 0, s, a);
+            Y2_LAUNCH_CHECK();
+            return Y2_OK;
+        }
 #define Y2_C0(NB_, OUT_, RAW_) Y2_LAUNCH("conv0_kernel", flops, (conv0_kernel<3, NB_, OUT_, true, RAW_>), dim3((unsigned)grid), dim3(256), 0, s, a)
         bool done = true;
         if (a.Cout == 32) {
@@ -286,9 +311,23 @@
 
 }
 
+static int conv0_fwd_impl(const float* x_nchw, const float* w, const float* scale, const float* shift, float* y, float* y_pool, double* stats,
+                          int B, int H, int W, int Cin, int Cout, int ldy, int ldp, float slope, y2_stream_t stream, const float* pool_sign);
+
 extern "C" int y2_conv0_fwd(const float* x_nchw, const float* w, const float* scale, const float* shift,
                             float* y, float* y_pool, double* stats,
                             int B, int H, int W, int Cin, int Cout, int ldy, int ldp, float slope, y2_stream_t stream) {
+    return conv0_fwd_impl(x_nchw, w, scale, shift, y, y_pool, stats, B, H, W, Cin, Cout, ldy, ldp, slope, stream, nullptr);
+}
+
+extern "C" int y2_conv0_fwd_sel(const float* x_nchw, const float* w, const float* gamma, float* z, float* z_sel, double* stats,
+                                int B, int H, int W, int Cin, int Cout, int ldz, int ldzs, y2_stream_t stream) {
+    return (gamma != nullptr && z != nullptr && z_sel != nullptr) ? conv0_fwd_impl(x_nchw, w, nullptr, nullptr, z, z_sel, stats, B, H, W, Cin, Cout, ldz, ldzs, 1.f, stream, gamma)
+                                                                  : Y2_EINVAL;
+}
+
+static int conv0_fwd_impl(const float* x_nchw, const float* w, const float* scale, const float* shift, float* y, float* y_pool, double* stats,
+                          int B, int H, int W, int Cin, int Cout, int ldy, int ldp, float slope, y2_stream_t stream, const float* pool_sign) {
     if (x_nchw == nullptr || w == nullptr || (y == nullptr && y_pool == nullptr && stats == nullptr)) return Y2_EINVAL;
     if (B <= 0 || H <= 0 || W <= 0 || Cin < 1 || Cin > 4 || Cout < 1 || Cout > 64) return Y2_ENOSUP;
     if (y != nullptr && ldy < Cout) return Y2_EINVAL;
@@ -296,7 +335,7 @@
     if (stats != nullptr && y2_det.on) return Y2_ENOSUP;
     Conv0Args a;
     a.x = x_nchw; a.w = w; a.scale = scale; a.shift = shift; a.y = y; a.y_pool = y_pool; a.stats = stats;
-    a.B = B; a.H = H; a.W = W; a.Cout = Cout; a.ldy = ldy; a.ldp = ldp; a.slope = slope;
+    a.B = B; a.H = H; a.W = W; a.Cout = Cout; a.ldy = ldy; a.ldp = ldp; a.slope = slope; a.pool_sign = pool_sign;
     a.tiles_y = y2_cdiv(H, TH); a.tiles_x = y2_cdiv(W, TW);
     a.ntiles = B * a.tiles_y * a.tiles_x;
     hipStream_t s = y2_s(stream);
diff --git a/yolo2-pytorch_amd/csrc/train.hip b/yolo2-pytorch_amd/csrc/train.hip
--- a/yolo2-pytorch_amd/csrc/train.hip
+++ b/yolo2-pytorch_amd/csrc/train.hip
@@ -39,6 +39,7 @@
     float slope;
     const float* res; int ldr;
     y2_fastdiv d_wo, d_ho;
+    float* z_sel; int ldzs;
 };
 
 __device__ __forceinline__ float act1(float z, float sc, float sh, float slope) {
@@ -54,7 +55,7 @@
     b = (int)bb;
 }
 
-template <bool POOL, int CV>
+template <bool POOL, int CV, bool SEL = false>
 __global__ void bn_act_fwd_kernel(const ActArgs a, long long total) {
     const int Cg = a.C / CV;
     const int Wo = POOL ? a.W / 2 : a.W, Ho = POOL ? a.H / 2 : a.H;
@@ -69,20 +70,21 @@
     for (uint32_t p = (uint32_t)(tid / Cg); p < npix; p += pstep) {
         int b = 0, yo = 0, xo = 0;
         if (need_yx) act_decode(p, a.d_wo, a.d_ho, Wo, Ho, b, yo, xo);
-        float pm[CV];
+        float pm[CV], bm[CV], zm[CV];
 #pragma unroll
         for (int q = 0; q < (POOL ? 4 : 1); ++q) {
             const int yy = POOL ? 2 * yo + (q >> 1) : yo, xx = POOL ? 2 * xo + (q & 1) : xo;
             const long long pix = need_yx ? ((long long)b * a.H + yy) * a.W + xx : (long long)p;
-            float v[CV];
+            float v[CV], zr[CV];
             if (CV == 4) {
                 const f32x4 zz = *reinterpret_cast<const f32x4*>(a.z + pix * a.ldz + c);
                 f32x4 rr = {0.f, 0.f, 0.f, 0.f};
                 if (a.res != nullptr) rr = *reinterpret_cast<const f32x4*>(a.res + pix * a.ldr + c);
 #pragma unroll
-                for (int e = 0; e < 4; ++e) { const float u = zz[e] * sc[e] + sh[e] + rr[e]; v[e] = u > 0.f ? u : u * a.slope; }
+                for (int e = 0; e < 4; ++e) { const float u = zz[e] * sc[e] + sh[e] + rr[e]; v[e] = u > 0.f ? u : u * a.slope; zr[e] = zz[e]; }
             } else {
-                const float u = a.z[pix * a.ldz + c] * sc[0] + sh[0] + (a.res != nullptr ? a.res[pix * a.ldr + c] : 0.f);
+                zr[0] = a.z[pix * a.ldz + c];
+                const float u = zr[0] * sc[0] + sh[0] + (a.res != nullptr ? a.res[pix * a.ldr + c] : 0.f);
                 v[0] = u > 0.f ? u : u * a.slope;
             }
             if (a.y != nullptr) {
@@ -96,12 +98,20 @@
                 else a.y[o] = v[0];
             }
 #pragma unroll
-            for (int e = 0; e < CV; ++e) pm[e] = (q == 0) ? v[e] : fmaxf(pm[e], v[e]);
+            for (int e = 0; e < CV; ++e) {
+                if (SEL && (q == 0 || v[e] > bm[e])) { bm[e] = v[e]; zm[e] = zr[e]; }
+                pm[e] = (q == 0) ? v[e] : fmaxf(pm[e], v[e]);
+            }
         }
         if (POOL && a.y_pool != nullptr) {
             const long long o = (long long)p * a.ldp + a.poff + c;
             if (CV == 4) { f32x4 w = {pm[0], pm[1], pm[2], pm[3]}; *reinterpret_cast<f32x4*>(a.y_pool + o) = w; }
             else a.y_pool[o] = pm[0];
+        }
+        if (POOL && SEL) {
+            const long long o = (long long)p * a.ldzs + c;
+            if (CV == 4) { f32x4 w = {zm[0], zm[1], zm[2], zm[3]}; *reinterpret_cast<f32x4*>(a.z_sel + o) = w; }
+            else a.z_sel[o] = zm[0];
         }
     }
 }
@@ -838,34 +848,50 @@
     return Y2_OK;
 }
 
-extern "C" int y2_bn_act_fwd_ex(const float* z, const float* scale, const float* shift, float slope, const float* residual, int ldr, float* y, float* y_pool,
-                                int B, int H, int W, int C, int ldz, int ldy, int coff, int ldp, int poff, int out_mode, y2_stream_t stream) {
+static int bn_act_fwd_impl(const float* z, const float* scale, const float* shift, float slope, const float* residual, int ldr, float* y, float* y_pool,
+                           int B, int H, int W, int C, int ldz, int ldy, int coff, int ldp, int poff, int out_mode, y2_stream_t stream, float* z_sel, int ldzs) {
     if (!z || (!y && !y_pool) || B <= 0 || H <= 0 || W <= 0 || C <= 0) return Y2_EINVAL;
     const bool pool = y_pool != nullptr;
+    if (z_sel != nullptr && (!pool || residual != nullptr || ldzs < C)) return Y2_EINVAL;
     if ((pool || out_mode == 1) && ((H & 1) || (W & 1))) return Y2_EINVAL;
     ActArgs a;
     a.z = z; a.scale = scale; a.shift = shift; a.y = y; a.y_pool = y_pool;
     a.B = B; a.H = H; a.W = W; a.C = C; a.ldz = ldz; a.ldy = ldy; a.coff = coff; a.ldp = ldp; a.poff = poff; a.out_mode = out_mode; a.slope = slope;
-    a.res = residual; a.ldr = ldr;
+    a.res = residual; a.ldr = ldr; a.z_sel = z_sel; a.ldzs = ldzs;
     if (residual != nullptr && ldr < C) return Y2_EINVAL;
-    const bool vec = (!residual || (!(ldr & 3) && y2_aligned16(residual))) && !(C & 3) && !(ldz & 3) && (!y || (!(ldy & 3) && !(coff & 3) && y2_aligned16(y))) && (!pool || (!(ldp & 3) && !(poff & 3) && y2_aligned16(y_pool))) && y2_aligned16(z);
+    const bool vec = (!residual || (!(ldr & 3) && y2_aligned16(residual))) && !(C & 3) && !(ldz & 3) && (!y || (!(ldy & 3) && !(coff & 3) && y2_aligned16(y))) && (!pool || (!(ldp & 3) && !(poff & 3) && y2_aligned16(y_pool))) && y2_aligned16(z) &&
+                     (!z_sel || (!(ldzs & 3) && y2_aligned16(z_sel)));
     const long long pix = (long long)B * (pool ? H / 2 : H) * (pool ? W / 2 : W);
     if (pix >= 0x7fffffffLL || C > 8192) return Y2_ENOSUP;
     const long long total = pix * (vec ? C / 4 : C);
     const int grid = act_grid(total, vec ? C / 4 : C);
     a.d_wo = y2_make_fastdiv((uint32_t)(pool ? W / 2 : W)); a.d_ho = y2_make_fastdiv((uint32_t)(pool ? H / 2 : H));
     hipStream_t s = y2_s(stream);
-    if (pool) { if (vec) Y2_LAUNCH("bn_act_fwd_kernel", 0.0, (bn_act_fwd_kernel<true, 4>), dim3(grid), dim3(256), 0, s, a, total); else Y2_LAUNCH("bn_act_fwd_kernel", 0.0, (bn_act_fwd_kernel<true, 1>), dim3(grid), dim3(256), 0, s, a, total); }
+    if (z_sel != nullptr) { if (vec) Y2_LAUNCH("bn_act_fwd_kernel", 0.0, (bn_act_fwd_kernel<true, 4, true>), dim3(grid), dim3(256), 0, s, a, total); else Y2_LAUNCH("bn_act_fwd_kernel", 0.0, (bn_act_fwd_kernel<true, 1, true>), dim3(grid), dim3(256), 0, s, a, total); }
+    else if (pool) { if (vec) Y2_LAUNCH("bn_act_fwd_kernel", 0.0, (bn_act_fwd_kernel<true, 4>), dim3(grid), dim3(256), 0, s, a, total); else Y2_LAUNCH("bn_act_fwd_kernel", 0.0, (bn_act_fwd_kernel<true, 1>), dim3(grid), dim3(256), 0, s, a, total); }
     else { if (vec) Y2_LAUNCH("bn_act_fwd_kernel", 0.0, (bn_act_fwd_kernel<false, 4>), dim3(grid), dim3(256), 0, s, a, total); else Y2_LAUNCH("bn_act_fwd_kernel", 0.0, (bn_act_fwd_kernel<false, 1>), dim3(grid), dim3(256), 0, s, a, total); }
     Y2_LAUNCH_CHECK();
     return Y2_OK;
 }
 
+extern "C" int y2_bn_act_fwd_ex(const float* z, const float* scale, const float* shift, float slope, const float* residual, int ldr, float* y, float* y_pool,
+                                int B, int H, int W, int C, int ldz, int ldy, int coff, int ldp, int poff, int out_mode, y2_stream_t stream) {
+    return bn_act_fwd_impl(z, scale, shift, slope, residual, ldr, y, y_pool, B, H, W, C, ldz, ldy, coff, ldp, poff, out_mode, stream, nullptr, 0);
+}
+
+extern "C" int y2_bn_act_fwd_sel(const float* z, const float* scale, const float* shift, float slope, float* y_pool, float* z_sel,
+                                 int B, int H, int W, int C, int ldz, int ldp, int poff, int ldzs, y2_stream_t stream) {
+    if (!y_pool || !z_sel) return Y2_EINVAL;
+    return bn_act_fwd_impl(z, scale, shift, slope, nullptr, 0, nullptr, y_pool, B, H, W, C, ldz, 0, 0, ldp, poff, 0, stream, z_sel, ldzs);
+}
+
 static int bn_act_bwd_impl(const float* z, const float* scale, const float* shift, const float* mean, const float* invstd, const float* gamma,
                            float slope, const float* dy_full, int ldf, int foff, int fmode, const float* dy_pool, int ldp, int poff,
                            const float* dy_full2, int ld2, const float* residual, int ldr, float* dres, int lddr,
-                           double* sums, float* dz, int ldd, int B, int H, int W, int C, int ldz, int has_bn, y2_stream_t stream, float* park, long long park_floats) {
+                           double* sums, float* dz, int ldd, int B, int H, int W, int C, int ldz, int has_bn, y2_stream_t stream, float* park, long long park_floats,
+                           const float* z_sel = nullptr, int ldzs = 0) {
     if (!z || (!dy_full && !dy_pool) || !sums || B <= 0 || H <= 0 || W <= 0 || C <= 0) return Y2_EINVAL;
+    if (z_sel != nullptr && (!dy_pool || dy_full || dy_full2 || residual || has_bn != 1 || ldzs < C)) return Y2_EINVAL;
     if (dz == nullptr && dres != nullptr) return Y2_EINVAL;
     if (has_bn < 0 || has_bn > 2 || (has_bn && (!mean || !invstd || !gamma))) return Y2_EINVAL;
     const bool pool = dy_pool != nullptr;
@@ -878,7 +904,8 @@
     a.slope = slope; a.n = (double)B * H * W; a.has_bn = has_bn;
     a.dy_full2 = dy_full2; a.ld2 = ld2; a.res = residual; a.ldr = ldr; a.dres = dres; a.lddr = lddr;
     const bool vec = (!dy_full2 || (!(ld2 & 3) && y2_aligned16(dy_full2))) && (!residual || (!(ldr & 3) && y2_aligned16(residual))) && (!dres || (!(lddr & 3) && y2_aligned16(dres))) && !(C & 3) && !(ldz & 3) && (!dz || (!(ldd & 3) && y2_aligned16(dz))) && y2_aligned16(z) &&
-                     (!dy_full || (!(ldf & 3) && !(foff & 3) && y2_aligned16(dy_full))) && (!pool || (!(ldp & 3) && !(poff & 3) && y2_aligned16(dy_pool)));
+                     (!dy_full || (!(ldf & 3) && !(foff & 3) && y2_aligned16(dy_full))) && (!pool || (!(ldp & 3) && !(poff & 3) && y2_aligned16(dy_pool))) &&
+                     (!z_sel || (!(ldzs & 3) && y2_aligned16(z_sel)));
     const int Cg = vec ? C / 4 : C;
     const long long pix = (long long)B * (pool ? H / 2 : H) * (pool ? W / 2 : W);
     if (pix >= 0x7fffffffLL) return Y2_ENOSUP;
@@ -897,7 +924,7 @@
     };
     const long long opix = pix;
     const bool aliased = dz != nullptr && (overlaps(z, npix * ldz) || overlaps(dy_full, (fmode == 1 ? npix / 4 : npix) * (long long)ldf) || overlaps(dy_pool, opix * ldp) ||
-                                           overlaps(dy_full2, npix * ld2) || overlaps(residual, npix * ldr) || overlaps(dres, npix * lddr));
+                                           overlaps(dy_full2, npix * ld2) || overlaps(residual, npix * ldr) || overlaps(dres, npix * lddr) || overlaps(z_sel, opix * ldzs));
     a.block_partial = (dz != nullptr && !aliased && !y2_det.on && ldd == C && grid > 16 && (long long)grid * 2 * C <= npix * ldd) ? dz : nullptr;
     if (dz == nullptr && park != nullptr && !y2_det.on && grid > 16 && (long long)grid * 2 * C <= park_floats && y2_aligned16(park)) a.block_partial = park;
     const long long prow = (long long)grid * 256 / Cg;
@@ -905,9 +932,14 @@
         if ((size_t)prow * 2 * C * sizeof(float) > y2_det.bytes || prow > 0x7fffffffLL) return Y2_EINVAL;
         a.partial = y2_det.ws;
     }
+    ActBwdArgs a1 = a;
+    if (z_sel != nullptr) {
+        a1.z = z_sel; a1.ldz = ldzs; a1.dy_full = dy_pool; a1.ldf = ldp; a1.foff = poff; a1.fmode = 0; a1.dy_pool = nullptr; a1.H = H / 2; a1.W = W / 2;
+    }
 #define Y2_BWD(POOL, CV)                                                                                             \
     do {                                                                                                             \
-        Y2_LAUNCH("bn_act_bwd_kernel", 0.0, (bn_act_bwd_kernel<POOL, CV, false>), dim3(grid), dim3(256), lds, s, a, total);            \
+        if (z_sel != nullptr) Y2_LAUNCH("bn_act_bwd_kernel", 0.0, (bn_act_bwd_kernel<false, CV, false>), dim3(grid), dim3(256), lds, s, a1, total);            \
+        else Y2_LAUNCH("bn_act_bwd_kernel", 0.0, (bn_act_bwd_kernel<POOL, CV, false>), dim3(grid), dim3(256), lds, s, a, total);            \
         if (a.partial != nullptr) {                                                                                  \
             const int rc_ = y2_det_reduce_f32(a.partial, (int)prow, (long long)2 * C, (long long)2 * C, sums, nullptr, s);            \
             if (rc_ != Y2_OK) return rc_;                                                                            \
@@ -929,6 +961,14 @@
                                 double* sums, float* dz, int ldd, int B, int H, int W, int C, int ldz, int has_bn, y2_stream_t stream) {
     return bn_act_bwd_impl(z, scale, shift, mean, invstd, gamma, slope, dy_full, ldf, foff, fmode, dy_pool, ldp, poff, dy_full2, ld2, residual, ldr, dres, lddr,
                            sums, dz, ldd, B, H, W, C, ldz, has_bn, stream, nullptr, 0);
+}
+
+extern "C" int y2_bn_act_bwd_sel(const float* z, const float* z_sel, int ldzs, const float* scale, const float* shift, const float* mean, const float* invstd,
+                                 const float* gamma, float slope, const float* dy_pool, int ldp, int poff, double* sums, float* dz, int ldd,
+                                 int B, int H, int W, int C, int ldz, y2_stream_t stream) {
+    if (!z_sel) return Y2_EINVAL;
+    return bn_act_bwd_impl(z, scale, shift, mean, invstd, gamma, slope, nullptr, 0, 0, 0, dy_pool, ldp, poff, nullptr, 0, nullptr, 0, nullptr, 0,
+                           sums, dz, ldd, B, H, W, C, ldz, 1, stream, nullptr, 0, z_sel, ldzs);
 }
 
 extern "C" long long y2_wino6_tiles(int32_t B, int32_t H, int32_t W) {
diff --git a/yolo2-pytorch_amd/model/train_graph.py b/yolo2-pytorch_amd/model/train_graph.py
--- a/yolo2-pytorch_amd/model/train_graph.py
+++ b/yolo2-pytorch_amd/model/train_graph.py
@@ -26,6 +26,7 @@
 GRAD_F43 = os.environ.get('Y2_GRAD_F43', '1') != '0'
 FUSE_WINO6 = os.environ.get('Y2_FUSE_WINO6', '1') != '0'
 FUSE_CONV0 = os.environ.get('Y2_FUSE_CONV0', '1') != '0'
+POOL_SEL = {'0': False, '1': True, 'act': 'act'}[os.environ.get('Y2_POOL_SEL', '1')]
 DEBUG_TAP = None
 
 SYNC_POSITIVES = True
@@ -98,7 +99,7 @@
 
 class _Block(object):
     __slots__ = ('mod', 'name', 'x', 'ldx', 'H', 'W', 'cin', 'cout', 'k', 'z', 'scale', 'shift', 'mean', 'invstd', 'pool',
-                 'out_full', 'out_pool', 'out_ld', 'out_off', 'out_mode', 'has_bn', 'slope', 'first', 'wino_v', 'eff')
+                 'out_full', 'out_pool', 'out_ld', 'out_off', 'out_mode', 'has_bn', 'slope', 'first', 'wino_v', 'eff', 'z_sel')
 
 
 PRUNE_OPERANDS = os.environ.get('Y2_PRUNE_OPERANDS', '1') != '0'
@@ -294,7 +295,13 @@
         z = _new(dev, B, h, w, cout)
         stats = arena.take(cout) if (blk.has_bn and not frozen) else None
         estats = arena.epilogue(stats)
-        if first:
+        sel = bool(POOL_SEL and pool and out_full is None and not want_full and blk.has_bn and not frozen and not _hip.DETERMINISTIC and not (h & 1) and not (w & 1))
+        blk.z_sel = _new(dev, B, h // 2, w // 2, cout) if sel else None
+        sel_conv = sel and POOL_SEL is True and first
+        if sel_conv:
+            _hip.check(L.y2_conv0_fwd_sel(_hip.ptr(xin), _hip.ptr(e.w), _hip.ptr(e.gamma), _hip.ptr(z), _hip.ptr(blk.z_sel), _hip.ptr(estats),
+                                          B, h, w, cin, cout, cout, cout, st), 'y2_conv0_fwd_sel')
+        elif first:
             _hip.check(L.y2_conv0_fwd(_hip.ptr(xin), _hip.ptr(e.w), None, None, _hip.ptr(z), None, _hip.ptr(estats),
                                       B, h, w, cin, cout, cout, 0, 1.0, st), 'y2_conv0_fwd')
         elif mod in prepared:
@@ -325,8 +332,15 @@
             y_full, out_ld, out_off = _new(dev, B, h, w, cout), cout, 0
         if pool:
             y_pool = _new(dev, B, h // 2, w // 2, cout)
-        _hip.check(L.y2_bn_act_fwd(_hip.ptr(z), _hip.ptr(blk.scale), _hip.ptr(blk.shift), blk.slope, _hip.ptr(y_full), _hip.ptr(y_pool),
-                                   B, h, w, cout, cout, out_ld, out_off, cout, 0, out_mode, st), 'y2_bn_act_fwd')
+        if sel_conv:
+            _hip.check(L.y2_bn_act_fwd(_hip.ptr(blk.z_sel), _hip.ptr(blk.scale), _hip.ptr(blk.shift), blk.slope, _hip.ptr(y_pool), None,
+                                       B, h // 2, w // 2, cout, cout, cout, 0, 0, 0, 0, st), 'y2_bn_act_fwd')
+        elif sel:
+            _hip.check(L.y2_bn_act_fwd_sel(_hip.ptr(z), _hip.ptr(blk.scale), _hip.ptr(blk.shift), blk.slope, _hip.ptr(y_pool), _hip.ptr(blk.z_sel),
+                                           B, h, w, cout, cout, cout, 0, cout, st), 'y2_bn_act_fwd_sel')
+        else:
+            _hip.check(L.y2_bn_act_fwd(_hip.ptr(z), _hip.ptr(blk.scale), _hip.ptr(blk.shift), blk.slope, _hip.ptr(y_full), _hip.ptr(y_pool),
+                                       B, h, w, cout, cout, out_ld, out_off, cout, 0, out_mode, st), 'y2_bn_act_fwd')
         blk.out_full, blk.out_pool, blk.out_ld, blk.out_off, blk.out_mode = y_full, y_pool, out_ld, out_off, out_mode
         blocks.append(blk)
         return blk, y_full, y_pool
@@ -373,8 +387,8 @@
     return cur
 
 
-_Geo = collections.namedtuple('_Geo', 'H W cin cout k ldx first has_v padded ud_ok full pooled')
-_Plan = collections.namedtuple('_Plan', 'wgrad zero final fuse0 fused6 problem')
+_Geo = collections.namedtuple('_Geo', 'H W cin cout k ldx first has_v padded ud_ok full pooled has_sel', defaults=(False,))
+_Plan = collections.namedtuple('_Plan', 'wgrad zero final fuse0 fused6 problem sel', defaults=(False,))
 
 
 def _routes(names, pools, n1, c_pt):
@@ -401,10 +415,11 @@
     plans = []
     for g in geo:
         cop = (g.cout + 3) // 4 * 4
+        sel = bool(g.has_sel and g.pooled and g.full is None)
         if g.first:
             small = g.cin <= 3 and g.cout <= 64
             fuse0 = bool(FUSE_CONV0 and small and g.full is None and g.pooled and not (g.H & 1) and not (g.W & 15) and B * g.H * g.W * g.cout * 4 < 0xffff0000 and not need_dx)
-            plans.append(_Plan(0, small, small, fuse0, None, None))
+            plans.append(_Plan(0, small, small, fuse0, None, None, sel))
             continue
         wgrad = _hip.wgrad_choice(B, g.H, g.W, g.cin, g.ldx, cop, cop, g.k, g.has_v, dev)
         fused6 = problem = None
@@ -413,7 +428,7 @@
             problem = _problem(B, g.H, g.W, cop, cop, g.cin, g.k, g.cin)
             hit = _hip.autotune_conv(problem, dev, f43=True if _f43_offered(g.ud_ok, cop, g.H, g.W) else None, wino_eligible=g.ud_ok, peek=True)
             fused6 = tuple(hit) if (hit is not None and hit[0] == 6) else None
-        plans.append(_Plan(wgrad, wgrad == 0, g.k == 1 and cop == g.cout and not g.padded, False, fused6, problem if fused6 else None))
+        plans.append(_Plan(wgrad, wgrad == 0, g.k == 1 and cop == g.cout and not g.padded, False, fused6, problem if fused6 else None, sel))
     return plans
 
 
@@ -436,7 +451,7 @@
     routes, full, pooled = _routes([b.name for b in blocks], [b.pool for b in blocks], len(dnn._blocks()[0]), c_pt)
     need_dx = bool(getattr(ctx, 'need_dx', False))
     plans = _decide_bwd([_Geo(b.H, b.W, b.cin, b.cout, b.k, b.ldx, b.first, b.wino_v is not None, b.eff.padded,
-                              ctx.prepared[b.mod]['ud_ok'] if (not b.first and b.mod in ctx.prepared) else None, full[i], pooled[i]) for i, b in enumerate(blocks)], B, str(dev), need_dx)
+                              ctx.prepared[b.mod]['ud_ok'] if (not b.first and b.mod in ctx.prepared) else None, full[i], pooled[i], b.z_sel is not None) for i, b in enumerate(blocks)], B, str(dev), need_dx)
     order = list(range(n - 1, -1, -1))
     main = torch.cuda.current_stream(dev)
     side = _side_stream(dev) if (BWD_STREAMS > 1 and not _hip.DETERMINISTIC and (not torch.cuda.is_current_stream_capturing() or getattr(ctx, 'fork_ok', False))) else None
@@ -503,6 +518,9 @@
                                              _hip.ptr(e.gamma) if blk.has_bn else None, blk.slope, _hip.ptr(sf[0]), sf[1], sf[2], _hip.ptr(sums),
                                              _hip.ptr(fused6[0]), _hip.ptr(fused6[1]), None, 0, B, h, w, cout, cout,
                                              (2 if ctx.frozen else 1) if blk.has_bn else 0, st), 'y2_bn_act_bwd_wino6')
+        elif plan.sel:
+            _hip.check(L.y2_bn_act_bwd_sel(_hip.ptr(blk.z), _hip.ptr(blk.z_sel), cout, _hip.ptr(blk.scale), _hip.ptr(blk.shift), _hip.ptr(blk.mean), _hip.ptr(blk.invstd),
+                                           _hip.ptr(e.gamma), blk.slope, _hip.ptr(sp), cout, 0, _hip.ptr(sums), _hip.ptr(dz), cop, B, h, w, cout, cout, st), 'y2_bn_act_bwd_sel')
         else:
             _hip.check(L.y2_bn_act_bwd(_hip.ptr(blk.z), _hip.ptr(blk.scale), _hip.ptr(blk.shift), _hip.ptr(blk.mean), _hip.ptr(blk.invstd),
                                        _hip.ptr(e.gamma) if blk.has_bn else None, blk.slope,
@@ -607,7 +625,7 @@
                     src_pool[j] = dx
                 else:
                     src_full[j] = (dx, cin, off, mode)
-        blk.z = None
+        blk.z = blk.z_sel = None
     sink.hand_affine(sums_arena, affine_grads, st)
     flush_weight_grads()
     L.y2_prof_set_tag(0)
```
